# IBM/BadDiffusion

Hardware: AMD Instinct MI355X
Metric: train images/sec (32x32 UNet, DDPM-CIFAR10-32 topology, bs128/GPU, poison_rate 0.1) (higher is better)
Workload: dtype f32 (split-bf16 hi+lo products, fp32 accumulate); 1 GPU; BASELINE configs[1]: CIFAR10 DDPM-CIFAR10-32 train step, batch 128/GPU, poison_rate 0.1, BOX_14 trigger, HAT target, clip 1.0 + Adam, fp32 storage; global_batch=128, parallelism=dp1, params=35746308

## Files before the change

baddiffusion_amd/_lib.py:

```python
import ctypes as C
import os

import torch

_HERE = os.path.dirname(os.path.abspath(__file__))
LIB_PATH = os.path.join(_HERE, "libbd_hip.so")

i32, i64, f32, f64, vp, sz = C.c_int, C.c_int64, C.c_float, C.c_double, C.c_void_p, C.c_size_t


class PoisonQsampleDesc(C.Structure):
    _fields_ = [("B", i32), ("C", i32), ("H", i32), ("W", i32),
                ("images_f32", vp), ("images_u8", vp), ("is_poison", vp), ("trigger", vp), ("target_img", vp),
                ("noise", vp), ("timesteps", vp), ("alphas", vp), ("alphas_cumprod", vp), ("vmin", f32),
                ("x_noisy", vp), ("ld_noisy", i64), ("target", vp), ("ld_target", i64),
                ("R_out", vp), ("x0_out", vp), ("mask_out", vp), ("image_out", vp), ("row_index", vp), ("flip", vp)]


class QsampleDesc(C.Structure):
    _fields_ = [("B", i32), ("C", i32), ("H", i32), ("W", i32), ("x0", vp), ("R", vp), ("noise", vp),
                ("timesteps", vp), ("alphas", vp), ("alphas_cumprod", vp),
                ("x_noisy", vp), ("ld_noisy", i64), ("target", vp), ("ld_target", i64)]


class DdpmStepDesc(C.Structure):
    _fields_ = [("n", i64), ("model_output", vp), ("sample", vp), ("noise", vp), ("prev_sample", vp),
                ("pred_original", vp), ("alphas_cumprod", vp), ("t", i32), ("prev_t", i32), ("variance_type", i32),
                ("clip_sample", i32), ("clip_sample_range", f32), ("clip_defense", i32), ("clip_defense_range", f32)]


class DdimStepDesc(C.Structure):
    _fields_ = [("n", i64), ("model_output", vp), ("sample", vp), ("noise", vp), ("prev_sample", vp),
                ("pred_original", vp), ("alphas_cumprod", vp), ("t", i32), ("prev_t", i32),
                ("final_alpha_cumprod", f32), ("eta", f32), ("clip_sample", i32), ("clip_sample_range", f32)]


class GnFwdDesc(C.Structure):
    _fields_ = [("B", i32), ("HW", i32), ("C", i32), ("G", i32), ("eps", f32), ("silu", i32),
                ("x", vp), ("ldx", i64), ("gamma", vp), ("beta", vp), ("y", vp), ("ldy", i64),
                ("mean", vp), ("rstd", vp), ("workspace", vp), ("workspace_bytes", sz),
                ("y_split", vp), ("ldys", i64), ("stats", vp), ("stats_splits", i32)]


class GnBwdDesc(C.Structure):
    _fields_ = [("B", i32), ("HW", i32), ("C", i32), ("G", i32), ("silu", i32),
                ("x", vp), ("ldx", i64), ("gamma", vp), ("beta", vp), ("mean", vp), ("rstd", vp),
                ("dy", vp), ("lddy", i64), ("dx", vp), ("lddx", i64), ("accumulate_dx", i32),
                ("dgamma", vp), ("dbeta", vp), ("workspace", vp), ("workspace_bytes", sz),
                ("dx_colsum", vp), ("ld_colsum", i64), ("dx_split", vp), ("lddxs", i64),
                ("dx_add", vp), ("ld_add", i64), ("param_partials", vp), ("dx_split_c0", i32), ("dx_split_c1", i32)]


class GnParamItem(C.Structure):
    _fields_ = [("partials", vp), ("C", i32), ("dgamma", vp), ("dbeta", vp)]


class Operand(C.Structure):
    _fields_ = [("kind", i32), ("kc", i32), ("p", vp), ("ld", i64), ("bs_outer", i64), ("bs_inner", i64),
                ("C", i32), ("Hs", i32), ("Ws", i32), ("Ho", i32), ("Wo", i32), ("stride", i32),
                ("pad_t", i32), ("pad_l", i32), ("ups", i32), ("split", vp)]


class IgemmDesc(C.Structure):
    _fields_ = [("A", Operand), ("B", Operand), ("M", i32), ("N", i32), ("K", i32),
                ("batch_outer", i32), ("batch_inner", i32),
                ("C", vp), ("ldc", i64), ("c_bs_outer", i64), ("c_bs_inner", i64),
                ("alpha", f32), ("out_scale", f32), ("bias", vp),
                ("rowbias", vp), ("ld_rowbias", i64), ("rows_per_group", i32),
                ("residual", vp), ("ldr", i64), ("accumulate", i32), ("ksplit", i32),
                ("workspace", vp), ("workspace_bytes", sz), ("tile", i32), ("mode", i32),
                ("a_colsum", vp)]


class ConvFwdDesc(C.Structure):
    _fields_ = [("B", i32), ("Hs", i32), ("Ws", i32), ("Cin", i32), ("Cout", i32), ("stride", i32),
                ("pad_t", i32), ("pad_l", i32), ("ups", i32), ("Ho", i32), ("Wo", i32),
                ("x", vp), ("ldx", i64), ("w", vp), ("bias", vp), ("rowbias", vp), ("ld_rowbias", i64),
                ("residual", vp), ("ldr", i64), ("out_scale", f32), ("y", vp), ("ldy", i64),
                ("workspace", vp), ("workspace_bytes", sz), ("mode", i32), ("w_split", vp)]


class ConvDgradDesc(C.Structure):
    _fields_ = [("B", i32), ("Hs", i32), ("Ws", i32), ("Cin", i32), ("Cout", i32), ("stride", i32),
                ("pad_t", i32), ("pad_l", i32), ("ups", i32), ("Ho", i32), ("Wo", i32),
                ("dy", vp), ("lddy", i64), ("w", vp), ("dx", vp), ("lddx", i64), ("accumulate", i32),
                ("workspace", vp), ("workspace_bytes", sz), ("mode", i32), ("w_split", vp)]


class ConvWgradDesc(C.Structure):
    _fields_ = [("B", i32), ("Hs", i32), ("Ws", i32), ("Cin", i32), ("Cout", i32), ("stride", i32),
                ("pad_t", i32), ("pad_l", i32), ("ups", i32), ("Ho", i32), ("Wo", i32),
                ("x", vp), ("ldx", i64), ("dy", vp), ("lddy", i64), ("dw", vp),
                ("workspace", vp), ("workspace_bytes", sz), ("mode", i32), ("db", vp)]


class ConvPsDesc(C.Structure):
    _fields_ = [("B", i32), ("H", i32), ("W", i32), ("K", i32), ("N", i32), ("direction", i32),
                ("x_split", vp), ("ldx", i64), ("w_split", vp), ("bias", vp), ("rowbias", vp), ("ld_rowbias", i64),
                ("residual", vp), ("ldr", i64), ("out_scale", f32), ("y", vp), ("ldy", i64), ("accumulate", i32),
                ("workspace", vp), ("workspace_bytes", sz), ("gn_part", vp), ("gn_groups", i32), ("mode", i32)]


class ConvPsWgradDesc(C.Structure):
    _fields_ = [("B", i32), ("H", i32), ("W", i32), ("Cin", i32), ("Cout", i32), ("x_split", vp), ("ldx", i64),
                ("dy_split", vp), ("lddy", i64), ("dw", vp), ("db", vp), ("workspace", vp), ("workspace_bytes", sz),
                ("mode", i32)]


class UpsampleConvDesc(C.Structure):
    _fields_ = [("B", i32), ("H", i32), ("W", i32), ("Cin", i32), ("Cout", i32), ("x_split", vp), ("ldx", i64), ("dy_split", vp),
                ("lddy", i64), ("e_split", vp), ("et_split", vp), ("bias", vp), ("y", vp), ("ldy", i64), ("dx", vp), ("lddx", i64),
                ("accumulate", i32), ("dw", vp), ("db", vp), ("workspace", vp), ("workspace_bytes", sz), ("mode", i32)]


class ConvS2DgradDesc(C.Structure):
    _fields_ = [("B", i32), ("Ho", i32), ("Wo", i32), ("Cin", i32), ("Cout", i32), ("pad", i32), ("dy_split", vp), ("lddy", i64),
                ("wT_split", vp), ("dx", vp), ("lddx", i64), ("accumulate", i32), ("mode", i32)]


class GemmSpDesc(C.Structure):
    _fields_ = [("M", i32), ("N", i32), ("K", i32), ("batch", i32), ("a", vp), ("lda", i64), ("a_bs", i64), ("a_kmajor", i32),
                ("b", vp), ("ldb", i64), ("b_bs", i64), ("b_kmajor", i32), ("c", vp), ("ldc", i64), ("c_bs", i64),
                ("c_split", vp), ("ldcs", i64), ("cs_bs", i64), ("bias", vp), ("residual", vp), ("ldr", i64), ("r_bs", i64),
                ("alpha", f32), ("out_scale", f32), ("accumulate", i32), ("a_colsum", vp), ("workspace", vp), ("workspace_bytes", sz),
                ("mode", i32)]


class AttnSpDesc(C.Structure):
    _fields_ = [("B", i32), ("heads", i32), ("N", i32), ("dh", i32), ("qkv_split", vp), ("ld", i64), ("scale", f32), ("o_split", vp),
                ("ldo", i64), ("pt_split", vp), ("do_split", vp), ("lddo", i64), ("dst_split", vp), ("dqkv_split", vp), ("lddqkv", i64),
                ("mode", i32)]


class Conv2dDesc(C.Structure):
    _fields_ = [("x", vp), ("ldx", i64), ("w", vp), ("bias", vp), ("y", vp), ("ldy", i64), ("B", i32), ("H", i32), ("W", i32), ("Cin", i32),
                ("Cout", i32), ("KH", i32), ("KW", i32), ("stride_h", i32), ("stride_w", i32), ("pad_h", i32), ("pad_w", i32), ("relu", i32),
                ("w_kc", i32)]


class UnetConfig(C.Structure):
    _fields_ = [("sample_size", i32), ("in_channels", i32), ("out_channels", i32), ("num_blocks", i32),
                ("block_out_channels", i32 * 8), ("down_attn", i32 * 8), ("up_attn", i32 * 8),
                ("layers_per_block", i32), ("downsample_padding", i32), ("flip_sin_to_cos", i32),
                ("freq_shift", f32), ("norm_eps", f32), ("norm_num_groups", i32), ("attention_head_dim", i32),
                ("mid_block_scale_factor", f32), ("compute_mode", i32)]


SIGNATURES = {
    "bd_last_error": (C.c_char_p, []),
    "bd_version": (i32, []),
    "bd_poison_qsample": (i32, [C.POINTER(PoisonQsampleDesc), vp]),
    "bd_qsample": (i32, [C.POINTER(QsampleDesc), vp]),
    "bd_nchw_to_nhwc": (i32, [vp, vp, i32, i32, i32, i32, i64, vp]),
    "bd_nhwc_to_nchw": (i32, [vp, i64, vp, i32, i32, i32, i32, vp]),
    "bd_ddpm_step": (i32, [C.POINTER(DdpmStepDesc), vp]),
    "bd_ddim_step": (i32, [C.POINTER(DdimStepDesc), vp]),
    "bd_to_image": (i32, [vp, i32, i64, i32, i32, i32, i32, vp, vp, vp]),
    "bd_timestep_embedding": (i32, [vp, i32, i32, i32, i32, f32, vp, vp]),
    "bd_gn_workspace_bytes": (sz, [i32, i32]),
    "bd_gn_fwd_takes_stats": (i32, [i32, i32, i32, i32]),
    "bd_gn_fwd": (i32, [C.POINTER(GnFwdDesc), vp]),
    "bd_gn_bwd": (i32, [C.POINTER(GnBwdDesc), vp]),
    "bd_lincomb": (i32, [i32, C.POINTER(vp), C.POINTER(f32), i64, i32, f32, vp, vp]),
    "bd_anp_apply": (i32, [vp, i64, vp, vp, vp, i32, i64, vp, vp]),
    "bd_anp_grad": (i32, [vp, vp, vp, i32, i64, vp, vp, vp, vp, vp]),
    "bd_ssim_workspace_bytes": (sz, [i32, i32, i32, i32]),
    "bd_ssim": (i32, [vp, vp, i32, i32, i32, i32, i64, i64, i64, i64, f32, vp, vp, sz, vp]),
    "bd_conv2d_nhwc": (i32, [C.POINTER(Conv2dDesc), vp]),
    "bd_pool2d_nhwc": (i32, [vp, i64, vp, i64, i32, i32, i32, i32, i32, i32, i32, i32, i32, vp]),
    "bd_resize_bilinear_nhwc": (i32, [vp, i32, vp, i32, i32, i32, i32, i32, i32, f32, f32, vp]),
    "bd_global_avgpool_nhwc": (i32, [vp, i64, vp, i32, i32, i32, vp]),
    "bd_gn_bwd_defers": (i32, [i32, i32, i32, i32]),
    "bd_gn_bwd_params": (i32, [C.POINTER(GnParamItem), i32, i32, vp]),
    "bd_igemm_workspace_bytes": (sz, [C.POINTER(IgemmDesc)]),
    "bd_igemm": (i32, [C.POINTER(IgemmDesc), vp]),
    "bd_split_bf16": (i32, [vp, i64, vp, vp]),
    "bd_split_rows": (i32, [vp, i64, i64, i32, vp, i64, vp]),
    "bd_split_wt": (i32, [vp, i32, i32, vp, vp]),
    "bd_split_rows_ups2": (i32, [vp, i64, i32, i32, i32, i32, vp, i64, vp]),
    "bd_conv3x3_ps": (i32, [C.POINTER(ConvPsDesc), vp]),
    "bd_conv3x3_ps_workspace_bytes": (sz, [C.POINTER(ConvPsDesc)]),
    "bd_conv3x3_ps_gn_splits": (i32, [i32, i32, i32, i32, i32, i32]),
    "bd_upsample_weights": (i32, [vp, i32, i32, vp, vp, vp]),
    "bd_upsample_conv_fwd": (i32, [C.POINTER(UpsampleConvDesc), vp]),
    "bd_upsample_conv_dgrad": (i32, [C.POINTER(UpsampleConvDesc), vp]),
    "bd_upsample_conv_wgrad": (i32, [C.POINTER(UpsampleConvDesc), vp]),
    "bd_upsample_conv_wgrad_workspace_bytes": (sz, [C.POINTER(UpsampleConvDesc)]),
    "bd_upsample_conv_dgrad_workspace_bytes": (sz, [C.POINTER(UpsampleConvDesc)]),
    "bd_conv3x3_s2_dgrad_ps": (i32, [C.POINTER(ConvS2DgradDesc), vp]),
    "bd_gemm_sp_workspace_bytes": (sz, [C.POINTER(GemmSpDesc)]),
    "bd_gemm_sp": (i32, [C.POINTER(GemmSpDesc), vp]),
    "bd_attn_sp_supported": (i32, [i32, i32]),
    "bd_attn_sp_fwd": (i32, [C.POINTER(AttnSpDesc), vp]),
    "bd_attn_sp_bwd": (i32, [C.POINTER(AttnSpDesc), vp]),
    "bd_conv3x3_ps_wgrad": (i32, [C.POINTER(ConvPsWgradDesc), vp]),
    "bd_conv3x3_ps_wgrad_workspace_bytes": (sz, [C.POINTER(ConvPsWgradDesc)]),
    "bd_conv3x3_fwd": (i32, [C.POINTER(ConvFwdDesc), vp]),
    "bd_conv3x3_dgrad": (i32, [C.POINTER(ConvDgradDesc), vp]),
    "bd_conv3x3_wgrad": (i32, [C.POINTER(ConvWgradDesc), vp]),
    "bd_conv3x3_workspace_bytes": (sz, [i32] * 8),
    "bd_colsum": (i32, [vp, i64, i64, i32, i64, vp, i64, i32, vp]),
    "bd_sum2x2": (i32, [vp, i64, vp, i64, i32, i32, i32, i32, i32, vp]),
    "bd_softmax_fwd": (i32, [vp, vp, i64, i32, vp]),
    "bd_softmax_bwd": (i32, [vp, vp, vp, i64, i32, vp]),
    "bd_silu_fwd": (i32, [vp, vp, i64, vp]),
    "bd_silu_bwd": (i32, [vp, vp, vp, i64, i32, vp]),
    "bd_reduce_workspace_bytes": (sz, []),
    "bd_loss_fwd_bwd": (i32, [vp, i64, vp, i64, i64, i32, i32, f32, vp, vp, i64, vp, vp]),
    "bd_sumsq": (i32, [vp, i64, vp, vp, vp]),
    "bd_adam_clip": (i32, [vp, vp, vp, vp, i64, vp, f64, f64, f64, f64, f64, i32, vp, vp]),
    "bd_prof_enable": (i32, [i32]),
    "bd_prof_enabled": (i32, []),
    "bd_prof_reset": (i32, []),
    "bd_prof_num_classes": (i32, []),
    "bd_prof_get": (i32, [i32, C.POINTER(C.c_char_p), C.POINTER(i64), C.POINTER(f64), C.POINTER(f64), C.POINTER(f64)]),
    "bd_mfma_probe": (i32, [i32, i32, i32, C.POINTER(f64), vp]),
    "bd_axpy": (i32, [vp, vp, i64, f32, i32, vp]),
    "bd_adam_clip_dev": (i32, [vp, vp, vp, vp, i64, vp, f64, vp, f64, f64, f64, vp, vp]),
    "bd_unet_create": (i32, [C.POINTER(UnetConfig), C.POINTER(vp)]),
    "bd_unet_destroy": (None, [vp]),
    "bd_unet_set_compute_mode": (i32, [vp, i32]),
    "bd_unet_set_deferred_join": (i32, [vp, i32]),
    "bd_unet_stream_wait_aux": (i32, [vp, vp]),
    "bd_unet_num_params": (i64, [vp]),
    "bd_unet_num_tensors": (i32, [vp]),
    "bd_unet_param_info": (i32, [vp, i32, C.POINTER(C.c_char_p), C.POINTER(i64), C.POINTER(i32), i64 * 4, C.POINTER(i32)]),
    "bd_unet_workspace_bytes": (sz, [vp, i32, i32]),
    "bd_unet_forward": (i32, [vp, i32, i32, vp, vp, i64, vp, i32, vp, i64, vp, sz, vp]),
    "bd_unet_backward": (i32, [vp, i32, vp, vp, i64, vp, i64, vp, vp, sz, vp]),
    "bd_unet_backward_input": (i32, [vp, i32, vp, vp, i64, vp, i64, vp, vp, i64, vp, sz, vp]),
    "bd_unet_num_segments": (i32, [vp]),
    "bd_unet_set_aux_stream": (i32, [vp, i32]),
    "bd_unet_set_static_weights": (i32, [vp, i32]),
    "bd_unet_reset_static_cache": (i32, [vp]),
    "bd_tune_set": (i32, [C.c_char_p, i32]),
    "bd_unet_segment_range": (i32, [vp, i32, C.POINTER(i64), C.POINTER(i64)]),
    "bd_unet_segment_num_ranges": (i32, [vp, i32]),
    "bd_unet_segment_range_k": (i32, [vp, i32, i32, C.POINTER(i64), C.POINTER(i64)]),
    "bd_unet_backward_segment": (i32, [vp, i32, i32, vp, vp, i64, vp, i64, vp, vp, sz, vp, C.POINTER(i64), C.POINTER(i64)]),
}

_lib = None


def load():
    global _lib
    if _lib is not None:
        return _lib
    if not os.path.exists(LIB_PATH):
        raise RuntimeError(
            f"{LIB_PATH} is missing: build it with `python -m baddiffusion_amd.build` (hipcc, gfx950). "
            "There is no CPU / PyTorch fallback for the hot path.")
    lib = C.CDLL(LIB_PATH)
    for name, (res, args) in SIGNATURES.items():
        fn = getattr(lib, name)
        fn.restype = res
        fn.argtypes = args
    _lib = lib
    return lib


def check(status, what=""):
    if status != 0:
        msg = load().bd_last_error()
        raise RuntimeError(f"libbd_hip {what} failed ({status}): {msg.decode() if msg else ''}")


def ptr(t):
    return None if t is None else t.data_ptr()


def stream():
    return torch.cuda.current_stream().cuda_stream
```

baddiffusion_amd/csrc/conv_ps.hip:

```cpp
#include "common.h"
#include <string.h>

#include <type_traits>
#include <cstdlib>

namespace bd {

typedef float floatx16 __attribute__((ext_vector_type(16)));
typedef __bf16 bf16x8 __attribute__((ext_vector_type(8)));
typedef __bf16 bf16x2 __attribute__((ext_vector_type(2)));
typedef __attribute__((address_space(3))) void* lds_ptr;
typedef const __attribute__((address_space(1))) void* gbl_ptr;

constexpr int BD_WT_MAX = 64;
constexpr int PS_BM = 256, PS_BN = 128, PS_NT = 512, PS_STAGES = 3;
constexpr int PS_A_BYTES = PS_BM * 128, PS_B_BYTES = PS_BN * 128, PS_STAGE_BYTES = PS_A_BYTES + PS_B_BYTES;
constexpr int PS_LDS_BYTES = PS_STAGES * PS_STAGE_BYTES;

struct PsParams {
    const char* a;
    const char* w;
    float* y;
    const float* bias; const float* rowbias; const float* residual;
    long long lda, ldy, ldr, ld_rowbias;
// ... 1031 lines not shown
                                                            float* __restrict__ dw, float* __restrict__ db, int brows) {
    const long long i = (long long)blockIdx.x * 256 + threadIdx.x;
    const long long n4 = mn >> 2;
    if (i < n4) {
        float4 a = *reinterpret_cast<const float4*>(part + 4 * i);
#pragma unroll 4
        for (int s = 1; s < ksplit; ++s) {
            const float4 b = *reinterpret_cast<const float4*>(part + (long long)s * mn + 4 * i);
            a.x += b.x; a.y += b.y; a.z += b.z; a.w += b.w;
        }
        *reinterpret_cast<float4*>(dw + 4 * i) = a;
    } else if (db && i - n4 < M) {
        const long long m = i - n4;
        float v = 0.f;
        for (int s = 0; s < brows; ++s) v += part[(long long)ksplit * mn + (long long)s * M + m];
        db[m] = v;
    }
}

__device__ __forceinline__ unsigned ps_pack_hi(float a, float b) { return bd_pack_hi(a, b); }
__device__ __forceinline__ unsigned ps_pack_lo(float a, float b) { return bd_pack_lo(a, b); }

__global__ __launch_bounds__(256) void split_rows_kernel(const float* __restrict__ src, long long lds, long long rows, int C,
                                                          unsigned short* __restrict__ dst, long long ldd) {
    const int c8 = C >> 3;
    const long long total = rows * c8;
    for (long long i = (long long)blockIdx.x * 256 + threadIdx.x; i < total; i += (long long)gridDim.x * 256) {
        const long long r = i / c8;
        const int j = (int)(i - r * c8);
        const float4 a = *reinterpret_cast<const float4*>(src + r * lds + j * 8);
        const float4 b = *reinterpret_cast<const float4*>(src + r * lds + j * 8 + 4);
        unsigned short* o = dst + 2 * r * ldd + (j >> 2) * 64 + (j & 3) * 8;
        *reinterpret_cast<uint4*>(o) = make_uint4(ps_pack_hi(a.x, a.y), ps_pack_hi(a.z, a.w), ps_pack_hi(b.x, b.y), ps_pack_hi(b.z, b.w));
        *reinterpret_cast<uint4*>(o + 32) = make_uint4(ps_pack_lo(a.x, a.y), ps_pack_lo(a.z, a.w), ps_pack_lo(b.x, b.y), ps_pack_lo(b.z, b.w));
    }
}

__global__ __launch_bounds__(256) void split_rows_ups2_kernel(const float* __restrict__ src, long long lds, int B, int H, int W, int C,
                                                               unsigned short* __restrict__ dst, long long ldd) {
    const int c8 = C >> 3;
    const long long total = (long long)B * 4 * H * W * c8;
    for (long long i = (long long)blockIdx.x * 256 + threadIdx.x; i < total; i += (long long)gridDim.x * 256) {
        const long long r = i / c8;
        const int j = (int)(i - r * c8);
        const int x = (int)(r % (2 * W));
        const long long t = r / (2 * W);
        const int y = (int)(t % (2 * H));
        const long long b = t / (2 * H);
        const long long rs = (b * H + (y >> 1)) * W + (x >> 1);
        const float4 a = *reinterpret_cast<const float4*>(src + rs * lds + j * 8);
        const float4 bb = *reinterpret_cast<const float4*>(src + rs * lds + j * 8 + 4);
        unsigned short* o = dst + 2 * r * ldd + (j >> 2) * 64 + (j & 3) * 8;
        *reinterpret_cast<uint4*>(o) = make_uint4(ps_pack_hi(a.x, a.y), ps_pack_hi(a.z, a.w), ps_pack_hi(bb.x, bb.y), ps_pack_hi(bb.z, bb.w));
        *reinterpret_cast<uint4*>(o + 32) = make_uint4(ps_pack_lo(a.x, a.y), ps_pack_lo(a.z, a.w), ps_pack_lo(bb.x, bb.y), ps_pack_lo(bb.z, bb.w));
    }
}

__global__ __launch_bounds__(256) void split_wT_kernel(const float* __restrict__ w, int Cin, int Cout, unsigned short* __restrict__ out) {
    __shared__ float t[32][33];
    const int cib = blockIdx.x, cob = blockIdx.y, tap = blockIdx.z;
    const int tx = threadIdx.x & 31, ty = threadIdx.x >> 5;
#pragma unroll
    for (int i = 0; i < 4; ++i) {
        const int co = cob * 32 + ty + 8 * i;
        t[ty + 8 * i][tx] = w[((long long)co * 9 + tap) * Cin + cib * 32 + tx];
    }
    __syncthreads();
    const int r = threadIdx.x >> 3, c4 = (threadIdx.x & 7) * 4;
    const float v0 = t[c4][r], v1 = t[c4 + 1][r], v2 = t[c4 + 2][r], v3 = t[c4 + 3][r];
    unsigned short* o = out + 2 * (((long long)(cib * 32 + r) * 9 + tap) * Cout + cob * 32) + c4;
    *reinterpret_cast<uint2*>(o) = make_uint2(ps_pack_hi(v0, v1), ps_pack_hi(v2, v3));
    *reinterpret_cast<uint2*>(o + 32) = make_uint2(ps_pack_lo(v0, v1), ps_pack_lo(v2, v3));
}

struct WtTable {
    int n;
    long long off[BD_WT_MAX];
    int cin[BD_WT_MAX], cout[BD_WT_MAX], blk0[BD_WT_MAX + 1];
};
__global__ __launch_bounds__(256) void split_wT_batched_kernel(const float* __restrict__ params, unsigned short* __restrict__ out, WtTable t) {
    __shared__ float tl[32][33];
    int e = 0;
    while (e + 1 < t.n && (int)blockIdx.x >= t.blk0[e + 1]) ++e;
    const int Cin = t.cin[e], Cout = t.cout[e];
    const float* w = params + t.off[e];
    unsigned short* o_base = out + 2 * t.off[e];
    int b = blockIdx.x - t.blk0[e];
    const int ncib = Cin / 32, ncob = Cout / 32;
    const int cib = b % ncib; b /= ncib;
    const int cob = b % ncob; const int tap = b / ncob;
    const int tx = threadIdx.x & 31, ty = threadIdx.x >> 5;
#pragma unroll
    for (int i = 0; i < 4; ++i) {
        const int co = cob * 32 + ty + 8 * i;
        tl[ty + 8 * i][tx] = w[((long long)co * 9 + tap) * Cin + cib * 32 + tx];
    }
    __syncthreads();
    const int r = threadIdx.x >> 3, c4 = (threadIdx.x & 7) * 4;
    const float v0 = tl[c4][r], v1 = tl[c4 + 1][r], v2 = tl[c4 + 2][r], v3 = tl[c4 + 3][r];
    unsigned short* o = o_base + 2 * (((long long)(cib * 32 + r) * 9 + tap) * Cout + cob * 32) + c4;
    *reinterpret_cast<uint2*>(o) = make_uint2(ps_pack_hi(v0, v1), ps_pack_hi(v2, v3));
    *reinterpret_cast<uint2*>(o + 32) = make_uint2(ps_pack_lo(v0, v1), ps_pack_lo(v2, v3));
}

int split_wt_batched(const float* params, uint16_t* out, const long long* off, const int* cin, const int* cout, int n, hipStream_t st) {
    for (int i0 = 0; i0 < n; i0 += BD_WT_MAX) {
        WtTable t;
        t.n = n - i0 < BD_WT_MAX ? n - i0 : BD_WT_MAX;
        int blk = 0;
        for (int i = 0; i < t.n; ++i) {
            t.off[i] = off[i0 + i]; t.cin[i] = cin[i0 + i]; t.cout[i] = cout[i0 + i]; t.blk0[i] = blk;
            blk += 9 * (t.cin[i] / 32) * (t.cout[i] / 32);
        }
        t.blk0[t.n] = blk;
        hipLaunchKernelGGL(split_wT_batched_kernel, dim3((unsigned)blk), dim3(256), 0, st, params, out, t);
        BD_LAUNCH_CHECK("split_wT_batched");
    }
    return BD_OK;
}

static int ilog2x(int v) {
    if (v <= 0 || (v & (v - 1))) return -1;
    int l = 0;
    while ((1 << l) < v) ++l;
    return l;
}

bool conv3x3_ps_supported(int B, int H, int W, int K_channels, int N_channels) {
    return B > 0 && ilog2x(H) >= 0 && ilog2x(W) >= 0 && K_channels % 32 == 0 && N_channels % PS_BN == 0 && K_channels >= 32;
}
static bool ps_large(long long M, int N) { return cdiv(M, PS_BM) * (N / PS_BN) >= 96; }
static void ps_small_split(long long M, int N, int K, int& ksplit, int& cps) {
    const long long tiles = cdiv(M, 128) * (N / 128);
    const int nchunks = 9 * (K / 32);
    static const int slots = [] {
        int dev = 0, cus = 256;
        if (hipGetDevice(&dev) == hipSuccess) (void)hipDeviceGetAttribute(&cus, hipDeviceAttributeMultiprocessorCount, dev);
        return cus;
    }();
    constexpr int mincps = 4;
    int ks = (int)(slots / tiles);
    if (ks < 1) ks = 1;
    if (ks > nchunks / mincps) ks = nchunks / mincps;
    if (ks < 1) ks = 1;
    cps = (int)cdiv(nchunks, ks);
    ksplit = (int)cdiv(nchunks, cps);
}
size_t conv3x3_ps_workspace_bytes(const bd_conv3x3_ps_desc& d) {
    const long long M = (long long)d.B * d.H * d.W;
    if (d.N % PS_BN || ps_large(M, d.N)) return 0;
    int ks, cps;
    ps_small_split(M, d.N, d.K, ks, cps);
    return ks > 1 ? (size_t)ks * (size_t)M * d.N * sizeof(float) : 0;
}

static bool ps_takes_v3(int B, int H, int W, int N) {
    static const bool v3_off = getenv("BD_PS_V3") && atoi(getenv("BD_PS_V3")) == 0;
    static const int v3_maxw = getenv("BD_PS_V3_MAXW") ? atoi(getenv("BD_PS_V3_MAXW")) : (1 << 30);
    const long long M = (long long)B * H * W;
    const int vw = W < 32 ? W : 32;
    return ps_large(M, N) && !v3_off && W >= 16 && W <= v3_maxw && ((long long)H * vw) % PS_BM == 0 && M % PS_BM == 0;
}
int conv3x3_ps_gn_splits(int B, int H, int W, int K, int N, int groups) {
    if (B <= 0 || ilog2x(H) < 0 || ilog2x(W) < 0 || K <= 0 || K % 32 || N <= 0 || N % PS_BN || groups <= 0 || N % groups) return 0;
    const int lc = ilog2x(N / groups);
    if (lc < 2 || lc > 5 || (H * W) % PS_BM) return 0;
    return ps_takes_v3(B, H, W, N) ? H * W / PS_BM : 0;
}

int conv3x3_ps(const bd_conv3x3_ps_desc& d, hipStream_t st) {
    BD_CHECK(d.x_split && d.w_split && d.y, BD_ERR_INVALID, "conv3x3_ps: null pointer");
    BD_CHECK(d.B > 0 && ilog2x(d.H) >= 0 && ilog2x(d.W) >= 0, BD_ERR_UNSUPPORTED, "conv3x3_ps: H, W must be powers of two");
    BD_CHECK(d.K > 0 && d.K % 32 == 0 && d.N > 0 && d.N % PS_BN == 0, BD_ERR_UNSUPPORTED,
             "conv3x3_ps: K channels %% 32 and N channels %% %d must be 0 (got %d, %d)", PS_BN, d.K, d.N);
    BD_CHECK(d.ldx % 32 == 0 && ((uintptr_t)d.x_split & 127) == 0 && ((uintptr_t)d.w_split & 127) == 0, BD_ERR_UNSUPPORTED,
             "conv3x3_ps: split planes need ld %% 32 == 0 and 128-byte aligned bases");
    BD_CHECK(d.direction == 1 || d.direction == -1, BD_ERR_INVALID, "conv3x3_ps: direction must be +1 or -1");
    BD_CHECK(sp_mode_valid(d.mode), BD_ERR_INVALID, "conv3x3_ps: unknown compute mode %d", d.mode);
    const bool sp = d.mode == BD_MODE_BF16;
    BD_CHECK(d.ldy % 4 == 0 && ((uintptr_t)d.y & 15) == 0, BD_ERR_UNSUPPORTED, "conv3x3_ps: y needs ldy %% 4 == 0 and a 16-byte aligned base");
    BD_CHECK(!d.residual || (d.ldr % 4 == 0 && ((uintptr_t)d.residual & 15) == 0), BD_ERR_UNSUPPORTED,
             "conv3x3_ps: residual needs ldr %% 4 == 0 and a 16-byte aligned base");
    BD_CHECK(!d.rowbias || (d.ld_rowbias % 4 == 0 && ((uintptr_t)d.rowbias & 15) == 0), BD_ERR_UNSUPPORTED,
             "conv3x3_ps: rowbias needs ld_rowbias %% 4 == 0 and a 16-byte aligned base");
    BD_CHECK(!d.bias || ((uintptr_t)d.bias & 15) == 0, BD_ERR_UNSUPPORTED, "conv3x3_ps: bias needs a 16-byte aligned base");
    const long long M = (long long)d.B * d.H * d.W;
    BD_CHECK(M < (1ll << 31), BD_ERR_UNSUPPORTED, "conv3x3_ps: pixel count overflows int32");
    BD_CHECK((long long)(d.W + 1) * d.ldx * 4 < (1ll << 31), BD_ERR_UNSUPPORTED, "conv3x3_ps: row pitch too large");
    PsParams p = {};
    p.a = reinterpret_cast<const char*>(d.x_split); p.w = reinterpret_cast<const char*>(d.w_split);
    p.y = d.y; p.bias = d.bias; p.rowbias = d.rowbias; p.residual = d.residual;
    p.lda = d.ldx; p.ldy = d.ldy; p.ldr = d.ldr; p.ld_rowbias = d.ld_rowbias;
    p.C = d.K; p.H = d.H; p.W = d.W; p.lw = ilog2x(d.W); p.lhw = ilog2x(d.W) + ilog2x(d.H);
    p.sign = d.direction; p.M = (int)M; p.N = d.N;
    p.out_scale = d.out_scale == 0.f ? 1.f : d.out_scale; p.accumulate = d.accumulate;
    const bool large = ps_large(M, d.N);
    int rec = -1;
    if (prof_on()) {
        static const char* kName[2][2][2] = {{{"conv_ps128_dgrad", "conv_ps_dgrad"}, {"conv_ps128_fwd", "conv_ps_fwd"}},
                                             {{"conv_ps128_dgrad_bf16", "conv_ps_dgrad_bf16"}, {"conv_ps128_fwd_bf16", "conv_ps_fwd_bf16"}}};
        rec = prof_begin(kName[sp][d.direction > 0][large],
                         2.0 * (double)M * d.N * 9.0 * d.K, ((double)M * d.K + 9.0 * d.K * d.N + (double)M * d.N) * 4.0, st);
    }
    const int epi = (d.residual ? 1 : 0) | (d.rowbias ? 2 : 0) | (d.accumulate ? 4 : 0);
    if (large) {
        p.tiles_m = (int)cdiv(M, PS_BM); p.tiles_n = d.N / PS_BN;
        const dim3 grid((unsigned)(p.tiles_m * p.tiles_n)), block(PS_NT);
        const int vw = d.W < 32 ? d.W : 32;
        const bool v3 = ps_takes_v3(d.B, d.H, d.W, d.N);
        p.lvw = ilog2x(vw);
        if (d.gn_part) {
            BD_CHECK(d.direction == 1 && (epi == 1 || epi == 2) && conv3x3_ps_gn_splits(d.B, d.H, d.W, d.K, d.N, d.gn_groups) > 0, BD_ERR_UNSUPPORTED,
                     "conv3x3_ps: gn_part needs a forward call with exactly one of rowbias / residual and bd_conv3x3_ps_gn_splits() > 0");
            p.gn_part = d.gn_part; p.gn_G = d.gn_groups; p.gn_lcpg = ilog2x(d.N / d.gn_groups);
        }
#define PS_LAUNCH(E) do { if (v3) { if (sp) hipLaunchKernelGGL((conv_ps3_kernel<E, true>), grid, block, 0, st, p); \
                                    else hipLaunchKernelGGL((conv_ps3_kernel<E, false>), grid, block, 0, st, p); } \
                          else if (sp) hipLaunchKernelGGL((conv_ps_kernel<E, true>), grid, block, 0, st, p); \
                          else hipLaunchKernelGGL((conv_ps_kernel<E, false>), grid, block, 0, st, p); } while (0)
        switch (epi) {
            case 0: PS_LAUNCH(0); break;
            case 1: PS_LAUNCH(1); break;
            case 2: PS_LAUNCH(2); break;
            case 3: PS_LAUNCH(3); break;
            case 4: PS_LAUNCH(4); break;
            case 5: PS_LAUNCH(5); break;
            case 6: PS_LAUNCH(6); break;
            default: PS_LAUNCH(7); break;
        }
#undef PS_LAUNCH
        BD_LAUNCH_CHECK("conv_ps");
    } else {
        BD_CHECK(!d.gn_part, BD_ERR_UNSUPPORTED, "conv3x3_ps: gn_part on a small layer (bd_conv3x3_ps_gn_splits() == 0)");
        PsSmallParams pp = {};
        p.tiles_m = (int)cdiv(M, 128); p.tiles_n = d.N / 128;
        pp.q = p;
        ps_small_split(M, d.N, d.K, pp.ksplit, pp.cps);
        if (pp.ksplit > 1) {
            const size_t need = (size_t)pp.ksplit * (size_t)M * d.N * sizeof(float);
            BD_CHECK(d.workspace && d.workspace_bytes >= need, BD_ERR_WORKSPACE, "conv3x3_ps: split-K needs %zu workspace bytes, got %zu", need,
                     d.workspace_bytes);
            pp.partial = reinterpret_cast<float*>(d.workspace);
        }
        const dim3 grid((unsigned)(p.tiles_m * p.tiles_n * pp.ksplit)), block(512);
        constexpr int deep_maxcps = 9;
#define PS128_LAUNCH(E, ...) do { if (sp) hipLaunchKernelGGL((conv_ps128_kernel<E, true, ##__VA_ARGS__>), grid, block, 0, st, pp); \
                                      else hipLaunchKernelGGL((conv_ps128_kernel<E, false, ##__VA_ARGS__>), grid, block, 0, st, pp); } while (0)
        if (pp.ksplit > 1 && pp.cps <= deep_maxcps) {
            PS128_LAUNCH(0, 4);
        } else
        switch (pp.ksplit > 1 ? 0 : epi) {
            case 0: PS128_LAUNCH(0); break;
            case 1: PS128_LAUNCH(1); break;
            case 2: PS128_LAUNCH(2); break;
            case 3: PS128_LAUNCH(3); break;
            case 4: PS128_LAUNCH(4); break;
            case 5: PS128_LAUNCH(5); break;
            case 6: PS128_LAUNCH(6); break;
            default: PS128_LAUNCH(7); break;
        }
#undef PS128_LAUNCH
        BD_LAUNCH_CHECK("conv_ps128");
        if (pp.ksplit > 1) {
            hipLaunchKernelGGL(conv_ps128_reduce, dim3((unsigned)cdiv(M * (d.N / 4), 256)), dim3(256), 0, st, pp);
            BD_LAUNCH_CHECK("conv_ps128_reduce");
        }
    }
    prof_end(rec, st);
    return BD_OK;
}

bool conv3x3_ps_wgrad_supported(int B, int H, int W, int Cin, int Cout) {
    return B > 0 && ilog2x(H) >= 0 && ilog2x(W) >= 0 && Cin % WG_BN == 0 && Cout % WG_BM == 0;
}
static bool ps_wgrad_v3(const bd_conv3x3_ps_wgrad_desc& d) {
    static const bool off = getenv("BD_PS_WG3") && atoi(getenv("BD_PS_WG3")) == 0;
    static const int maxw = getenv("BD_PS_WG3_MAXW") ? atoi(getenv("BD_PS_WG3_MAXW")) : (1 << 30);
    return !off && d.W >= 16 && d.W <= maxw && ((long long)d.B * d.H * d.W) % 32 == 0;
}
static int g_wg3_slots_override = 0;
static void ps_wgrad_split(const bd_conv3x3_ps_wgrad_desc& d, int& ksplit, int& cps) {
    const bool v3 = ps_wgrad_v3(d);
    const long long tiles = (long long)(d.Cout / WG_BM) * ((v3 ? 3 : 9) * d.Cin / WG_BN);
    const int nchunks = (int)cdiv((long long)d.B * d.H * d.W, 32);
    static const int slots = [] {
        int dev = 0, cus = 256;
        if (hipGetDevice(&dev) == hipSuccess) (void)hipDeviceGetAttribute(&cus, hipDeviceAttributeMultiprocessorCount, dev);
        return 2 * cus;
    }();
    static const int slots3_getenv = getenv("BD_PS_WG3_SLOTS") ? atoi(getenv("BD_PS_WG3_SLOTS")) : 0;
    const int slots3_env = g_wg3_slots_override > 0 ? g_wg3_slots_override : slots3_getenv;
    const int slots3 = slots3_env > 0 ? slots3_env : (d.W > 32 ? slots / 4 : slots * 3 / 8);
    constexpr int mincps = 8;
    int ks = (int)((v3 ? slots3 : slots) / tiles);
    if (ks < 1) ks = 1;
    if (ks > nchunks / mincps) ks = nchunks / mincps > 0 ? nchunks / mincps : 1;
    cps = (int)cdiv(nchunks, ks);
    ksplit = (int)cdiv(nchunks, cps);
}
size_t conv3x3_ps_wgrad_workspace_bytes(const bd_conv3x3_ps_wgrad_desc& d) {
    int ks, cps;
    ps_wgrad_split(d, ks, cps);
    return ks > 1 ? (size_t)ks * ((size_t)d.Cout * 9 * d.Cin + d.Cout) * sizeof(float) : 0;
}
int conv3x3_ps_wgrad(const bd_conv3x3_ps_wgrad_desc& d, hipStream_t st) {
    BD_CHECK(d.x_split && d.dy_split && d.dw, BD_ERR_INVALID, "conv3x3_ps_wgrad: null pointer");
    BD_CHECK(d.B > 0 && conv3x3_ps_wgrad_supported(d.B, d.H, d.W, d.Cin, d.Cout), BD_ERR_UNSUPPORTED,
             "conv3x3_ps_wgrad: needs power-of-two H, W, Cin and Cout multiples of 128");
    BD_CHECK(d.ldx % 32 == 0 && d.lddy % 32 == 0 && ((uintptr_t)d.x_split & 127) == 0 && ((uintptr_t)d.dy_split & 127) == 0,
             BD_ERR_UNSUPPORTED, "conv3x3_ps_wgrad: split planes need ld %% 32 == 0 and 128-byte aligned bases");
    BD_CHECK(sp_mode_valid(d.mode), BD_ERR_INVALID, "conv3x3_ps_wgrad: unknown compute mode %d", d.mode);
    const bool sp = d.mode == BD_MODE_BF16;
    PsWgParams p = {};
    p.dy = reinterpret_cast<const char*>(d.dy_split); p.x = reinterpret_cast<const char*>(d.x_split);
    p.lddy = d.lddy; p.ldx = d.ldx; p.Cin = d.Cin; p.Cout = d.Cout; p.H = d.H; p.W = d.W; p.lw = ilog2x(d.W);
    p.lh = ilog2x(d.H); p.lvw = ilog2x(d.W < 32 ? d.W : 32);
    p.P = d.B * d.H * d.W;
    const bool v3 = ps_wgrad_v3(d);
    p.tiles_m = d.Cout / WG_BM; p.tiles_n = (v3 ? 3 : 9) * d.Cin / WG_BN; p.ntaps = 9;
    ps_wgrad_split(d, p.ksplit, p.cps);
    p.want_db = d.db != nullptr;
    const long long mn = (long long)d.Cout * 9 * d.Cin;
    if (p.ksplit > 1) {
        const size_t need = (size_t)p.ksplit * ((size_t)mn + d.Cout) * sizeof(float);
        BD_CHECK(d.workspace && d.workspace_bytes >= need, BD_ERR_WORKSPACE, "conv3x3_ps_wgrad: workspace %zu < %zu", d.workspace_bytes, need);
        p.out = reinterpret_cast<float*>(d.workspace);
    } else {
        p.out = d.dw; p.db = d.db;
    }
    int rec = -1;
    if (prof_on())
        rec = prof_begin(v3 ? (sp ? "conv_ps_wgrad3_bf16" : "conv_ps_wgrad3") : (sp ? "conv_ps_wgrad_bf16" : "conv_ps_wgrad"), 2.0 * (double)p.P * d.Cout * 9.0 * d.Cin,
                         ((double)p.P * (d.Cin + d.Cout) + 9.0 * d.Cin * d.Cout) * 4.0, st);
    const dim3 grid((unsigned)(p.tiles_m * p.tiles_n * p.ksplit));
    if (v3 && sp) hipLaunchKernelGGL(conv_ps_wgrad3_kernel<true>, grid, dim3(512), 0, st, p);
    else if (v3) hipLaunchKernelGGL(conv_ps_wgrad3_kernel<false>, grid, dim3(512), 0, st, p);
    else if (sp) hipLaunchKernelGGL((conv_ps_wgrad_kernel<2, 8, true>), grid, dim3(512), 0, st, p);
    else hipLaunchKernelGGL((conv_ps_wgrad_kernel<2, 8, false>), grid, dim3(512), 0, st, p);
    BD_LAUNCH_CHECK("conv_ps_wgrad");
    if (p.ksplit > 1) {
        const long long total = mn / 4 + (d.db ? d.Cout : 0);
        if (v3) hipLaunchKernelGGL(conv_ps_wgrad_reduce<true>, dim3((unsigned)cdiv(total, 256)), dim3(256), 0, st, p.out, p.ksplit, mn, d.Cout, d.dw, d.db, p.ksplit);
        else hipLaunchKernelGGL(conv_ps_wgrad_reduce<false>, dim3((unsigned)cdiv(total, 256)), dim3(256), 0, st, p.out, p.ksplit, mn, d.Cout, d.dw, d.db, p.ksplit);
        BD_LAUNCH_CHECK("conv_ps_wgrad_reduce");
    }
    prof_end(rec, st);
    return BD_OK;
}

int ups_dweff_combine(const float* de, int Cin, int Cout, float* dw, hipStream_t st);

static void ups_wgrad_split(const bd_upsample_conv_desc& d, int& ksplit, int& cps) {
    bd_conv3x3_ps_wgrad_desc q = {};
    q.B = d.B; q.H = d.H; q.W = d.W; q.Cin = d.Cin; q.Cout = d.Cout;
    const long long tiles = (long long)(d.Cout / WG_BM) * (16 * d.Cin / WG_BN);
    const int nchunks = (int)cdiv((long long)d.B * d.H * d.W, 32);
    int dev = 0, cus = 256;
    if (hipGetDevice(&dev) == hipSuccess) (void)hipDeviceGetAttribute(&cus, hipDeviceAttributeMultiprocessorCount, dev);
    int ks = (int)(2 * cus / tiles);
    if (ks < 1) ks = 1;
    if (ks > nchunks / 8) ks = nchunks / 8 > 0 ? nchunks / 8 : 1;
    cps = (int)cdiv(nchunks, ks);
    ksplit = (int)cdiv(nchunks, cps);
}
size_t upsample_conv_wgrad_workspace_bytes(const bd_upsample_conv_desc& d) {
    int ks, cps;
    ups_wgrad_split(d, ks, cps);
    const size_t mn = (size_t)d.Cout * 16 * d.Cin;
    return ((size_t)ks * (mn + 4 * (size_t)d.Cout) + mn) * sizeof(float);
}
int upsample_conv_wgrad(const bd_upsample_conv_desc& d, hipStream_t st) {
    BD_CHECK(d.x_split && d.dy_split && d.dw, BD_ERR_INVALID, "bd_upsample_conv_wgrad: null pointer");
    BD_CHECK(d.B > 0 && conv3x3_ps_wgrad_supported(d.B, d.H, d.W, d.Cin, d.Cout), BD_ERR_UNSUPPORTED,
             "bd_upsample_conv_wgrad: needs power-of-two H, W, Cin and Cout multiples of 128");
    BD_CHECK(d.ldx % 32 == 0 && d.lddy % 32 == 0 && ((uintptr_t)d.x_split & 127) == 0 && ((uintptr_t)d.dy_split & 127) == 0,
             BD_ERR_UNSUPPORTED, "bd_upsample_conv_wgrad: split planes need ld %% 32 == 0 and 128-byte aligned bases");
    BD_CHECK((long long)d.B * d.H * d.W * 4 < (1ll << 31), BD_ERR_UNSUPPORTED, "bd_upsample_conv_wgrad: pixel count overflows int32");
    BD_CHECK(sp_mode_valid(d.mode), BD_ERR_INVALID, "bd_upsample_conv_wgrad: unknown compute mode %d", d.mode);
    const size_t need = upsample_conv_wgrad_workspace_bytes(d);
    BD_CHECK(d.workspace && d.workspace_bytes >= need, BD_ERR_WORKSPACE, "bd_upsample_conv_wgrad: workspace %zu < %zu", d.workspace_bytes, need);
    PsWgParams p = {};
    p.dy = reinterpret_cast<const char*>(d.dy_split); p.x = reinterpret_cast<const char*>(d.x_split);
    p.lddy = d.lddy; p.ldx = d.ldx; p.Cin = d.Cin; p.Cout = d.Cout; p.H = d.H; p.W = d.W; p.lw = ilog2x(d.W);
    p.P = d.B * d.H * d.W;
    p.tiles_m = d.Cout / WG_BM; p.tiles_n = 16 * d.Cin / WG_BN; p.ntaps = 16;
    ups_wgrad_split(d, p.ksplit, p.cps);
    p.want_db = d.db != nullptr;
    const long long mn = (long long)d.Cout * 16 * d.Cin;
    p.out = reinterpret_cast<float*>(d.workspace);
    float* de = p.out + (size_t)p.ksplit * ((size_t)mn + 4 * (size_t)d.Cout);
    int rec = -1;
    if (prof_on())
        rec = prof_begin(d.mode == BD_MODE_BF16 ? "conv_ph_ups_wgrad_bf16" : "conv_ph_ups_wgrad", 2.0 * (double)p.P * 4.0 * d.Cout * 9.0 * d.Cin,
                         ((double)p.P * (d.Cin + 4.0 * d.Cout) + 9.0 * d.Cin * d.Cout) * 4.0, st);
    const dim3 grid((unsigned)(p.tiles_m * p.tiles_n * p.ksplit));
    if (d.mode == BD_MODE_BF16) hipLaunchKernelGGL((conv_ps_wgrad_kernel<2, 8, true, true>), grid, dim3(512), 0, st, p);
    else hipLaunchKernelGGL((conv_ps_wgrad_kernel<2, 8, false, true>), grid, dim3(512), 0, st, p);
    BD_LAUNCH_CHECK("conv_ps_wgrad (phase)");
    const long long total = mn / 4 + (d.db ? d.Cout : 0);
    hipLaunchKernelGGL(conv_ps_wgrad_reduce<false>, dim3((unsigned)cdiv(total, 256)), dim3(256), 0, st, p.out, p.ksplit, mn, d.Cout, de, d.db, 4 * p.ksplit);
    BD_LAUNCH_CHECK("conv_ps_wgrad_reduce (phase)");
    BD_TRY(ups_dweff_combine(de, d.Cin, d.Cout, d.dw, st));
    prof_end(rec, st);
    return BD_OK;
}

int g_tune_gen = 0;
int tune_set(const char* key, int value) {
    BD_CHECK(key, BD_ERR_INVALID, "bd_tune_set: null key");
    if (!strcmp(key, "ps_wg3_slots")) { g_wg3_slots_override = value > 0 ? value : 0; ++g_tune_gen; return BD_OK; }
    set_error("bd_tune_set: unknown key '%s' (known: ps_wg3_slots)", key);
    return BD_ERR_INVALID;
}
}

extern "C" int bd_tune_set(const char* key, int value) { return bd::tune_set(key, value); }
extern "C" size_t bd_upsample_conv_wgrad_workspace_bytes(const bd_upsample_conv_desc* d) {
    return d ? bd::upsample_conv_wgrad_workspace_bytes(*d) : 0;
}
extern "C" int bd_upsample_conv_wgrad(const bd_upsample_conv_desc* d, bd_stream_t s) {
    BD_CHECK(d, BD_ERR_INVALID, "bd_upsample_conv_wgrad: null descriptor");
    return bd::upsample_conv_wgrad(*d, bd::S(s));
}
extern "C" size_t bd_conv3x3_ps_workspace_bytes(const bd_conv3x3_ps_desc* d) { return d ? bd::conv3x3_ps_workspace_bytes(*d) : 0; }
extern "C" int bd_conv3x3_ps_gn_splits(int B, int H, int W, int K, int N, int groups) { return bd::conv3x3_ps_gn_splits(B, H, W, K, N, groups); }
extern "C" int bd_conv3x3_ps(const bd_conv3x3_ps_desc* d, bd_stream_t s) {
    BD_CHECK(d, BD_ERR_INVALID, "bd_conv3x3_ps: null descriptor");
    return bd::conv3x3_ps(*d, bd::S(s));
}
extern "C" int bd_conv3x3_ps_wgrad(const bd_conv3x3_ps_wgrad_desc* d, bd_stream_t s) {
    BD_CHECK(d, BD_ERR_INVALID, "bd_conv3x3_ps_wgrad: null descriptor");
    return bd::conv3x3_ps_wgrad(*d, bd::S(s));
}
extern "C" size_t bd_conv3x3_ps_wgrad_workspace_bytes(const bd_conv3x3_ps_wgrad_desc* d) {
    return d ? bd::conv3x3_ps_wgrad_workspace_bytes(*d) : 0;
}
extern "C" int bd_split_rows(const float* src, int64_t ld_src, int64_t rows, int C, uint16_t* dst, int64_t ld_dst, bd_stream_t stream) {
    BD_CHECK(src && dst && rows > 0 && C > 0, BD_ERR_INVALID, "bd_split_rows: bad args");
    BD_CHECK(C % 32 == 0 && ld_dst % 32 == 0 && (ld_src & 3) == 0 && bd::aligned16(src) && ((uintptr_t)dst & 127) == 0, BD_ERR_UNSUPPORTED,
             "bd_split_rows: C, ld_dst %% 32, ld_src %% 4, 16-byte aligned src and 128-byte aligned dst required");
    long long nb = bd::cdiv(rows * (C / 8), 256);
    if (nb > 8192) nb = 8192;
    hipLaunchKernelGGL(bd::split_rows_kernel, dim3((unsigned)nb), dim3(256), 0, bd::S(stream), src, (long long)ld_src, (long long)rows, C, dst,
                       (long long)ld_dst);
    BD_LAUNCH_CHECK("split_rows");
    return BD_OK;
}
extern "C" int bd_split_rows_ups2(const float* src, int64_t ld_src, int B, int H, int W, int C, uint16_t* dst, int64_t ld_dst, bd_stream_t stream) {
    BD_CHECK(src && dst && B > 0 && H > 0 && W > 0 && C > 0, BD_ERR_INVALID, "bd_split_rows_ups2: bad args");
    BD_CHECK(C % 32 == 0 && ld_dst % 32 == 0 && (ld_src & 3) == 0 && bd::aligned16(src) && ((uintptr_t)dst & 127) == 0, BD_ERR_UNSUPPORTED,
             "bd_split_rows_ups2: C, ld_dst %% 32, ld_src %% 4, 16-byte aligned src and 128-byte aligned dst required");
    long long nb = bd::cdiv((long long)B * 4 * H * W * (C / 8), 256);
    if (nb > 8192) nb = 8192;
    hipLaunchKernelGGL(bd::split_rows_ups2_kernel, dim3((unsigned)nb), dim3(256), 0, bd::S(stream), src, (long long)ld_src, B, H, W, C, dst,
                       (long long)ld_dst);
    BD_LAUNCH_CHECK("split_rows_ups2");
    return BD_OK;
}
extern "C" int bd_split_wt(const float* w, int Cin, int Cout, uint16_t* out, bd_stream_t stream) {
    BD_CHECK(w && out && Cin > 0 && Cout > 0, BD_ERR_INVALID, "bd_split_wt: bad args");
    BD_CHECK(Cin % 32 == 0 && Cout % 32 == 0 && ((uintptr_t)out & 127) == 0, BD_ERR_UNSUPPORTED, "bd_split_wt: Cin, Cout %% 32 and 128-byte aligned out required");
    hipLaunchKernelGGL(bd::split_wT_kernel, dim3(Cin / 32, Cout / 32, 9), dim3(256), 0, bd::S(stream), w, Cin, Cout, out);
    BD_LAUNCH_CHECK("split_wT");
    return BD_OK;
}
```

baddiffusion_amd/csrc/groupnorm.hip:

```cpp
#include "common.h"

namespace bd {

constexpr int GN_MAX_SPLITS = 128;

static int gn_max_splits(int B) {
    int s = 512 / (B > 0 ? B : 1);
    return s < 1 ? 1 : (s > GN_MAX_SPLITS ? GN_MAX_SPLITS : s);
}
static int gn_splits(int B, int HW) {
    int s = 512 / (B > 0 ? B : 1);
    if (s < 1) s = 1;
    if (s > GN_MAX_SPLITS) s = GN_MAX_SPLITS;
    while (s > 1 && HW / s < 32) s >>= 1;
    return s;
}
static void gn_block(int C, int& threads, int& r) {
    const int q = C / 4;
    r = 256 / q;
    if (r < 1) r = 1;
    threads = q * r;
}

static int gn_apply_rows(int HW, int r) {
// ... 297 lines not shown
            for (int sp = sub; sp < S; sp += nsub) s += (double)p[(long long)sp * 3 * C];
        }
        red[t] = s;
        __syncthreads();
        if (base + t < items && t < (nsub > 1 ? items : 256)) {
            double v = red[t];
            for (int k = 1; k < nsub; ++k) v += red[k * items + t];
            tot[base + t] = v;
        }
        __syncthreads();
    }
    if (t < 2) {
        double v = 0.0;
        const double* q = tot + (t == 0 ? cpg : 0);
        for (int c = 0; c < cpg; ++c) v += q[c] * (double)gamma[g * cpg + c];
        sg[t] = v;
        ds[((long long)b * G + g) * 2 + t] = (float)v;
    }
    if (ppart)
        for (int i = t; i < 2 * cpg; i += 256) {
            const int plane = i / cpg, c = g * cpg + i - plane * cpg;
            ppart[((long long)b * 2 + plane) * C + c] = (float)tot[i];
        }
    if (dx_colsum) {
        __syncthreads();
        const float s1 = (float)sg[0], s2 = (float)sg[1], rs = rstd[b * G + g];
        for (int cl = t; cl < cpg; cl += 256) {
            const int c = g * cpg + cl;
            const float sa = (float)tot[cpg + cl], sh2 = (float)tot[2 * cpg + cl];
            dx_colsum[(long long)b * ld_colsum + c] = rs * (gamma[c] * sa - ((float)HW * s1 + s2 * sh2) * inv_n);
        }
    }
}

__global__ void gn_bwd_apply_kernel(const float* __restrict__ x, long long ldx, const float* __restrict__ dy, long long lddy,
                                    float* __restrict__ dx, long long lddx, int HW, int C, int G, int r, int per,
                                    const float* __restrict__ ds, const float* __restrict__ gamma,
                                    const float* __restrict__ beta, const float* __restrict__ mean,
                                    const float* __restrict__ rstd, float inv_n, int silu, int acc,
                                    unsigned short* __restrict__ dxs, long long lddxs, const float* __restrict__ addp,
                                    long long ldadd, int dxs_c0, int dxs_c1) {
    const int q = C / 4, cpg = C / G;
    const int t = threadIdx.x;
    const int cq = t % q, prow = t / q;
    const int b = blockIdx.y;
    const int p0 = blockIdx.x * per;
    int p1 = p0 + per;
    if (p1 > HW) p1 = HW;
    float mu[4], rs[4], gg[4], bb[4], g1[4], g2[4];
#pragma unroll
    for (int j = 0; j < 4; ++j) {
        const int c = cq * 4 + j, g = c / cpg;
        mu[j] = mean[b * G + g]; rs[j] = rstd[b * G + g];
        g1[j] = ds[((long long)b * G + g) * 2]; g2[j] = ds[((long long)b * G + g) * 2 + 1];
        gg[j] = gamma[c]; bb[j] = beta[c];
    }
    const float* xb = x + (long long)b * HW * ldx + cq * 4;
    const float* db = dy + (long long)b * HW * lddy + cq * 4;
    float* ob = dx + (long long)b * HW * lddx + cq * 4;
    const bool do_acc = dx && acc;
    const float* ab = addp ? addp + (long long)b * HW * ldadd + cq * 4 : xb;
    for (int p = p0 + prow; p < p1; p += 2 * r) {
        float4 v[2], d[2], e[2], a2[2];
#pragma unroll
        for (int u = 0; u < 2; ++u) {
            const bool ok = p + u * r < p1;
            v[u] = gn_ld4_if(xb + (long long)(p + u * r) * ldx, ok);
            d[u] = gn_ld4_if(db + (long long)(p + u * r) * lddy, ok);
            e[u] = gn_ld4_if(ob + (long long)(p + u * r) * lddx, ok && do_acc);
            a2[u] = gn_ld4_if(ab + (long long)(p + u * r) * ldadd, ok && addp != nullptr);
        }
#pragma unroll
        for (int u = 0; u < 2; ++u) {
            const float in[4] = {v[u].x, v[u].y, v[u].z, v[u].w}, dd[4] = {d[u].x, d[u].y, d[u].z, d[u].w};
            const float ee[4] = {e[u].x, e[u].y, e[u].z, e[u].w}, aa[4] = {a2[u].x, a2[u].y, a2[u].z, a2[u].w};
            float o[4];
#pragma unroll
            for (int j = 0; j < 4; ++j) {
                const float xh = (in[j] - mu[j]) * rs[j];
                float dz = dd[j];
                if (silu) dz *= silu_grad_fast(xh * gg[j] + bb[j]);
                o[j] = (rs[j] * (dz * gg[j] - (g1[j] + xh * g2[j]) * inv_n) + ee[j]) + aa[j];
            }
            v[u] = make_float4(o[0], o[1], o[2], o[3]);
        }
#pragma unroll
        for (int u = 0; u < 2; ++u) {
            const int pu = p + u * r;
            if (pu < p1) {
                if (dx) *reinterpret_cast<float4*>(ob + (long long)pu * lddx) = v[u];
                if (dxs && cq * 4 >= dxs_c0 && cq * 4 < dxs_c1) {
                    const float o[4] = {v[u].x, v[u].y, v[u].z, v[u].w};
                    gn_store_split4(dxs + 2 * ((long long)b * HW + pu) * lddxs, cq * 4 - dxs_c0, o);
                }
            }
        }
    }
}

constexpr int GN_RES_EMAX = 16;

struct GnRes {
    int cb, q, R, E, nblk, nt;
};
static int gcd_i(int a, int b) { return b ? gcd_i(b, a % b) : a; }
static bool gn_resident_plan(int B, int HW, int C, int G, GnRes& o, bool wide_ok = false) {
    const int cpg = C / G;
    const int unit = cpg / gcd_i(cpg, 4) * 4;
    for (int nt = 256; nt <= 512; nt *= 2) {
        int best = 0;
        for (int cb = unit; cb <= C; cb += unit) {
            if (C % cb) continue;
            const int q = cb / 4;
            if (q > nt) break;
            if (cdiv(HW, nt / q) <= GN_RES_EMAX && cb / cpg <= 256) best = cb;
        }
        if (!best || (best < 16 && best < C)) continue;
        constexpr int row_align = 64;
        if ((best * 4) % row_align != 0 && best < C) continue;
        while ((long long)B * (C / best) < 512) {
            const int half = best / 2;
            if (half < 16 || half % unit || C % half) break;
            best = half;
        }
        o.cb = best; o.q = best / 4; o.R = nt / o.q; o.E = (int)cdiv(HW, o.R); o.nblk = C / best; o.nt = nt;
        if (wide_ok && nt == 256 && o.E > 8 && 512 % o.q == 0) { o.nt = 512; o.R = 512 / o.q; o.E = (int)cdiv(HW, o.R); }
        return true;
    }
    return false;
}

struct GnCoord {
    int b, bx;
};
__device__ __forceinline__ GnCoord gn_res_coord(int nblk) {
    const unsigned L = blockIdx.x, T = gridDim.x, qq = T >> 3;
    unsigned j = (L & 7) * qq + (L >> 3);
    if (L >= (qq << 3)) j = L;
    GnCoord c;
    c.b = (int)(j / (unsigned)nblk);
    c.bx = (int)(j - (unsigned)c.b * (unsigned)nblk);
    return c;
}

__device__ __forceinline__ void gn_fwd_group_stats(double a, double c2, double n, float eps, float* st, float* mean, float* rstd) {
    const double mu = a / n;
    double var = c2 / n - mu * mu;
    if (var < 0.0) var = 0.0;
    const float m = (float)mu, r = (float)(1.0 / sqrt(var + (double)eps));
    st[0] = m; st[1] = r;
    *mean = m; *rstd = r;
}

template <int EMAX, int NT>
__global__ __launch_bounds__(NT, NT == 256 ? 4 : 2) void gn_fwd_res_kernel(const float* __restrict__ x, long long ldx, float* __restrict__ y,
                                                       long long ldy, int HW, int C, int G, int cb, int q, int R, int E,
                                                       float eps, const float* __restrict__ gamma,
                                                       const float* __restrict__ beta, float* __restrict__ mean,
                                                       float* __restrict__ rstd, int silu, unsigned short* __restrict__ ys,
                                                       long long ldys) {
    __shared__ double shd[4 * NT];
    float* sh = reinterpret_cast<float*>(shd);
    __shared__ float st[2 * 256];
    const int t = threadIdx.x;
    const int cq = t % q, prow = t / q;
    const bool active = prow < R;
    const GnCoord wgc = gn_res_coord(C / cb);
    const int b = wgc.b, c0 = wgc.bx * cb;
    const int cpg = C / G, ng = cb / cpg;
    const float* xb = x + (long long)b * HW * ldx + c0 + cq * 4;
    float4 v[EMAX];
    float sm[4] = {0.f, 0.f, 0.f, 0.f}, sq[4] = {0.f, 0.f, 0.f, 0.f};
#pragma unroll
    for (int i = 0; i < EMAX; ++i) {
        const int p = prow + R * i;
        const bool ok = active && i < E && p < HW;
        v[i] = gn_ld4_if(xb + (long long)p * ldx, ok);
        sm[0] += v[i].x; sm[1] += v[i].y; sm[2] += v[i].z; sm[3] += v[i].w;
        sq[0] += v[i].x * v[i].x; sq[1] += v[i].y * v[i].y; sq[2] += v[i].z * v[i].z; sq[3] += v[i].w * v[i].w;
    }
    const bool wred = q < 64 && (q & (q - 1)) == 0;
    const int rows = wred ? NT / 64 : R;
    if (wred) {
        double a[4], c2[4];
#pragma unroll
        for (int j = 0; j < 4; ++j) { a[j] = (double)sm[j]; c2[j] = (double)sq[j]; }
        for (int off = q; off < 64; off <<= 1) {
#pragma unroll
            for (int j = 0; j < 4; ++j) { a[j] += __shfl_xor(a[j], off); c2[j] += __shfl_xor(c2[j], off); }
        }
        if ((t & 63) < q) {
#pragma unroll
            for (int j = 0; j < 4; ++j) {
                shd[((t >> 6) * cb + cq * 4 + j) * 2 + 0] = a[j];
                shd[((t >> 6) * cb + cq * 4 + j) * 2 + 1] = c2[j];
            }
        }
    } else if (active) {
#pragma unroll
        for (int j = 0; j < 4; ++j) {
            sh[(prow * cb + cq * 4 + j) * 2 + 0] = sm[j];
            sh[(prow * cb + cq * 4 + j) * 2 + 1] = sq[j];
        }
    }
    __syncthreads();
    if (wred) {
        if (t < ng) {
            double a = 0.0, c2 = 0.0;
            for (int pr = 0; pr < rows; ++pr)
                for (int c = t * cpg; c < (t + 1) * cpg; ++c) {
                    a += shd[(pr * cb + c) * 2 + 0];
                    c2 += shd[(pr * cb + c) * 2 + 1];
                }
            gn_fwd_group_stats(a, c2, (double)HW * cpg, eps, st + 2 * t, mean + b * G + c0 / cpg + t, rstd + b * G + c0 / cpg + t);
        }
    } else {
        for (int g = t >> 6; g < ng; g += NT / 64) {
            double a = 0.0, c2 = 0.0;
            for (int idx = t & 63; idx < R * cpg; idx += 64) {
                const int pr = idx / cpg, c = g * cpg + idx - pr * cpg;
                a += (double)sh[(pr * cb + c) * 2 + 0];
                c2 += (double)sh[(pr * cb + c) * 2 + 1];
            }
            for (int off = 1; off < 64; off <<= 1) { a += __shfl_xor(a, off); c2 += __shfl_xor(c2, off); }
            if ((t & 63) == 0)
                gn_fwd_group_stats(a, c2, (double)HW * cpg, eps, st + 2 * g, mean + b * G + c0 / cpg + g, rstd + b * G + c0 / cpg + g);
        }
    }
    __syncthreads();
    if (!active) return;
    float mu[4], rs[4], gg[4], bb[4];
#pragma unroll
    for (int j = 0; j < 4; ++j) {
        const int lc = cq * 4 + j;
        mu[j] = st[2 * (lc / cpg)]; rs[j] = st[2 * (lc / cpg) + 1];
        gg[j] = gamma[c0 + lc]; bb[j] = beta[c0 + lc];
    }
    float* yb = y + (long long)b * HW * ldy + c0 + cq * 4;
#pragma unroll
    for (int i = 0; i < EMAX; ++i) {
        const float in[4] = {v[i].x, v[i].y, v[i].z, v[i].w};
        float o[4];
#pragma unroll
        for (int j = 0; j < 4; ++j) {
            const float z = (in[j] - mu[j]) * rs[j] * gg[j] + bb[j];
            o[j] = silu ? silu_fast_pinned(z) : z;
        }
        v[i] = make_float4(o[0], o[1], o[2], o[3]);
    }
#pragma unroll
    for (int i = 0; i < EMAX; ++i) {
        const int p = prow + R * i;
        if (i < E && p < HW) {
            if (y) *reinterpret_cast<float4*>(yb + (long long)p * ldy) = v[i];
            if (ys) {
                const float o[4] = {v[i].x, v[i].y, v[i].z, v[i].w};
                gn_store_split4(ys + 2 * ((long long)b * HW + p) * ldys, c0 + cq * 4, o);
            }
        }
    }
}

template <int EMAX, int NT>
__global__ __launch_bounds__(NT) void gn_bwd_res_kernel(const float* __restrict__ x, long long ldx,
                                                       const float* __restrict__ dy, long long lddy, float* __restrict__ dx,
                                                       long long lddx, int HW, int C, int G, int cb, int q, int R, int E,
                                                       const float* __restrict__ gamma, const float* __restrict__ beta,
                                                       const float* __restrict__ mean, const float* __restrict__ rstd,
                                                       int silu, int acc, float* __restrict__ part,
                                                       float* __restrict__ dx_colsum, long long ld_colsum,
                                                       unsigned short* __restrict__ dxs, long long lddxs,
                                                       const float* __restrict__ addp, long long ldadd, int dxs_c0, int dxs_c1) {
    __shared__ float sh[3 * 4 * NT];
    __shared__ float ch[3 * 4 * NT];
    __shared__ float sg[2 * 256];
    const int t = threadIdx.x;
    const int cq = t % q, prow = t / q;
    const bool active = prow < R;
    const GnCoord wgc = gn_res_coord(C / cb);
    const int b = wgc.b, c0 = wgc.bx * cb;
    const int cpg = C / G, ng = cb / cpg;
    const float inv_n = 1.0f / ((float)HW * cpg);
    float mu[4], rs[4], gg[4], bb[4];
#pragma unroll
    for (int j = 0; j < 4; ++j) {
        const int c = c0 + (active ? cq * 4 + j : 0);
        mu[j] = mean[b * G + c / cpg]; rs[j] = rstd[b * G + c / cpg];
        gg[j] = gamma[c]; bb[j] = beta[c];
    }
    const float* xb = x + (long long)b * HW * ldx + c0 + cq * 4;
    const float* db = dy + (long long)b * HW * lddy + c0 + cq * 4;
    float4 xh[EMAX], dz[EMAX];
    float s0[4] = {0.f, 0.f, 0.f, 0.f}, s1[4] = {0.f, 0.f, 0.f, 0.f}, s2[4] = {0.f, 0.f, 0.f, 0.f};
#pragma unroll
    for (int i = 0; i < EMAX; ++i) {
        const int p = prow + R * i;
        const bool ok = active && i < E && p < HW;
        xh[i] = gn_ld4_if(xb + (long long)p * ldx, ok);
        dz[i] = gn_ld4_if(db + (long long)p * lddy, ok);
    }
#pragma unroll
    for (int i = 0; i < EMAX; ++i) {
        const int p = prow + R * i;
        const bool ok = active && i < E && p < HW;
        float in[4] = {xh[i].x, xh[i].y, xh[i].z, xh[i].w}, dd[4] = {dz[i].x, dz[i].y, dz[i].z, dz[i].w};
#pragma unroll
        for (int j = 0; j < 4; ++j) {
            const float h = ok ? (in[j] - mu[j]) * rs[j] : 0.f;
            float d = dd[j];
            if (silu) d *= silu_grad_fast(h * gg[j] + bb[j]);
            in[j] = h; dd[j] = d;
            s0[j] += d; s1[j] += d * h; s2[j] += h;
        }
        xh[i] = make_float4(in[0], in[1], in[2], in[3]);
        dz[i] = make_float4(dd[0], dd[1], dd[2], dd[3]);
    }
    const bool wred = q < 64 && (q & (q - 1)) == 0;
    const int rows = wred ? NT / 64 : R;
    if (wred) {
        for (int off = q; off < 64; off <<= 1) {
#pragma unroll
            for (int j = 0; j < 4; ++j) {
                s0[j] += __shfl_xor(s0[j], off); s1[j] += __shfl_xor(s1[j], off); s2[j] += __shfl_xor(s2[j], off);
            }
        }
    }
    if (wred ? (t & 63) < q : active) {
        const int row = wred ? (t >> 6) : prow;
#pragma unroll
        for (int j = 0; j < 4; ++j) {
            float* o = sh + (row * cb + cq * 4 + j) * 3;
            o[0] = s0[j]; o[1] = s1[j]; o[2] = s2[j];
        }
    }
    __syncthreads();
    if (wred) {
        for (int c = t; c < cb; c += NT) {
            float a = 0.f, e = 0.f, h = 0.f;
            for (int pr = 0; pr < rows; ++pr) {
                const float* o = sh + (pr * cb + c) * 3;
                a += o[0]; e += o[1]; h += o[2];
            }
            ch[3 * c] = a; ch[3 * c + 1] = e; ch[3 * c + 2] = h;
            if (part) {
                float* o = part + (long long)b * 2 * C + c0 + c;
                o[0] = e;
                o[C] = a;
            }
        }
    } else {
        for (int c = t >> 6; c < cb; c += NT / 64) {
            float a = 0.f, e = 0.f, h = 0.f;
            for (int pr = t & 63; pr < R; pr += 64) {
                const float* o = sh + (pr * cb + c) * 3;
                a += o[0]; e += o[1]; h += o[2];
            }
            for (int off = 1; off < 64; off <<= 1) { a += __shfl_xor(a, off); e += __shfl_xor(e, off); h += __shfl_xor(h, off); }
            if ((t & 63) == 0) {
                ch[3 * c] = a; ch[3 * c + 1] = e; ch[3 * c + 2] = h;
                if (part) {
                    float* o = part + (long long)b * 2 * C + c0 + c;
                    o[0] = e;
                    o[C] = a;
                }
            }
        }
    }
    __syncthreads();
    if (t < ng) {
        double a = 0.0, e = 0.0;
        for (int c = t * cpg; c < (t + 1) * cpg; ++c) {
            a += (double)ch[3 * c] * gamma[c0 + c];
            e += (double)ch[3 * c + 1] * gamma[c0 + c];
        }
        sg[2 * t] = (float)a; sg[2 * t + 1] = (float)e;
    }
    __syncthreads();
    if (dx_colsum) {
        for (int c = t; c < cb; c += NT) {
            const int g = c / cpg;
            const float r = rstd[b * G + (c0 + c) / cpg];
            dx_colsum[(long long)b * ld_colsum + c0 + c] =
                r * (gamma[c0 + c] * ch[3 * c] - ((float)HW * sg[2 * g] + sg[2 * g + 1] * ch[3 * c + 2]) * inv_n);
        }
    }
    if (!active) return;
    float g1[4], g2[4];
#pragma unroll
    for (int j = 0; j < 4; ++j) {
        const int g = (cq * 4 + j) / cpg;
        g1[j] = sg[2 * g]; g2[j] = sg[2 * g + 1];
    }
    float* ob = dx + (long long)b * HW * lddx + c0 + cq * 4;
#pragma unroll
    for (int i = 0; i < EMAX; ++i) {
        const float h[4] = {xh[i].x, xh[i].y, xh[i].z, xh[i].w}, d[4] = {dz[i].x, dz[i].y, dz[i].z, dz[i].w};
        float o[4];
#pragma unroll
        for (int j = 0; j < 4; ++j) o[j] = rs[j] * (d[j] * gg[j] - (g1[j] + h[j] * g2[j]) * inv_n);
        dz[i] = make_float4(o[0], o[1], o[2], o[3]);
    }
    if (dx && acc) {
#pragma unroll
        for (int i = 0; i < EMAX; ++i) {
            const int p = prow + R * i;
            xh[i] = gn_ld4_if(ob + (long long)p * lddx, i < E && p < HW);
        }
#pragma unroll
        for (int i = 0; i < EMAX; ++i) { dz[i].x += xh[i].x; dz[i].y += xh[i].y; dz[i].z += xh[i].z; dz[i].w += xh[i].w; }
    }
    if (addp) {
        const float* ab = addp + (long long)b * HW * ldadd + c0 + cq * 4;
#pragma unroll
        for (int i = 0; i < EMAX; ++i) {
            const int p = prow + R * i;
            xh[i] = gn_ld4_if(ab + (long long)p * ldadd, i < E && p < HW);
        }
#pragma unroll
        for (int i = 0; i < EMAX; ++i) { dz[i].x += xh[i].x; dz[i].y += xh[i].y; dz[i].z += xh[i].z; dz[i].w += xh[i].w; }
    }
#pragma unroll
    for (int i = 0; i < EMAX; ++i) {
        const int p = prow + R * i;
        if (i < E && p < HW) {
            if (dx) *reinterpret_cast<float4*>(ob + (long long)p * lddx) = dz[i];
            if (dxs && c0 + cq * 4 >= dxs_c0 && c0 + cq * 4 < dxs_c1) {
                const float o[4] = {dz[i].x, dz[i].y, dz[i].z, dz[i].w};
                gn_store_split4(dxs + 2 * ((long long)b * HW + p) * lddxs, c0 + cq * 4 - dxs_c0, o);
            }
        }
    }
}

static int gn_common_checks(const char* who, int B, int HW, int C, int G, const void* x, long long ldx) {
    BD_CHECK(B > 0 && HW > 0 && C > 0 && G > 0, BD_ERR_INVALID, "%s: bad shape", who);
    BD_CHECK(C % G == 0, BD_ERR_INVALID, "%s: C=%d not divisible by G=%d", who, C, G);
    BD_CHECK((C & 3) == 0 && (ldx & 3) == 0 && aligned16(x), BD_ERR_UNSUPPORTED,
             "%s: needs C and ld multiples of 4 and a 16B-aligned pointer (C=%d ld=%lld)", who, C, ldx);
    BD_CHECK(C / 4 <= 1024, BD_ERR_UNSUPPORTED, "%s: C=%d too large", who, C);
    BD_CHECK(B <= 65535, BD_ERR_UNSUPPORTED, "%s: B=%d too large", who, B);
    return BD_OK;
}

}

using namespace bd;

extern "C" size_t bd_gn_workspace_bytes(int B, int C) {
    const size_t ms = (size_t)gn_max_splits(B);
    size_t fwd = (size_t)B * ms * (size_t)C * 2 * sizeof(double);
    size_t bwd = (size_t)B * ms * (size_t)C * 3 * sizeof(float) + (size_t)B * C * 2 * sizeof(float) + 256;
    return fwd > bwd ? fwd : bwd;
}

extern "C" int bd_gn_fwd(const bd_gn_fwd_desc* d, bd_stream_t stream) {
    BD_CHECK(d, BD_ERR_INVALID, "bd_gn_fwd: null descriptor");
    BD_TRY(gn_common_checks("bd_gn_fwd", d->B, d->HW, d->C, d->G, d->x, d->ldx));
    BD_CHECK(d->gamma && d->beta && (d->y || d->y_split) && d->mean && d->rstd && d->workspace, BD_ERR_INVALID, "bd_gn_fwd: null pointer");
    BD_CHECK((d->ldy & 3) == 0 && aligned16(d->y) && aligned16(d->gamma) && aligned16(d->beta), BD_ERR_UNSUPPORTED,
             "bd_gn_fwd: y/gamma/beta must be 16B aligned, ldy multiple of 4");
    BD_CHECK(!d->y_split || (d->C % 32 == 0 && d->ldys % 32 == 0 && ((uintptr_t)d->y_split & 127) == 0), BD_ERR_UNSUPPORTED,
             "bd_gn_fwd: y_split needs C %% 32 == 0, ldys %% 32 == 0 and a 128-byte aligned base");
    GnRes rp;
    if (gn_resident_plan(d->B, d->HW, d->C, d->G, rp)) {
        const dim3 grid((unsigned)rp.nblk * (unsigned)d->B);
        int rec = -1;
        if (prof_on())
            rec = prof_begin("gn_fwd_res", 0.0, (double)d->B * d->HW * d->C * 4.0 * (1.0 + (d->y ? 1.0 : 0.0) + (d->y_split ? 1.0 : 0.0)), S(stream));
#define BD_GN_FWD_RES(EM, NT)                                                                                              \
    hipLaunchKernelGGL((gn_fwd_res_kernel<EM, NT>), grid, dim3(NT), 0, S(stream), d->x, (long long)d->ldx, d->y,             \
                       (long long)d->ldy, d->HW, d->C, d->G, rp.cb, rp.q, rp.R, rp.E, d->eps, d->gamma, d->beta, d->mean,       \
                       d->rstd, d->silu, d->y_split, (long long)d->ldys)
        if (rp.nt == 512 && rp.E <= 8) BD_GN_FWD_RES(8, 512);
        else if (rp.nt == 512) BD_GN_FWD_RES(GN_RES_EMAX, 512);
        else if (rp.E <= 4) BD_GN_FWD_RES(4, 256);
        else BD_GN_FWD_RES(GN_RES_EMAX, 256);
#undef BD_GN_FWD_RES
        BD_LAUNCH_CHECK("gn_fwd_res");
        prof_end(rec, S(stream));
        return BD_OK;
    }
    const int S_ = gn_splits(d->B, d->HW);
    const size_t need = (size_t)d->B * S_ * d->G * 2 * sizeof(double);
    BD_CHECK(d->workspace_bytes >= need, BD_ERR_WORKSPACE, "bd_gn_fwd: workspace %zu < %zu", d->workspace_bytes, need);
    int threads, r;
    gn_block(d->C, threads, r);
    const double* part = reinterpret_cast<double*>(d->workspace);
    int Sf = S_;
    if (d->stats) {
        BD_CHECK(d->stats_splits > 0, BD_ERR_INVALID, "bd_gn_fwd: stats without stats_splits");
        part = d->stats; Sf = d->stats_splits;
    } else {
        hipLaunchKernelGGL(gn_stats_kernel, dim3(S_, d->B), dim3(threads), (size_t)r * d->C * 2 * sizeof(float), S(stream), d->x,
                           (long long)d->ldx, d->HW, d->C, d->G, r, S_, reinterpret_cast<double*>(d->workspace));
        BD_LAUNCH_CHECK("gn_stats");
    }
    {
        const int per = gn_apply_rows(d->HW, r);
        hipLaunchKernelGGL(gn_fwd_finalize_kernel, dim3(d->B), dim3(256), 0, S(stream), part, d->G, Sf,
                           (double)d->HW * (d->C / d->G), d->eps, d->mean, d->rstd);
        hipLaunchKernelGGL(gn_apply_kernel, dim3((unsigned)cdiv(d->HW, per), d->B), dim3(threads), 0, S(stream), d->x,
                           (long long)d->ldx, d->y, (long long)d->ldy, d->HW, d->C, d->G, r, per, d->gamma, d->beta, d->mean,
                           d->rstd, d->silu, d->y_split, (long long)d->ldys);
    }
    BD_LAUNCH_CHECK("gn_apply");
    return BD_OK;
}

extern "C" int bd_gn_fwd_takes_stats(int B, int HW, int C, int G) {
    GnRes rp;
    return B > 0 && HW > 0 && C > 0 && G > 0 && C % G == 0 && (C & 3) == 0 && !gn_resident_plan(B, HW, C, G, rp) ? 1 : 0;
}

extern "C" int bd_gn_bwd_defers(int B, int HW, int C, int G) {
    return B > 0 && HW > 0 && C > 0 && G > 0 && C % G == 0 && (C & 3) == 0 ? 1 : 0;
}

extern "C" int bd_gn_bwd_params(const bd_gn_param_item* items, int n, int B, bd_stream_t stream) {
    BD_CHECK(items && n > 0 && B > 0, BD_ERR_INVALID, "bd_gn_bwd_params: bad arguments");
    for (int i0 = 0; i0 < n; i0 += GN_PARAM_MAX) {
        GnParamTable t;
        t.n = n - i0 < GN_PARAM_MAX ? n - i0 : GN_PARAM_MAX;
        int blk = 0;
        for (int i = 0; i < t.n; ++i) {
            const bd_gn_param_item& it = items[i0 + i];
            BD_CHECK(it.partials && it.dgamma && it.dbeta && it.C > 0, BD_ERR_INVALID, "bd_gn_bwd_params: item %d", i0 + i);
            t.part[i] = it.partials; t.dg[i] = it.dgamma; t.db[i] = it.dbeta; t.C[i] = it.C; t.blk0[i] = blk;
            blk += (int)cdiv(2 * it.C, 64);
        }
        t.blk0[t.n] = blk;
        hipLaunchKernelGGL(gn_bwd_param_batched_kernel, dim3((unsigned)blk), dim3(1024), 0, S(stream), t, B);
        BD_LAUNCH_CHECK("gn_bwd_param_batched");
    }
    return BD_OK;
}

extern "C" int bd_gn_bwd(const bd_gn_bwd_desc* d, bd_stream_t stream) {
    BD_CHECK(d, BD_ERR_INVALID, "bd_gn_bwd: null descriptor");
    BD_TRY(gn_common_checks("bd_gn_bwd", d->B, d->HW, d->C, d->G, d->x, d->ldx));
    BD_CHECK(d->gamma && d->beta && d->mean && d->rstd && d->dy && (d->dx || d->dx_split) && d->workspace,
             BD_ERR_INVALID, "bd_gn_bwd: null pointer");
    const bool no_params = !d->dgamma && !d->dbeta && !d->param_partials;
    BD_CHECK(no_params || (d->dgamma && d->dbeta), BD_ERR_INVALID, "bd_gn_bwd: dgamma and dbeta go together (both null with null param_partials = no parameter gradients)");
    BD_CHECK(!d->dx_split || (d->C % 32 == 0 && d->lddxs % 32 == 0 && ((uintptr_t)d->dx_split & 127) == 0), BD_ERR_UNSUPPORTED,
             "bd_gn_bwd: dx_split needs C %% 32 == 0, lddxs %% 32 == 0 and a 128-byte aligned base");
    const int xs0 = d->dx_split_c1 > d->dx_split_c0 ? d->dx_split_c0 : 0, xs1 = d->dx_split_c1 > d->dx_split_c0 ? d->dx_split_c1 : d->C;
    BD_CHECK(!d->dx_split || (xs0 >= 0 && xs1 <= d->C && xs0 % 32 == 0 && xs1 % 32 == 0 && d->lddxs >= xs1 - xs0), BD_ERR_INVALID,
             "bd_gn_bwd: dx_split channel range [%d, %d) must be whole 32-channel blocks inside C = %d with lddxs >= its width", xs0, xs1, d->C);
    BD_CHECK(d->dx || !d->accumulate_dx, BD_ERR_INVALID, "bd_gn_bwd: accumulate_dx needs dx");
    BD_CHECK((d->lddy & 3) == 0 && (d->lddx & 3) == 0 && aligned16(d->dy) && aligned16(d->dx) && aligned16(d->gamma) &&
                 aligned16(d->beta), BD_ERR_UNSUPPORTED, "bd_gn_bwd: pointers must be 16B aligned, ld multiples of 4");
    BD_CHECK(!(d->dx_colsum && (d->accumulate_dx || d->dx_add)), BD_ERR_INVALID, "bd_gn_bwd: dx_colsum is the column sum of this launch's dx term alone");
    BD_CHECK(!d->dx_add || (d->dx && (d->ld_add & 3) == 0 && aligned16(d->dx_add)), BD_ERR_INVALID, "bd_gn_bwd: dx_add needs dx, a 16B-aligned pointer and ld_add %% 4 == 0");
    GnRes rp;
    if (gn_resident_plan(d->B, d->HW, d->C, d->G, rp, true)) {
        const size_t need_r = d->param_partials || no_params ? 0 : (size_t)d->B * d->C * 2 * sizeof(float);
        BD_CHECK(d->workspace_bytes >= need_r, BD_ERR_WORKSPACE, "bd_gn_bwd: workspace %zu < %zu", d->workspace_bytes, need_r);
        float* part_r = d->param_partials ? d->param_partials : (no_params ? nullptr : reinterpret_cast<float*>(d->workspace));
        const dim3 grid((unsigned)rp.nblk * (unsigned)d->B);
        int rec = -1;
        if (prof_on())
            rec = prof_begin("gn_bwd_res", 0.0, (double)d->B * d->HW * 4.0 * ((double)d->C * (2.0 + (d->accumulate_dx ? 1.0 : 0.0) + (d->dx_add ? 1.0 : 0.0) +
                             (d->dx ? 1.0 : 0.0)) + (d->dx_split ? (double)(xs1 - xs0) : 0.0)), S(stream));
#define BD_GN_BWD_RES(EM, NT)                                                                                              \
    hipLaunchKernelGGL((gn_bwd_res_kernel<EM, NT>), grid, dim3(NT), 0, S(stream), d->x, (long long)d->ldx, d->dy,            \
                       (long long)d->lddy, d->dx, (long long)d->lddx, d->HW, d->C, d->G, rp.cb, rp.q, rp.R, rp.E, d->gamma,     \
                       d->beta, d->mean, d->rstd, d->silu, d->accumulate_dx, part_r, d->dx_colsum, (long long)d->ld_colsum, \
                       d->dx_split, (long long)d->lddxs, d->dx_add, (long long)d->ld_add, xs0, xs1)
        if (rp.nt == 512 && rp.E <= 8) BD_GN_BWD_RES(8, 512);
        else if (rp.nt == 512) BD_GN_BWD_RES(GN_RES_EMAX, 512);
        else if (rp.E <= 4) BD_GN_BWD_RES(4, 256);
        else BD_GN_BWD_RES(GN_RES_EMAX, 256);
#undef BD_GN_BWD_RES
        BD_LAUNCH_CHECK("gn_bwd_res");
        prof_end(rec, S(stream));
        if (d->param_partials || no_params) return BD_OK;
        hipLaunchKernelGGL(gn_bwd_param_kernel, dim3((unsigned)cdiv(2 * d->C, 64)), dim3(1024), 0, S(stream), part_r, d->B, 2 * d->C,
                           d->C, d->dgamma, d->dbeta);
        BD_LAUNCH_CHECK("gn_bwd_param");
        return BD_OK;
    }
    const int S_ = gn_splits(d->B, d->HW);
    const size_t part_bytes = align_up((size_t)d->B * S_ * d->C * 3 * sizeof(float), 256);
    const size_t need = part_bytes + (size_t)d->B * d->G * 2 * sizeof(float);
    BD_CHECK(d->workspace_bytes >= need, BD_ERR_WORKSPACE, "bd_gn_bwd: workspace %zu < %zu", d->workspace_bytes, need);
    float* part = reinterpret_cast<float*>(d->workspace);
    float* ds = reinterpret_cast<float*>(reinterpret_cast<char*>(d->workspace) + part_bytes);
    int threads, r;
    gn_block(d->C, threads, r);
    hipLaunchKernelGGL(gn_bwd_stats_kernel, dim3(S_, d->B), dim3(threads), (size_t)r * d->C * 3 * sizeof(float), S(stream), d->x,
                       (long long)d->ldx, d->dy, (long long)d->lddy, d->HW, d->C, d->G, r, S_, d->gamma, d->beta, d->mean,
                       d->rstd, d->silu, part);
    BD_LAUNCH_CHECK("gn_bwd_stats");
    if (!d->param_partials && !no_params) {
        hipLaunchKernelGGL(gn_bwd_param_kernel, dim3((unsigned)cdiv(2 * d->C, 64)), dim3(1024), 0, S(stream), part, d->B * S_, 3 * d->C,
                           d->C, d->dgamma, d->dbeta);
        BD_LAUNCH_CHECK("gn_bwd_param");
    }
    {
        const int per = gn_apply_rows(d->HW, r);
        const float inv_n = 1.0f / ((float)d->HW * (d->C / d->G));
        hipLaunchKernelGGL(gn_bwd_finalize_kernel, dim3(d->B, (unsigned)d->G), dim3(256), (size_t)(256 + 3 * (d->C / d->G) + 2) * sizeof(double),
                           S(stream), part, d->HW, d->C, d->G, S_, d->gamma, d->rstd, inv_n, ds, d->dx_colsum, (long long)d->ld_colsum,
                           d->param_partials);
        hipLaunchKernelGGL(gn_bwd_apply_kernel, dim3((unsigned)cdiv(d->HW, per), d->B), dim3(threads), 0, S(stream), d->x,
                           (long long)d->ldx, d->dy, (long long)d->lddy, d->dx, (long long)d->lddx, d->HW, d->C, d->G, r, per, ds,
                           d->gamma, d->beta, d->mean, d->rstd, inv_n, d->silu, d->accumulate_dx, d->dx_split,
                           (long long)d->lddxs, d->dx_add, (long long)d->ld_add, xs0, xs1);
    }
    BD_LAUNCH_CHECK("gn_bwd_apply");
    return BD_OK;
}
```

baddiffusion_amd/csrc/unet_plan.cpp:

```cpp
#include "common.h"

#include <functional>
#include <string>
#include <vector>
#include <cmath>
#include <cstdlib>

namespace bd {

int conv3x3_fwd(const bd_conv3x3_fwd_desc& d, hipStream_t st);
int conv3x3_dgrad(const bd_conv3x3_dgrad_desc& d, hipStream_t st);
int conv3x3_wgrad(const bd_conv3x3_wgrad_desc& d, hipStream_t st);
bool conv3x3_wgrad_is_thin(const bd_conv3x3_wgrad_desc& d);
int conv3x3_ps(const bd_conv3x3_ps_desc& d, hipStream_t st);
bool conv3x3_ps_supported(int B, int H, int W, int K_channels, int N_channels);
int conv3x3_ps_wgrad(const bd_conv3x3_ps_wgrad_desc& d, hipStream_t st);
size_t conv3x3_ps_wgrad_workspace_bytes(const bd_conv3x3_ps_wgrad_desc& d);
bool conv3x3_ps_wgrad_supported(int B, int H, int W, int Cin, int Cout);
int upsample_weights(const float* w, int Cin, int Cout, uint16_t* e_split, uint16_t* et_split, hipStream_t st);
int upsample_conv_fwd(const bd_upsample_conv_desc& d, hipStream_t st);
int upsample_conv_dgrad(const bd_upsample_conv_desc& d, hipStream_t st);
int upsample_conv_wgrad(const bd_upsample_conv_desc& d, hipStream_t st);
size_t upsample_conv_wgrad_workspace_bytes(const bd_upsample_conv_desc& d);
size_t upsample_conv_dgrad_workspace_bytes(const bd_upsample_conv_desc& d);
bool upsample_conv_ps_supported(int B, int H, int W, int Cin, int Cout);
int conv3x3_s2_dgrad_ps(const bd_conv3x3_s2_dgrad_desc& d, hipStream_t st);
int gemm_sp(const bd_gemm_sp_desc& d, hipStream_t st);
size_t gemm_sp_workspace_bytes(const bd_gemm_sp_desc& d);
bool gemm_sp_supported(int M, int N, int K);
int attn_sp_fwd(const bd_attn_sp_desc& d, hipStream_t st);
int attn_sp_bwd(const bd_attn_sp_desc& d, hipStream_t st);
bool attn_sp_supported(int N, int dh);
int split_wt_batched(const float* params, uint16_t* out, const long long* off, const int* cin, const int* cout, int n, hipStream_t st);

struct View {
    int buf = -1;
    int coff = 0;
    int C = 0, ld = 0, H = 0, W = 0;
};

enum Region { R_VALUE = 0, R_GRAD = 1, R_SCRATCH = 2 };
struct Buf {
    int64_t per_sample = 0, fixed = 0;
    int region = R_VALUE, group = 0;
    int64_t off = 0;
    int gbuf = -1;
    std::function<bool(int, int)> live;
};

struct Param {
    std::string name;
    int64_t off;
    int rank;
    int64_t shape[4];
    int layout;
};

struct Ctx {
    bool dry = false;
    bool training = true;
    int B = 0;
    int64_t s0 = 0;
    int LB = 0;
    float* ws = nullptr;
    const float* params = nullptr;
    float* grads = nullptr;
    hipStream_t st = nullptr;
    const float* x = nullptr; int64_t ldx = 0;
    const int64_t* t = nullptr; int t_stride = 0;
    float* out = nullptr; int64_t ldo = 0;
    const float* dout = nullptr; int64_t lddo = 0;
    bool wg = true;
    float* dx = nullptr; int64_t lddx = 0;
    char* opws = nullptr; size_t opws_bytes = 0; size_t opws_need = 0;
    hipStream_t st2 = nullptr; hipEvent_t ev_fork = nullptr, ev_join[2] = {nullptr, nullptr};
    char* opws2 = nullptr; int par = 0; bool launched = false, pend[2] = {false, false};
    const uint16_t* w_split = nullptr;
    const uint16_t* wT_split = nullptr;
    std::vector<char> ginit;
    float* gnpart = nullptr; size_t gnpart_floats = 0, gnpart_used = 0, gnpart_need = 0;
    std::vector<bd_gn_param_item> gn_items;
    float* gn_slot(int B, int HW, int C, int G, float* dgamma, float* dbeta) {
        if (!wg || !bd_gn_bwd_defers(B, HW, C, G)) return nullptr;
        const size_t n = ((size_t)B * 2 * C + 63) / 64 * 64;
        if (dry) { gnpart_need += n; return nullptr; }
        if (!gnpart || gnpart_used + n > gnpart_floats) return nullptr;
        float* p = gnpart + gnpart_used;
        gnpart_used += n;
        bd_gn_param_item it; it.partials = p; it.C = C; it.dgamma = dgamma; it.dbeta = dbeta;
        gn_items.push_back(it);
        return p;
    }
};

struct Conv3 {
    int64_t pw, pb;
    int Cin, Cout, Hs, Ws;
    int stride, pad, ups;
    int Ho, Wo;
};
static Conv3 conv3_same(int64_t pw, int64_t pb, int Cin, int Cout, int H, int W) { return Conv3{pw, pb, Cin, Cout, H, W, 1, 1, 0, H, W}; }
struct Opnd { const float* p; int64_t ld; };
struct Conv3Epi {
    const float* rowbias = nullptr; int64_t ld_rowbias = 0;
    const float* residual = nullptr; int64_t ldr = 0;
    float out_scale = 1.f;
    int gn_splits = 0;
};

typedef std::function<int(Ctx&)> Step;

}

using namespace bd;

struct bd_unet {
    bd_unet_config cfg;
    hipStream_t aux_stream = nullptr;
    hipEvent_t aux_ev_fork = nullptr, aux_ev_join[2] = {nullptr, nullptr};
    hipEvent_t aux_ev_seg = nullptr;
    bool aux_pend[2] = {false, false};
    int aux_enabled = 1, aux_defer = 0;
    std::vector<Buf> bufs;
    std::vector<Param> params;
    int64_t nparams = 0;
    std::vector<Step> fwd;
    struct BStep { Step fn; int seg; int group; };
    std::vector<BStep> bwd;
    struct Seg { int64_t lo, hi; int64_t tw_lo = -1, tw_hi = -1, tb_lo = -1, tb_hi = -1; };
    std::vector<Seg> segs;
    int cur_seg = 0, cur_group = 0;
    int lay_B = -1, lay_train = -1, lay_gen = -1;
    int fwd_gen = -1, fwd_B = -1; const void* fwd_ws = nullptr;
    int64_t value_floats = 0, grad_floats = 0, scratch_floats = 0;
    size_t opws_bytes = 0, gnpart_floats = 0;
    int T = 0, sumC = 0;
    int64_t p_tw = 0, p_tb = 0;
    int b_tproj = -1, b_dtproj = -1, b_embs = -1;
    std::vector<long long> wt_off; std::vector<int> wt_cin, wt_cout;
    struct GSplit { int buf, coff, C, H, W; int b_pl; std::function<bool(int)> want; bool claimed = false, emitted = false; };
    std::vector<GSplit> gsplits;
    int reg_gsplit(const View& y, std::function<bool(int)> want) {
        static const bool off = getenv("BD_GSPLIT") && atoi(getenv("BD_GSPLIT")) == 0;
        if (off || y.buf < 0 || y.C % 32 != 0) return -1;
        GSplit e; e.buf = y.buf; e.coff = y.coff; e.C = y.C; e.H = y.H; e.W = y.W; e.want = std::move(want);
        const int keep = cur_group;
        e.b_pl = new_buf((int64_t)y.H * y.W * y.C, 0, R_GRAD);
        cur_group = keep;
        gsplits.push_back(std::move(e));
        const int idx = (int)gsplits.size() - 1;
        bufs[gsplits[idx].b_pl].live = [this, idx](int B, int training) { return training && gsplits[idx].emitted && gsplits[idx].want(B); };
        return idx;
    }
    int claim_gsplit(const View& x, bool emits) {
        int got = -1;
        for (int i = 0; i < (int)gsplits.size(); ++i) {
            GSplit& e = gsplits[i];
            if (e.claimed || e.buf != x.buf || e.coff < x.coff || e.coff + e.C > x.coff + x.C) continue;
            e.claimed = true;
            if (emits && got < 0) { e.emitted = true; got = i; }
        }
        return got;
    }
    struct UpsW { int64_t pw; int C, H, W; int b_e, b_et; };
    int static_weights = 0; const void* prep_params = nullptr; const void* prep_ws = nullptr; int prep_B = -1;
    std::vector<UpsW> upsw;

    int new_buf(int64_t per_sample, int64_t fixed, int region) {
        Buf b;
        b.per_sample = per_sample; b.fixed = fixed; b.region = region; b.group = cur_group;
        bufs.push_back(b);
        return (int)bufs.size() - 1;
    }
    View new_tensor(int H, int W, int C) {
        View v;
        v.buf = new_buf((int64_t)H * W * C, 0, R_VALUE);
        bufs[v.buf].gbuf = new_buf((int64_t)H * W * C, 0, R_GRAD);
        v.coff = 0; v.C = C; v.ld = C; v.H = H; v.W = W;
        return v;
    }
    View slice(const View& v, int coff, int C) const {
        View s = v;
        s.coff = v.coff + coff; s.C = C;
        return s;
    }
    int scratch(int64_t per_sample, int64_t fixed = 0) { return new_buf(per_sample, fixed, R_SCRATCH); }
    int64_t add_param(const std::string& name, std::initializer_list<int64_t> shape, int layout = 0) {
        Param p;
        p.name = name; p.rank = (int)shape.size(); p.layout = layout;
        int64_t n = 1; int i = 0;
        for (auto s : shape) { p.shape[i++] = s; n *= s; }
        for (; i < 4; ++i) p.shape[i] = 1;
        nparams = (nparams + 31) / 32 * 32;
        p.off = nparams;
        nparams += n;
        params.push_back(p);
        if (!segs.empty()) {
            Seg& s = segs[cur_seg];
            if (s.lo < 0 || p.off < s.lo) s.lo = p.off;
            if (p.off + n > s.hi) s.hi = p.off + n;
        }
        return p.off;
    }
    void alias_param(const std::string& name, int64_t off, std::initializer_list<int64_t> shape) {
        Param p;
        p.name = name; p.rank = (int)shape.size(); p.layout = 0; p.off = off;
        int i = 0;
        for (auto s : shape) p.shape[i++] = s;
        for (; i < 4; ++i) p.shape[i] = 1;
        params.push_back(p);
    }
    void F(Step s) { fwd.push_back(std::move(s)); }
    void Bk(Step s) { bwd.push_back({std::move(s), cur_seg, cur_group}); }

    float* VP(Ctx& c, const View& v) const { return c.ws + bufs[v.buf].off + c.s0 * bufs[v.buf].per_sample + v.coff; }
    float* GP(Ctx& c, const View& v) const {
        const Buf& g = bufs[bufs[v.buf].gbuf];
        return c.ws + g.off + c.s0 * g.per_sample + v.coff;
    }
    float* BP(Ctx& c, int b) const { return c.ws + bufs[b].off + c.s0 * bufs[b].per_sample; }
    float* MEANP(Ctx& c, int b, int G) const { return c.ws + bufs[b].off + c.s0 * G; }
    float* RSTDP(Ctx& c, int b, int G) const { return c.ws + bufs[b].off + ((int64_t)c.LB + c.s0) * G; }
    static int64_t rows(const Ctx& c, const View& v) { return (int64_t)c.B * v.H * v.W; }

    template <class F>
    int on_aux(Ctx& c, F&& launch) const {
        if (!c.st2 || c.dry) return launch(c.st, c.opws);
        BD_HIP_TRY(hipEventRecord(c.ev_fork, c.st));
        BD_HIP_TRY(hipStreamWaitEvent(c.st2, c.ev_fork, 0));
        c.launched = true;
        return launch(c.st2, c.opws2);
    }
    static int aux_wait(Ctx& c, int p) {
        if (!c.pend[p]) return BD_OK;
        BD_HIP_TRY(hipStreamWaitEvent(c.st, c.ev_join[p], 0));
        c.pend[p] = false;
        return BD_OK;
    }
    static int aux_mark(Ctx& c, int p) {
        if (!c.launched) return BD_OK;
        BD_HIP_TRY(hipEventRecord(c.ev_join[p], c.st2));
        c.pend[p] = true; c.launched = false;
        return BD_OK;
    }
    static void need(Ctx& c, size_t bytes) { if (bytes > c.opws_need) c.opws_need = bytes; }
    static void note_conv(Ctx& c) { need(c, bd_conv3x3_workspace_bytes(0, 0, 0, 0, 0, 0, 0, 0)); }
    static int take_ginit(Ctx& c, int buf) {
        const int acc = c.ginit[buf];
        c.ginit[buf] = 1;
        return acc;
    }
    static int lay_batch(const Ctx& c) { return c.LB > 0 ? c.LB : c.B; }
    static bool planes(const Ctx& c) { return c.dry || c.w_split; }
    static uint16_t* U16(float* p) { return reinterpret_cast<uint16_t*>(p); }
    static const uint16_t* U16(const float* p) { return reinterpret_cast<const uint16_t*>(p); }

    int igemm(Ctx& c, bd_igemm_desc& g) const {
        g.workspace = c.opws; g.workspace_bytes = c.opws_bytes; g.mode = cfg.compute_mode;
        if (c.dry) { need(c, igemm_workspace_bytes(g)); return BD_OK; }
        return igemm_launch(g, c.st);
    }
    int gemm_s(Ctx& c, bd_gemm_sp_desc& g, bool aux = false) const {
        if (aux && !c.wg) return BD_OK;
        g.workspace_bytes = c.opws_bytes; g.mode = cfg.compute_mode;
        if (c.dry) { need(c, gemm_sp_workspace_bytes(g)); return BD_OK; }
        if (aux) return on_aux(c, [&](hipStream_t st, char* ws) { g.workspace = ws; return gemm_sp(g, st); });
        g.workspace = c.opws;
        return gemm_sp(g, c.st);
    }
    static bd_operand dense(const float* p, int64_t ld, int kc) {
        bd_operand o = {};
        o.kind = BD_OPK_DENSE; o.kc = kc; o.p = p; o.ld = ld;
        return o;
    }
    int linear_fwd(Ctx& c, const float* A, int64_t lda, const float* W, const float* bias, float* C, int64_t ldc, int M, int N,
                   int K, const float* residual = nullptr, int64_t ldr = 0, float out_scale = 1.f) const {
        bd_igemm_desc g = {};
        g.A = dense(A, lda, 1); g.B = dense(W, K, 1);
        g.M = M; g.N = N; g.K = K; g.batch_outer = g.batch_inner = 1;
        g.C = C; g.ldc = ldc; g.alpha = 1.f; g.out_scale = out_scale; g.bias = bias; g.residual = residual; g.ldr = ldr;
        return igemm(c, g);
    }
    int linear_dgrad(Ctx& c, const float* dY, int64_t lddy, const float* W, float* dX, int64_t lddx, int M, int N, int K,
                     int acc) const {
        bd_igemm_desc g = {};
        g.A = dense(dY, lddy, 1); g.B = dense(W, K, 0);
        g.M = M; g.N = K; g.K = N; g.batch_outer = g.batch_inner = 1;
        g.C = dX; g.ldc = lddx; g.alpha = 1.f; g.out_scale = 1.f; g.accumulate = acc;
        return igemm(c, g);
    }
    int linear_wgrad(Ctx& c, const float* dY, int64_t lddy, const float* X, int64_t ldx, float* dW, int M, int N, int K,
                     float* db = nullptr) const {
        if (!c.wg) return BD_OK;
        bd_igemm_desc g = {};
        g.A = dense(dY, lddy, 0); g.B = dense(X, ldx, 0);
        g.M = N; g.N = K; g.K = M; g.batch_outer = g.batch_inner = 1;
        g.C = dW; g.ldc = K; g.alpha = 1.f; g.out_scale = 1.f; g.a_colsum = db;
        if (c.dry) return igemm(c, g);
        g.workspace_bytes = c.opws_bytes; g.mode = cfg.compute_mode;
        return on_aux(c, [&](hipStream_t st, char* ws) { g.workspace = ws; return igemm_launch(g, st); });
    }
    int colsum(Ctx& c, const float* x, int64_t ldx, int64_t nrows, int N, int64_t rpg, float* out, int64_t ldo) const {
        if (c.dry) return BD_OK;
        return bd_colsum(x, ldx, nrows, N, rpg, out, ldo, 0, c.st);
    }
    int bias_grad(Ctx& c, const float* dY, int64_t ld, int HW, int N, int scratch_buf, float* db, float* db2 = nullptr) const {
        if (!c.wg) return BD_OK;
        float* s = BP(c, scratch_buf);
        BD_TRY(colsum(c, dY, ld, (int64_t)c.B * HW, N, HW, s, N));
        BD_TRY(colsum(c, s, N, c.B, N, c.B, db, N));
        if (db2) BD_TRY(colsum(c, s, N, c.B, N, c.B, db2, N));
        return BD_OK;
    }
    int add(Ctx& c, const float* src, int64_t lds, float* dst, int64_t ldd, int64_t nrows, int C, float scale, int acc) const {
        if (c.dry) return BD_OK;
        return add_launch(src, lds, dst, ldd, nrows, C, scale, acc, c.st);
    }
    int split_rows(Ctx& c, const float* src, int64_t ld, int64_t nrows, int C, float* dst) const {
        if (c.dry) return BD_OK;
        return bd_split_rows(src, ld, nrows, C, U16(dst), C, (bd_stream_t)c.st);
    }

    int gn_fwd(Ctx& c, const View& x, int64_t pg, int64_t pb, float* y, int64_t ldy, int stats_buf, int silu, bool planes = false,
               int stats_splits = 0) const {
        bd_gn_fwd_desc d = {};
        d.B = c.B; d.HW = x.H * x.W; d.C = x.C; d.G = cfg.norm_num_groups; d.eps = cfg.norm_eps; d.silu = silu;
        d.x = VP(c, x); d.ldx = x.ld; d.gamma = c.params + pg; d.beta = c.params + pb;
        if (planes) { d.y = nullptr; d.ldy = x.C; d.y_split = U16(y); d.ldys = x.C; }
        else { d.y = y; d.ldy = ldy; }
        d.mean = MEANP(c, stats_buf, d.G); d.rstd = RSTDP(c, stats_buf, d.G);
        d.workspace = c.opws; d.workspace_bytes = c.opws_bytes;
        if (stats_splits > 0) { d.stats = reinterpret_cast<const double*>(c.opws); d.stats_splits = stats_splits; }
        if (c.dry) { need(c, bd_gn_workspace_bytes(c.B, x.C)); return BD_OK; }
        return bd_gn_fwd(&d, (bd_stream_t)c.st);
    }
    int gn_bwd(Ctx& c, bd_gn_bwd_desc& d, const View& x, int64_t pg, int64_t pb, int stats_buf, const float* dy, int64_t lddy, int silu) const {
        d.B = c.B; d.HW = x.H * x.W; d.C = x.C; d.G = cfg.norm_num_groups; d.silu = silu;
        d.x = VP(c, x); d.ldx = x.ld; d.gamma = c.params + pg; d.beta = c.params + pb;
        d.mean = MEANP(c, stats_buf, d.G); d.rstd = RSTDP(c, stats_buf, d.G);
        d.dy = dy; d.lddy = lddy;
        if (c.wg) { d.dgamma = c.grads + pg; d.dbeta = c.grads + pb; }
        else { d.dx_colsum = nullptr; d.ld_colsum = 0; }
        d.workspace = c.opws; d.workspace_bytes = c.opws_bytes;
        d.param_partials = c.gn_slot(d.B, d.HW, d.C, d.G, d.dgamma, d.dbeta);
        if (c.dry) return BD_OK;
        return bd_gn_bwd(&d, (bd_stream_t)c.st);
    }
    int gn_bwd(Ctx& c, const View& x, int64_t pg, int64_t pb, int stats_buf, const float* dy, int64_t lddy, int silu,
               const float* dx_add = nullptr, int64_t ld_add = 0, int gs = -1) const {
        bd_gn_bwd_desc d = {};
        d.dx_add = dx_add; d.ld_add = ld_add;
        if (gs >= 0 && planes(c) && gsplits[gs].want(lay_batch(c))) {
            const GSplit& e = gsplits[gs];
            d.dx_split = U16(BP(c, e.b_pl)); d.lddxs = e.C; d.dx_split_c0 = e.coff - x.coff; d.dx_split_c1 = d.dx_split_c0 + e.C;
        }
        d.dx = GP(c, x); d.lddx = x.ld; d.accumulate_dx = take_ginit(c, x.buf);
        return gn_bwd(c, d, x, pg, pb, stats_buf, dy, lddy, silu);
    }

    template <class D>
    static void conv3_geometry(D& d, const Ctx& c, const Conv3& k) {
        d.B = c.B; d.Hs = k.Hs; d.Ws = k.Ws; d.Cin = k.Cin; d.Cout = k.Cout; d.stride = k.stride; d.pad_t = k.pad; d.pad_l = k.pad; d.ups = k.ups;
        d.Ho = k.Ho; d.Wo = k.Wo;
    }
    bool ps_shape(int B, int H, int W, int Cin, int Cout) const {
        static const bool off = getenv("BD_CONV_PS") && atoi(getenv("BD_CONV_PS")) == 0;
        return !off && mode_bf16(cfg.compute_mode) && conv3x3_ps_supported(B, H, W, Cin, Cout) && conv3x3_ps_supported(B, H, W, Cout, Cin) &&
               conv3x3_ps_wgrad_supported(B, H, W, Cin, Cout);
    }
    bool ps_ok(const Ctx& c, int H, int W, int Cin, int Cout) const { return planes(c) && ps_shape(lay_batch(c), H, W, Cin, Cout); }
    bool phase_shape(int B, int H, int W, int Cin, int Cout, int classes = 4, int min_wgs = 128) const {
        const long long wgs = (long long)classes * (((long long)B * H * W + 255) / 256) * (Cout / 128);
        return mode_bf16(cfg.compute_mode) && upsample_conv_ps_supported(B, H, W, Cin, Cout) && wgs >= min_wgs;
    }
    bool phase_ok(const Ctx& c, int H, int W, int Cin, int Cout, int classes = 4, int min_wgs = 128) const {
        return planes(c) && phase_shape(lay_batch(c), H, W, Cin, Cout, classes, min_wgs);
    }
    int conv3_planes(Ctx& c, const Conv3& k, int direction, const Opnd& x, float* y, int64_t ldy, int acc, const Conv3Epi& e) const {
        bd_conv3x3_ps_desc d = {};
        d.B = c.B; d.H = k.Ho; d.W = k.Wo; d.direction = direction;
        d.K = direction > 0 ? k.Cin : k.Cout; d.N = direction > 0 ? k.Cout : k.Cin;
        d.x_split = U16(x.p); d.ldx = x.ld; d.w_split = (direction > 0 ? c.w_split : c.wT_split) + 2 * k.pw;
        if (direction > 0) d.bias = c.params + k.pb;
        d.rowbias = e.rowbias; d.ld_rowbias = e.ld_rowbias; d.residual = e.residual; d.ldr = e.ldr; d.out_scale = e.out_scale;
        d.y = y; d.ldy = ldy; d.accumulate = acc;
        d.workspace = c.opws; d.workspace_bytes = c.opws_bytes; d.mode = cfg.compute_mode;
        if (e.gn_splits > 0) {
            d.gn_part = reinterpret_cast<double*>(c.opws); d.gn_groups = cfg.norm_num_groups;
            if (c.dry) need(c, (size_t)c.B * e.gn_splits * d.gn_groups * 2 * sizeof(double));
        }
        if (c.dry) { note_conv(c); return BD_OK; }
        return conv3x3_ps(d, c.st);
    }
    int conv3_fwd(Ctx& c, const Conv3& k, bool ps, const Opnd& x, float* y, int64_t ldy, const Conv3Epi& e = Conv3Epi()) const {
        if (ps) return conv3_planes(c, k, 1, x, y, ldy, 0, e);
        bd_conv3x3_fwd_desc d = {};
        conv3_geometry(d, c, k);
        d.x = x.p; d.ldx = x.ld; d.w = c.params + k.pw; d.bias = c.params + k.pb;
        d.rowbias = e.rowbias; d.ld_rowbias = e.ld_rowbias; d.residual = e.residual; d.ldr = e.ldr; d.out_scale = e.out_scale;
        d.y = y; d.ldy = ldy;
        d.workspace = c.opws; d.workspace_bytes = c.opws_bytes; d.mode = cfg.compute_mode;
        if (c.dry) { note_conv(c); return BD_OK; }
        if (c.w_split) d.w_split = c.w_split + 2 * k.pw;
        return conv3x3_fwd(d, c.st);
    }
    int conv3_dgrad(Ctx& c, const Conv3& k, bool ps, const Opnd& dy, float* dx, int64_t lddx, int acc) const {
        if (ps) return conv3_planes(c, k, -1, dy, dx, lddx, acc, Conv3Epi());
        bd_conv3x3_dgrad_desc d = {};
        conv3_geometry(d, c, k);
        d.dy = dy.p; d.lddy = dy.ld; d.w = c.params + k.pw; d.dx = dx; d.lddx = lddx; d.accumulate = acc;
        d.workspace = c.opws; d.workspace_bytes = c.opws_bytes; d.mode = cfg.compute_mode;
        if (c.dry) { note_conv(c); return BD_OK; }
        if (c.w_split) d.w_split = c.w_split + 2 * k.pw;
        return conv3x3_dgrad(d, c.st);
    }
    int conv3_wgrad(Ctx& c, const Conv3& k, bool ps, const Opnd& x, const Opnd& dy, int bias_scratch = -1) const {
        if (!c.wg) return BD_OK;
        if (ps) {
            bd_conv3x3_ps_wgrad_desc d = {};
            d.B = c.B; d.H = k.Ho; d.W = k.Wo; d.Cin = k.Cin; d.Cout = k.Cout;
            d.x_split = U16(x.p); d.ldx = x.ld; d.dy_split = U16(dy.p); d.lddy = dy.ld;
            d.dw = c.grads + k.pw; d.db = c.grads + k.pb;
            d.workspace_bytes = c.opws_bytes; d.mode = cfg.compute_mode;
            if (c.dry) {
                note_conv(c);
                need(c, conv3x3_ps_wgrad_workspace_bytes(d));
                return BD_OK;
            }
            return on_aux(c, [&](hipStream_t st, char* ws) { d.workspace = ws; return conv3x3_ps_wgrad(d, st); });
        }
        bd_conv3x3_wgrad_desc d = {};
        conv3_geometry(d, c, k);
        d.x = x.p; d.ldx = x.ld; d.dy = dy.p; d.lddy = dy.ld; d.dw = c.grads + k.pw; d.db = c.grads + k.pb;
        if (bias_scratch >= 0 && !conv3x3_wgrad_is_thin(d)) {
            d.db = nullptr;
            BD_TRY(bias_grad(c, dy.p, dy.ld, k.Ho * k.Wo, k.Cout, bias_scratch, c.grads + k.pb));
        }
        d.workspace = c.opws; d.workspace_bytes = c.opws_bytes; d.mode = cfg.compute_mode;
        if (c.dry) { note_conv(c); return BD_OK; }
        return on_aux(c, [&](hipStream_t st, char* ws) { d.workspace = ws; return conv3x3_wgrad(d, st); });
    }
    int grad_planes(Ctx& c, int gs, const float* dy, int64_t lddy, int64_t nrows, int C, int b_scratch, Opnd& out) const {
        const bool ready = gs >= 0 && gsplits[gs].emitted;
        float* pl = BP(c, ready ? gsplits[gs].b_pl : b_scratch);
        if (!ready) BD_TRY(split_rows(c, dy, lddy, nrows, C, pl));
        out = Opnd{pl, C};
        return BD_OK;
    }

    void build();
    void node_time_embed();
    void node_conv_in(const View& y);
    void node_resnet(const std::string& pre, const View& x, const View& y, int toff, float scale);
    void node_attention(const std::string& pre, const View& x, const View& y, float scale);
    void node_downsample(const std::string& pre, const View& x, const View& y);
    void node_upsample(const std::string& pre, const View& x, const View& y);
    void node_conv_out(const View& x);
    void layout(int B, int training);
};

void bd_unet::node_time_embed() {
    const int c0 = cfg.block_out_channels[0];
    const int64_t pw1 = add_param("time_embedding.linear_1.weight", {T, c0});
    const int64_t pb1 = add_param("time_embedding.linear_1.bias", {T});
    const int64_t pw2 = add_param("time_embedding.linear_2.weight", {T, T});
    const int64_t pb2 = add_param("time_embedding.linear_2.bias", {T});
    segs[cur_seg].hi = nparams;
    nparams = (nparams + 31) / 32 * 32;
    p_tw = nparams; nparams += (int64_t)sumC * T;
    p_tb = nparams; nparams += sumC;
    const int b_tsin = new_buf(c0, 0, R_VALUE), b_e1 = new_buf(T, 0, R_VALUE), b_e1s = new_buf(T, 0, R_VALUE);
    const int b_emb = new_buf(T, 0, R_VALUE);
    b_embs = new_buf(T, 0, R_VALUE);
    b_tproj = new_buf(sumC, 0, R_VALUE);
    b_dtproj = new_buf(sumC, 0, R_GRAD);
    const int b_dembs = scratch(T), b_demb = scratch(T), b_de1s = scratch(T), b_de1 = scratch(T);
    F([=](Ctx& c) {
        if (!c.dry)
            BD_TRY(bd_timestep_embedding(c.t, c.t_stride, c.B, c0, cfg.flip_sin_to_cos, cfg.freq_shift, BP(c, b_tsin), (bd_stream_t)c.st));
        BD_TRY(linear_fwd(c, BP(c, b_tsin), c0, c.params + pw1, c.params + pb1, BP(c, b_e1), T, c.B, T, c0));
        if (!c.dry) BD_TRY(bd_silu_fwd(BP(c, b_e1), BP(c, b_e1s), (int64_t)c.B * T, (bd_stream_t)c.st));
        BD_TRY(linear_fwd(c, BP(c, b_e1s), T, c.params + pw2, c.params + pb2, BP(c, b_emb), T, c.B, T, T));
        if (!c.dry) BD_TRY(bd_silu_fwd(BP(c, b_emb), BP(c, b_embs), (int64_t)c.B * T, (bd_stream_t)c.st));
        BD_TRY(linear_fwd(c, BP(c, b_embs), T, c.params + p_tw, c.params + p_tb, BP(c, b_tproj), sumC, c.B, sumC, T));
        return (int)BD_OK;
    });
    Bk([=](Ctx& c) {
        if (!c.wg) return (int)BD_OK;
        float* dtp = BP(c, b_dtproj);
        BD_TRY(linear_dgrad(c, dtp, sumC, c.params + p_tw, BP(c, b_dembs), T, c.B, sumC, T, 0));
        if (!c.dry) BD_TRY(bd_silu_bwd(BP(c, b_emb), BP(c, b_dembs), BP(c, b_demb), (int64_t)c.B * T, 0, (bd_stream_t)c.st));
        BD_TRY(linear_wgrad(c, BP(c, b_demb), T, BP(c, b_e1s), T, c.grads + pw2, c.B, T, T, c.grads + pb2));
        BD_TRY(linear_dgrad(c, BP(c, b_demb), T, c.params + pw2, BP(c, b_de1s), T, c.B, T, T, 0));
        if (!c.dry) BD_TRY(bd_silu_bwd(BP(c, b_e1), BP(c, b_de1s), BP(c, b_de1), (int64_t)c.B * T, 0, (bd_stream_t)c.st));
        BD_TRY(linear_wgrad(c, BP(c, b_de1), T, BP(c, b_tsin), c0, c.grads + pw1, c.B, T, c0, c.grads + pb1));
        return (int)BD_OK;
    });
}

void bd_unet::node_conv_in(const View& y) {
    const int S_ = cfg.sample_size;
    const int64_t pw = add_param("conv_in.weight", {y.C, cfg.in_channels, 3, 3}, 1);
    const int64_t pb = add_param("conv_in.bias", {y.C});
    const Conv3 k = conv3_same(pw, pb, cfg.in_channels, y.C, S_, S_);
    F([=](Ctx& c) { return conv3_fwd(c, k, false, {c.x, c.ldx}, VP(c, y), y.ld); });
    Bk([=](Ctx& c) {
        const Opnd dy = {GP(c, y), y.ld};
        BD_TRY(conv3_wgrad(c, k, false, {c.x, c.ldx}, dy));
        if (!c.dx && !c.dry) return (int)BD_OK;
        return conv3_dgrad(c, k, false, dy, c.dx, c.lddx, 0);
    });
}

void bd_unet::node_resnet(const std::string& pre, const View& x, const View& y, int toff, float scale) {
    const int Cin = x.C, Cout = y.C, H = x.H, W = x.W, HW = H * W;
    const bool shortcut = Cin != Cout;
    const int64_t pn1w = add_param(pre + "norm1.weight", {Cin}), pn1b = add_param(pre + "norm1.bias", {Cin});
    const int64_t pc1w = add_param(pre + "conv1.weight", {Cout, Cin, 3, 3}, 1), pc1b = add_param(pre + "conv1.bias", {Cout});
    alias_param(pre + "time_emb_proj.weight", p_tw + (int64_t)toff * T, {Cout, T});
    alias_param(pre + "time_emb_proj.bias", p_tb + toff, {Cout});
    {
        Seg& sg = segs[cur_seg];
        const int64_t wlo = p_tw + (int64_t)toff * T, whi = wlo + (int64_t)Cout * T, blo = p_tb + toff, bhi = blo + Cout;
        if (sg.tw_lo < 0) { sg.tw_lo = wlo; sg.tw_hi = whi; sg.tb_lo = blo; sg.tb_hi = bhi; }
        else {
            if (wlo < sg.tw_lo) sg.tw_lo = wlo;
            if (whi > sg.tw_hi) sg.tw_hi = whi;
            if (blo < sg.tb_lo) sg.tb_lo = blo;
            if (bhi > sg.tb_hi) sg.tb_hi = bhi;
        }
    }
    const int b_embs_ = b_embs, T_ = T;
    const int64_t pn2w = add_param(pre + "norm2.weight", {Cout}), pn2b = add_param(pre + "norm2.bias", {Cout});
    const int64_t pc2w = add_param(pre + "conv2.weight", {Cout, Cout, 3, 3}, 1), pc2b = add_param(pre + "conv2.bias", {Cout});
    const Conv3 k1 = conv3_same(pc1w, pc1b, Cin, Cout, H, W), k2 = conv3_same(pc2w, pc2b, Cout, Cout, H, W);
    int64_t psw = -1, psb = -1;
    if (shortcut) {
        psw = add_param(pre + "conv_shortcut.weight", {Cout, Cin, 1, 1}, 1);
        psb = add_param(pre + "conv_shortcut.bias", {Cout});
    }
    if (Cin % 32 == 0 && Cout % 32 == 0) {
        wt_off.push_back(pc1w); wt_cin.push_back(Cin); wt_cout.push_back(Cout);
        wt_off.push_back(pc2w); wt_cin.push_back(Cout); wt_cout.push_back(Cout);
    }
    const int b_a1 = new_buf((int64_t)HW * Cin, 0, R_VALUE), b_h1 = new_buf((int64_t)HW * Cout, 0, R_VALUE);
    const int b_a2 = new_buf((int64_t)HW * Cout, 0, R_VALUE);
    const int b_a1s = new_buf((int64_t)HW * Cin, 0, R_VALUE), b_a2s = new_buf((int64_t)HW * Cout, 0, R_VALUE);
    const int G = cfg.norm_num_groups;
    const int b_st1 = new_buf(2 * G, 0, R_VALUE), b_st2 = new_buf(2 * G, 0, R_VALUE);
    View h1v; h1v.buf = b_h1; h1v.coff = 0; h1v.C = Cout; h1v.ld = Cout; h1v.H = H; h1v.W = W;
    bufs[b_h1].gbuf = -1;
    const int b_dys = scale != 1.f ? scratch((int64_t)HW * Cout) : -1;
    const int b_da2 = scratch((int64_t)HW * Cout), b_dh1 = scratch((int64_t)HW * Cout);
    const int b_da1 = scratch((int64_t)HW * Cin);
    const int b_dyS = scratch((int64_t)HW * Cout), b_dh1S = scratch((int64_t)HW * Cout);
    const float inv = 1.f / scale;
    const int sumC_ = sumC;
    const int gs_in = claim_gsplit(x, true);
    const int gs_out = b_dys < 0 ? reg_gsplit(y, [this, H, W, Cout](int B) { return ps_shape(B, H, W, Cout, Cout); }) : -1;

    F([=](Ctx& c) {
        const bool ps1 = ps_ok(c, H, W, Cin, Cout), ps2 = ps_ok(c, H, W, Cout, Cout);
        float* a1 = BP(c, ps1 ? b_a1s : b_a1);
        float* a2 = BP(c, ps2 ? b_a2s : b_a2);
        BD_TRY(gn_fwd(c, x, pn1w, pn1b, a1, Cin, b_st1, 1, ps1));
        Conv3Epi e1;
        e1.rowbias = BP(c, b_tproj) + toff; e1.ld_rowbias = sumC_;
        if (ps1 && ps2 && bd_gn_fwd_takes_stats(c.B, HW, Cout, G)) e1.gn_splits = bd_conv3x3_ps_gn_splits(c.B, H, W, Cin, Cout, G);
        BD_TRY(conv3_fwd(c, k1, ps1, {a1, Cin}, BP(c, b_h1), Cout, e1));
        BD_TRY(gn_fwd(c, h1v, pn2w, pn2b, a2, Cout, b_st2, 1, ps2, e1.gn_splits));
        Conv3Epi e2;
        e2.residual = VP(c, x); e2.ldr = x.ld; e2.out_scale = inv;
        if (shortcut) {
            BD_TRY(linear_fwd(c, VP(c, x), x.ld, c.params + psw, c.params + psb, VP(c, y), y.ld, (int)rows(c, x), Cout, Cin));
            e2.residual = VP(c, y); e2.ldr = y.ld;
        }
        return conv3_fwd(c, k2, ps2, {a2, Cout}, VP(c, y), y.ld, e2);
    });
    Bk([=](Ctx& c) {
        const int M = (int)rows(c, x);
        Opnd dy = {GP(c, y), y.ld};
        if (b_dys >= 0) {
            BD_TRY(add(c, dy.p, dy.ld, BP(c, b_dys), Cout, M, Cout, inv, 0));
            dy = {BP(c, b_dys), Cout};
        }
        const bool ps1 = ps_ok(c, H, W, Cin, Cout), ps2 = ps_ok(c, H, W, Cout, Cout);
        Opnd dy2 = dy;
        if (ps2) BD_TRY(grad_planes(c, gs_out, dy.p, dy.ld, M, Cout, b_dyS, dy2));
        BD_TRY(conv3_wgrad(c, k2, ps2, {BP(c, ps2 ? b_a2s : b_a2), Cout}, dy2));
        BD_TRY(conv3_dgrad(c, k2, ps2, dy2, BP(c, b_da2), Cout, 0));
        float* dh1 = BP(c, ps1 ? b_dh1S : b_dh1);
        {
            bd_gn_bwd_desc d = {};
            d.lddx = Cout;
            if (ps1) { d.dx_split = U16(dh1); d.lddxs = Cout; }
            else d.dx = dh1;
            d.dx_colsum = BP(c, b_dtproj) + toff; d.ld_colsum = sumC_;
            BD_TRY(gn_bwd(c, d, h1v, pn2w, pn2b, b_st2, BP(c, b_da2), Cout, 1));
        }
        if (c.dry) BD_TRY(linear_wgrad(c, BP(c, b_dtproj), sumC_, BP(c, b_embs_), T_, c.grads, c.B, sumC_, T_, c.grads));
        BD_TRY(conv3_wgrad(c, k1, ps1, {BP(c, ps1 ? b_a1s : b_a1), Cin}, {dh1, Cout}));
        BD_TRY(conv3_dgrad(c, k1, ps1, {dh1, Cout}, BP(c, b_da1), Cin, 0));
        if (shortcut) {
            BD_TRY(linear_wgrad(c, dy.p, dy.ld, VP(c, x), x.ld, c.grads + psw, M, Cout, Cin, c.grads + psb));
            const int acc = take_ginit(c, x.buf);
            static const bool sc_sp = !(getenv("BD_SHORTCUT_SP") && atoi(getenv("BD_SHORTCUT_SP")) == 0);
            if (sc_sp && ps2 && gemm_sp_supported(M, Cin, Cout) && x.ld % 4 == 0) {
                bd_gemm_sp_desc g = {};
                g.M = M; g.N = Cin; g.K = Cout; g.batch = 1;
                g.a = U16(dy2.p); g.lda = Cout;
                g.b = c.w_split + 2 * psw; g.ldb = Cin; g.b_kmajor = 1;
                g.c = GP(c, x); g.ldc = x.ld; g.accumulate = acc; g.alpha = 1.f; g.out_scale = 1.f;
                BD_TRY(gemm_s(c, g));
            } else {
                BD_TRY(linear_dgrad(c, dy.p, dy.ld, c.params + psw, GP(c, x), x.ld, M, Cout, Cin, acc));
            }
        }
        return gn_bwd(c, x, pn1w, pn1b, b_st1, BP(c, b_da1), Cin, 1, shortcut ? nullptr : dy.p, dy.ld, gs_in);
    });
}

void bd_unet::node_attention(const std::string& pre, const View& x, const View& y, float scale) {
    const int C = x.C, H = x.H, W = x.W, N = H * W;
    const int heads = cfg.attention_head_dim > 0 ? C / cfg.attention_head_dim : 1;
    const int dh = C / heads;
    const float sm_scale = 1.0f / std::sqrt((float)C / (float)heads);
    const int64_t pgw = add_param(pre + "group_norm.weight", {C}), pgb = add_param(pre + "group_norm.bias", {C});
    const int64_t pqw = add_param(pre + "query.weight", {C, C});
    add_param(pre + "key.weight", {C, C});
    add_param(pre + "value.weight", {C, C});
    const int64_t pqb = add_param(pre + "query.bias", {C});
    add_param(pre + "key.bias", {C});
    add_param(pre + "value.bias", {C});
    const int64_t ppw = add_param(pre + "proj_attn.weight", {C, C}), ppb = add_param(pre + "proj_attn.bias", {C});
    const int G = cfg.norm_num_groups;
    const int b_n = new_buf((int64_t)N * C, 0, R_VALUE), b_qkv = new_buf((int64_t)N * 3 * C, 0, R_VALUE);
    const int b_p = new_buf((int64_t)heads * N * N, 0, R_VALUE), b_o = new_buf((int64_t)N * C, 0, R_VALUE);
    const int b_st = new_buf(2 * G, 0, R_VALUE);
    const int b_dys = scale != 1.f ? scratch((int64_t)N * C) : -1;
    const int b_do = scratch((int64_t)N * C), b_dp = scratch((int64_t)heads * N * N);
    const int b_dqkv = scratch((int64_t)N * 3 * C), b_dn = scratch((int64_t)N * C);
    const int b_dyS = scratch((int64_t)N * C);
    const float inv = 1.f / scale;

    auto batched = [=](bd_igemm_desc& g, int B) {
        g.batch_outer = B; g.batch_inner = heads;
    };
    auto sp_shape = [=](int B) {
        return mode_bf16(cfg.compute_mode) && attn_sp_supported(N, dh) && gemm_sp_supported((int)((int64_t)B * N), C, C) &&
               gemm_sp_supported(3 * C, C, 32);
    };
    auto use_sp = [=](const Ctx& c) { return planes(c) && sp_shape(lay_batch(c)); };
    const int gs_in = claim_gsplit(x, true);
    const int gs_out = b_dys < 0 ? reg_gsplit(y, sp_shape) : -1;
    F([=](Ctx& c) {
        const int M = (int)rows(c, x);
        const bool sp = use_sp(c);
        BD_TRY(gn_fwd(c, x, pgw, pgb, BP(c, b_n), C, b_st, 0, sp));
        if (sp) {
            bd_gemm_sp_desc q = {};
            q.M = M; q.N = 3 * C; q.K = C; q.batch = 1;
            q.a = U16(BP(c, b_n)); q.lda = C; q.b = c.w_split + 2 * pqw; q.ldb = C;
            q.c_split = U16(BP(c, b_qkv)); q.ldcs = 3 * C; q.bias = c.params + pqb; q.alpha = 1.f; q.out_scale = 1.f;
            BD_TRY(gemm_s(c, q));
            if (!c.dry) {
                bd_attn_sp_desc a = {};
                a.B = c.B; a.heads = heads; a.N = N; a.dh = dh; a.qkv_split = U16(BP(c, b_qkv)); a.ld = 3 * C; a.scale = sm_scale;
                a.o_split = U16(BP(c, b_o)); a.ldo = C; a.pt_split = c.training ? U16(BP(c, b_p)) : nullptr; a.mode = cfg.compute_mode;
                BD_TRY(attn_sp_fwd(a, c.st));
            }
            bd_gemm_sp_desc o = {};
            o.M = M; o.N = C; o.K = C; o.batch = 1;
            o.a = U16(BP(c, b_o)); o.lda = C; o.b = c.w_split + 2 * ppw; o.ldb = C;
            o.c = VP(c, y); o.ldc = y.ld; o.bias = c.params + ppb; o.residual = VP(c, x); o.ldr = x.ld; o.alpha = 1.f; o.out_scale = inv;
            return gemm_s(c, o);
        }
        BD_TRY(linear_fwd(c, BP(c, b_n), C, c.params + pqw, c.params + pqb, BP(c, b_qkv), 3 * C, M, 3 * C, C));
        float* qkv = BP(c, b_qkv);
        {
            {
                bd_igemm_desc g = {};
                g.A = dense(qkv, 3 * C, 1); g.A.bs_outer = (int64_t)N * 3 * C; g.A.bs_inner = dh;
                g.B = dense(qkv + C, 3 * C, 1); g.B.bs_outer = (int64_t)N * 3 * C; g.B.bs_inner = dh;
                g.M = N; g.N = N; g.K = dh; batched(g, c.B);
                g.C = BP(c, b_p); g.ldc = N; g.c_bs_outer = (int64_t)heads * N * N; g.c_bs_inner = (int64_t)N * N;
                g.alpha = sm_scale; g.out_scale = 1.f;
                BD_TRY(igemm(c, g));
            }
            if (!c.dry) BD_TRY(bd_softmax_fwd(BP(c, b_p), BP(c, b_p), (int64_t)c.B * heads * N, N, (bd_stream_t)c.st));
            {
                bd_igemm_desc g = {};
                g.A = dense(BP(c, b_p), N, 1); g.A.bs_outer = (int64_t)heads * N * N; g.A.bs_inner = (int64_t)N * N;
                g.B = dense(qkv + 2 * C, 3 * C, 0); g.B.bs_outer = (int64_t)N * 3 * C; g.B.bs_inner = dh;
                g.M = N; g.N = dh; g.K = N; batched(g, c.B);
                g.C = BP(c, b_o); g.ldc = C; g.c_bs_outer = (int64_t)N * C; g.c_bs_inner = dh;
                g.alpha = 1.f; g.out_scale = 1.f;
                BD_TRY(igemm(c, g));
            }
        }
        return linear_fwd(c, BP(c, b_o), C, c.params + ppw, c.params + ppb, VP(c, y), y.ld, M, C, C, VP(c, x), x.ld, inv);
    });
    Bk([=](Ctx& c) {
        const int M = (int)rows(c, x);
        const float* dy = GP(c, y); int64_t lddy = y.ld;
        if (b_dys >= 0) {
            BD_TRY(add(c, dy, lddy, BP(c, b_dys), C, M, C, inv, 0));
            dy = BP(c, b_dys); lddy = C;
        }
        if (use_sp(c)) {
            Opnd dyS;
            BD_TRY(grad_planes(c, gs_out, dy, lddy, M, C, b_dyS, dyS));
            bd_gemm_sp_desc w = {};
            w.M = C; w.N = C; w.K = M; w.batch = 1;
            w.a = U16(dyS.p); w.lda = C; w.a_kmajor = 1; w.b = U16(BP(c, b_o)); w.ldb = C; w.b_kmajor = 1;
            w.c = c.grads + ppw; w.ldc = C; w.a_colsum = c.grads + ppb; w.alpha = 1.f; w.out_scale = 1.f;
            BD_TRY(gemm_s(c, w, true));
            bd_gemm_sp_desc g = {};
            g.M = M; g.N = C; g.K = C; g.batch = 1;
            g.a = U16(dyS.p); g.lda = C; g.b = c.w_split + 2 * ppw; g.ldb = C; g.b_kmajor = 1;
            g.c_split = U16(BP(c, b_do)); g.ldcs = C; g.alpha = 1.f; g.out_scale = 1.f;
            BD_TRY(gemm_s(c, g));
            if (!c.dry) {
                bd_attn_sp_desc a = {};
                a.B = c.B; a.heads = heads; a.N = N; a.dh = dh; a.qkv_split = U16(BP(c, b_qkv)); a.ld = 3 * C; a.scale = sm_scale;
                a.pt_split = U16(BP(c, b_p)); a.do_split = U16(BP(c, b_do)); a.lddo = C; a.dst_split = U16(BP(c, b_dp));
                a.dqkv_split = U16(BP(c, b_dqkv)); a.lddqkv = 3 * C; a.mode = cfg.compute_mode;
                BD_TRY(attn_sp_bwd(a, c.st));
            }
            bd_gemm_sp_desc wq = {};
            wq.M = 3 * C; wq.N = C; wq.K = M; wq.batch = 1;
            wq.a = U16(BP(c, b_dqkv)); wq.lda = 3 * C; wq.a_kmajor = 1; wq.b = U16(BP(c, b_n)); wq.ldb = C; wq.b_kmajor = 1;
            wq.c = c.grads + pqw; wq.ldc = C; wq.a_colsum = c.grads + pqb; wq.alpha = 1.f; wq.out_scale = 1.f;
            BD_TRY(gemm_s(c, wq, true));
            bd_gemm_sp_desc dn = {};
            dn.M = M; dn.N = C; dn.K = 3 * C; dn.batch = 1;
            dn.a = U16(BP(c, b_dqkv)); dn.lda = 3 * C; dn.b = c.w_split + 2 * pqw; dn.ldb = C; dn.b_kmajor = 1;
            dn.c = BP(c, b_dn); dn.ldc = C; dn.alpha = 1.f; dn.out_scale = 1.f;
            BD_TRY(gemm_s(c, dn));
            return gn_bwd(c, x, pgw, pgb, b_st, BP(c, b_dn), C, 0, dy, lddy, gs_in);
        }
        float* qkv = BP(c, b_qkv); float* dqkv = BP(c, b_dqkv); float* P = BP(c, b_p); float* dP = BP(c, b_dp);
        float* dO = BP(c, b_do);
        BD_TRY(linear_wgrad(c, dy, lddy, BP(c, b_o), C, c.grads + ppw, M, C, C, c.grads + ppb));
        BD_TRY(linear_dgrad(c, dy, lddy, c.params + ppw, dO, C, M, C, C, 0));
        {
            bd_igemm_desc g = {};
            g.A = dense(dO, C, 1); g.A.bs_outer = (int64_t)N * C; g.A.bs_inner = dh;
            g.B = dense(qkv + 2 * C, 3 * C, 1); g.B.bs_outer = (int64_t)N * 3 * C; g.B.bs_inner = dh;
            g.M = N; g.N = N; g.K = dh; batched(g, c.B);
            g.C = dP; g.ldc = N; g.c_bs_outer = (int64_t)heads * N * N; g.c_bs_inner = (int64_t)N * N;
            g.alpha = 1.f; g.out_scale = 1.f;
            BD_TRY(igemm(c, g));
        }
        {
            bd_igemm_desc g = {};
            g.A = dense(P, N, 0); g.A.bs_outer = (int64_t)heads * N * N; g.A.bs_inner = (int64_t)N * N;
            g.B = dense(dO, C, 0); g.B.bs_outer = (int64_t)N * C; g.B.bs_inner = dh;
            g.M = N; g.N = dh; g.K = N; batched(g, c.B);
            g.C = dqkv + 2 * C; g.ldc = 3 * C; g.c_bs_outer = (int64_t)N * 3 * C; g.c_bs_inner = dh;
            g.alpha = 1.f; g.out_scale = 1.f;
            BD_TRY(igemm(c, g));
        }
        if (!c.dry) BD_TRY(bd_softmax_bwd(P, dP, dP, (int64_t)c.B * heads * N, N, (bd_stream_t)c.st));
        {
            bd_igemm_desc g = {};
            g.A = dense(dP, N, 1); g.A.bs_outer = (int64_t)heads * N * N; g.A.bs_inner = (int64_t)N * N;
            g.B = dense(qkv + C, 3 * C, 0); g.B.bs_outer = (int64_t)N * 3 * C; g.B.bs_inner = dh;
            g.M = N; g.N = dh; g.K = N; batched(g, c.B);
            g.C = dqkv; g.ldc = 3 * C; g.c_bs_outer = (int64_t)N * 3 * C; g.c_bs_inner = dh;
            g.alpha = sm_scale; g.out_scale = 1.f;
            BD_TRY(igemm(c, g));
// ... 145 lines not shown
            if (i != n - 1) { res /= 2; skips.push_back({boc[i], res}); }
        }
    }
    struct UpRes { int C1, C2, Cout, H; };
    std::vector<std::vector<UpRes>> ups(n);
    {
        int sk = (int)skips.size();
        int res = S0 >> (n - 1);
        for (int i = 0; i < n; ++i) {
            const int out = boc[n - 1 - i];
            const int prev = i == 0 ? boc[n - 1] : boc[n - i];
            for (int j = 0; j <= L; ++j) {
                const Skip& s = skips[--sk];
                ups[i].push_back({j == 0 ? prev : out, s.C, out, res});
            }
            if (i != n - 1) res *= 2;
        }
    }
    sumC = 0;
    for (int i = 0; i < n; ++i) sumC += L * boc[i];
    sumC += 2 * boc[n - 1];
    for (int i = 0; i < n; ++i) for (auto& u : ups[i]) sumC += u.Cout;

    const int nseg = 2 * n + 4;
    segs.assign(nseg, Seg{-1, -1});
    const int seg_out = 0;
    auto seg_up = [&](int i) { return 1 + (n - 1 - i); };
    const int seg_mid = n + 1;
    auto seg_down = [&](int i) { return n + 2 + (n - 1 - i); };
    const int seg_in = 2 * n + 2, seg_time = 2 * n + 3;

    std::vector<std::vector<View>> cat(n);
    for (int i = 0; i < n; ++i)
        for (auto& u : ups[i]) {
            View v = new_tensor(u.H, u.H, u.C1 + u.C2);
            cat[i].push_back(v);
        }
    std::vector<View> skipv(skips.size());
    {
        int sk = (int)skips.size();
        for (int i = 0; i < n; ++i)
            for (size_t j = 0; j < ups[i].size(); ++j) {
                --sk;
                skipv[sk] = slice(cat[i][j], ups[i][j].C1, ups[i][j].C2);
            }
    }

    cur_group = 0;
    cur_seg = seg_time; segs[seg_time].lo = 0;
    node_time_embed();
    int toff = 0, group = 1;
    cur_seg = seg_in; cur_group = group++;
    node_conv_in(skipv[0]);
    int sk = 1;
    View h = skipv[0];
    int res = S0;
    for (int i = 0; i < n; ++i) {
        cur_seg = seg_down(i);
        const std::string bp = "down_blocks." + std::to_string(i) + ".";
        for (int j = 0; j < L; ++j) {
            cur_group = group++;
            View dst = skipv[sk];
            if (cfg.down_attn[i]) {
                View mid = new_tensor(res, res, boc[i]);
                node_resnet(bp + "resnets." + std::to_string(j) + ".", h, mid, toff, 1.f);
                cur_group = group++;
                node_attention(bp + "attentions." + std::to_string(j) + ".", mid, dst, 1.f);
            } else {
                node_resnet(bp + "resnets." + std::to_string(j) + ".", h, dst, toff, 1.f);
            }
            toff += boc[i];
            h = dst; ++sk;
        }
        if (i != n - 1) {
            cur_group = group++;
            View dst = skipv[sk];
            node_downsample(bp + "downsamplers.0.", h, dst);
            h = dst; ++sk; res /= 2;
        }
    }
    {
        cur_seg = seg_mid;
        const int C = boc[n - 1];
        const float s = cfg.mid_block_scale_factor;
        View m1 = new_tensor(res, res, C), m2 = new_tensor(res, res, C);
        View dst = slice(cat[0][0], 0, ups[0][0].C1);
        cur_group = group++;
        node_resnet("mid_block.resnets.0.", h, m1, toff, s); toff += C;
        cur_group = group++;
        node_attention("mid_block.attentions.0.", m1, m2, s);
        cur_group = group++;
        node_resnet("mid_block.resnets.1.", m2, dst, toff, s); toff += C;
    }
    View last;
    for (int i = 0; i < n; ++i) {
        cur_seg = seg_up(i);
        const std::string bp = "up_blocks." + std::to_string(i) + ".";
        const int nl = (int)ups[i].size();
        for (int j = 0; j < nl; ++j) {
            const UpRes& u = ups[i][j];
            View dst;
            const bool last_layer = j == nl - 1;
            if (!last_layer) dst = slice(cat[i][j + 1], 0, ups[i][j + 1].C1);
            else dst = new_tensor(u.H, u.H, u.Cout);
            cur_group = group++;
            if (cfg.up_attn[i]) {
                View mid = new_tensor(u.H, u.H, u.Cout);
                node_resnet(bp + "resnets." + std::to_string(j) + ".", cat[i][j], mid, toff, 1.f);
                cur_group = group++;
                node_attention(bp + "attentions." + std::to_string(j) + ".", mid, dst, 1.f);
            } else {
                node_resnet(bp + "resnets." + std::to_string(j) + ".", cat[i][j], dst, toff, 1.f);
            }
            toff += u.Cout;
            last = dst;
        }
        if (i != n - 1) {
            cur_group = group++;
            View dst = slice(cat[i + 1][0], 0, ups[i + 1][0].C1);
            node_upsample(bp + "upsamplers.0.", last, dst);
        }
    }
    cur_seg = seg_out; cur_group = group++;
    node_conv_out(last);
    nparams = (nparams + 3) / 4 * 4;
}

void bd_unet::layout(int B, int training) {
    if (lay_B == B && lay_train == training && lay_gen == bd::g_tune_gen) return;
    auto al = [](int64_t x) { return (x + 63) / 64 * 64; };
    int64_t v = 0, g = 0;
    for (auto& b : bufs) if (b.region == R_VALUE) { b.off = v; if (!b.live || b.live(B, training)) v += al(b.per_sample * B + b.fixed); }
    value_floats = v;
    for (auto& b : bufs) if (b.region == R_GRAD) { b.off = v + g; if (!b.live || b.live(B, training)) g += al(b.per_sample * B + b.fixed); }
    grad_floats = training ? g : 0;
    const int64_t base = value_floats + grad_floats;
    int64_t smax = 0;
    for (int pass = 0; pass < 2; ++pass) {
        int cur = -1; int64_t s = 0;
        for (auto& b : bufs) if (b.region == R_SCRATCH) {
            if (b.group != cur) { cur = b.group; s = 0; }
            const int64_t n = al(b.per_sample * B + b.fixed);
            if (pass == 0) { if (s + n > smax) smax = s + n; }
            else b.off = base + (b.group & 1) * smax + s;
            s += n;
        }
    }
    scratch_floats = training ? 2 * smax : 0;
    Ctx c;
    c.dry = true; c.B = B; c.ws = nullptr; c.ginit.assign(bufs.size(), 0);
    c.opws_bytes = (size_t)1 << 62;
    for (auto& f : fwd) f(c);
    if (training) for (auto it = bwd.rbegin(); it != bwd.rend(); ++it) it->fn(c);
    opws_bytes = align_up(c.opws_need, 256);
    gnpart_floats = training ? c.gnpart_need : 0;
    lay_B = B; lay_train = training; lay_gen = bd::g_tune_gen;
    prep_params = nullptr; prep_ws = nullptr; prep_B = -1;
}

extern "C" int bd_unet_create(const bd_unet_config* cfg, bd_unet** out) {
    BD_CHECK(cfg && out, BD_ERR_INVALID, "bd_unet_create: null argument");
    const int n = cfg->num_blocks;
    BD_CHECK(n >= 1 && n <= 8, BD_ERR_INVALID, "bd_unet_create: num_blocks %d out of range", n);
    BD_CHECK(cfg->layers_per_block >= 1, BD_ERR_INVALID, "bd_unet_create: layers_per_block");
    BD_CHECK(cfg->sample_size > 0 && (cfg->sample_size % (1 << (n - 1))) == 0, BD_ERR_INVALID,
             "bd_unet_create: sample_size %d not divisible by 2^%d", cfg->sample_size, n - 1);
    BD_CHECK(cfg->in_channels > 0 && cfg->out_channels > 0, BD_ERR_INVALID, "bd_unet_create: channels");
    BD_CHECK(cfg->norm_num_groups > 0, BD_ERR_INVALID, "bd_unet_create: norm_num_groups");
    for (int i = 0; i < n; ++i) {
        const int C = cfg->block_out_channels[i];
        BD_CHECK(C > 0 && C % cfg->norm_num_groups == 0 && C % 4 == 0, BD_ERR_UNSUPPORTED,
                 "bd_unet_create: block_out_channels[%d]=%d must be a multiple of norm_num_groups and of 4", i, C);
        if (cfg->attention_head_dim > 0 && (cfg->down_attn[i] || cfg->up_attn[n - 1 - i]))
            BD_CHECK(C % cfg->attention_head_dim == 0 && cfg->attention_head_dim % 4 == 0, BD_ERR_UNSUPPORTED,
                     "bd_unet_create: attention_head_dim %d must divide %d and be a multiple of 4", cfg->attention_head_dim, C);
    }
    BD_CHECK(cfg->mid_block_scale_factor != 0.f, BD_ERR_INVALID, "bd_unet_create: mid_block_scale_factor == 0");
    BD_CHECK(mode_valid(cfg->compute_mode), BD_ERR_INVALID, "bd_unet_create: compute_mode %d", cfg->compute_mode);
    bd_unet* u = new (std::nothrow) bd_unet();
    BD_CHECK(u, BD_ERR_INVALID, "bd_unet_create: out of host memory");
    u->cfg = *cfg;
    u->build();
    *out = u;
    return BD_OK;
}
extern "C" void bd_unet_destroy(bd_unet* u) {
    if (!u) return;
    if (u->aux_stream) {
        (void)hipStreamSynchronize(u->aux_stream);
        (void)hipEventDestroy(u->aux_ev_fork);
        (void)hipEventDestroy(u->aux_ev_join[0]);
        (void)hipEventDestroy(u->aux_ev_join[1]);
        (void)hipEventDestroy(u->aux_ev_seg);
        (void)hipStreamDestroy(u->aux_stream);
    }
    delete u;
}
extern "C" int bd_unet_set_aux_stream(bd_unet* u, int enabled) {
    BD_CHECK(u, BD_ERR_INVALID, "bd_unet_set_aux_stream: null plan");
    u->aux_enabled = enabled ? 1 : 0;
    return BD_OK;
}
extern "C" int bd_unet_set_deferred_join(bd_unet* u, int enabled) {
    BD_CHECK(u, BD_ERR_INVALID, "bd_unet_set_deferred_join: null plan");
    u->aux_defer = enabled ? 1 : 0;
    return BD_OK;
}
extern "C" int bd_unet_stream_wait_aux(bd_unet* u, bd_stream_t stream) {
    BD_CHECK(u, BD_ERR_INVALID, "bd_unet_stream_wait_aux: null plan");
    if (!u->aux_stream || !u->aux_ev_seg) return BD_OK;
    BD_HIP_TRY(hipStreamWaitEvent(S(stream), u->aux_ev_seg, 0));
    return BD_OK;
}
extern "C" int bd_unet_set_static_weights(bd_unet* u, int enabled) {
    BD_CHECK(u, BD_ERR_INVALID, "bd_unet_set_static_weights: null plan");
    u->static_weights = enabled ? 1 : 0;
    u->prep_params = nullptr; u->prep_ws = nullptr; u->prep_B = -1;
    return BD_OK;
}
extern "C" int bd_unet_set_compute_mode(bd_unet* u, int mode) {
    BD_CHECK(u && mode_valid(mode), BD_ERR_INVALID, "bd_unet_set_compute_mode: bad arguments (mode %d)", mode);
    if (u->cfg.compute_mode != mode) {
        u->lay_B = -1;
        u->prep_params = nullptr; u->prep_ws = nullptr; u->prep_B = -1;
    }
    u->cfg.compute_mode = mode;
    return BD_OK;
}
extern "C" int bd_unet_reset_static_cache(bd_unet* u) {
    BD_CHECK(u, BD_ERR_INVALID, "bd_unet_reset_static_cache: null plan");
    u->prep_params = nullptr; u->prep_ws = nullptr; u->prep_B = -1;
    return BD_OK;
}
extern "C" int64_t bd_unet_num_params(const bd_unet* u) { return u ? u->nparams : 0; }
extern "C" int bd_unet_num_tensors(const bd_unet* u) { return u ? (int)u->params.size() : 0; }
extern "C" int bd_unet_param_info(const bd_unet* u, int i, const char** name, int64_t* offset, int* rank, int64_t shape[4],
                                  int* layout) {
    BD_CHECK(u && i >= 0 && i < (int)u->params.size(), BD_ERR_INVALID, "bd_unet_param_info: index out of range");
    const Param& p = u->params[i];
    if (name) *name = p.name.c_str();
    if (offset) *offset = p.off;
    if (rank) *rank = p.rank;
    if (shape) for (int k = 0; k < 4; ++k) shape[k] = p.shape[k];
    if (layout) *layout = p.layout;
    return BD_OK;
}
static size_t wsplit_elems(const bd_unet* u) { return (size_t)(u->nparams / 32 * 32); }
static size_t wsplit_bytes(const bd_unet* u) { return align_up(wsplit_elems(u) * 2 * sizeof(uint16_t), 256); }

extern "C" size_t bd_unet_workspace_bytes(bd_unet* u, int B, int training) {
    if (!u || B <= 0) return 0;
    u->layout(B, training);
    return (size_t)(u->value_floats + u->grad_floats + u->scratch_floats) * sizeof(float) + u->opws_bytes + 256 +
           2 * wsplit_bytes(u) + align_up(u->opws_bytes, 256) +
           align_up(u->gnpart_floats * sizeof(float), 256);
}

static int unet_ctx(bd_unet* u, Ctx& c, int B, int training, void* workspace, size_t workspace_bytes) {
    BD_CHECK(u, BD_ERR_INVALID, "bd_unet: null plan");
    BD_CHECK(B > 0, BD_ERR_INVALID, "bd_unet: B must be > 0");
    const size_t need = bd_unet_workspace_bytes(u, B, training);
    BD_CHECK(workspace && workspace_bytes >= need, BD_ERR_WORKSPACE, "bd_unet: workspace %zu < %zu bytes", workspace_bytes, need);
    BD_CHECK(aligned16(workspace), BD_ERR_INVALID, "bd_unet: workspace must be 16-byte aligned");
    c.B = B; c.LB = B;
    c.ws = reinterpret_cast<float*>(workspace);
    const size_t fl = (size_t)(u->value_floats + u->grad_floats + u->scratch_floats) * sizeof(float);
    c.opws = reinterpret_cast<char*>(workspace) + align_up(fl, 256);
    c.opws_bytes = u->opws_bytes;
    if (mode_bf16(u->cfg.compute_mode)) {
        c.w_split = reinterpret_cast<const uint16_t*>(c.opws + align_up(u->opws_bytes, 256));
    }
    c.opws2 = c.opws + align_up(u->opws_bytes, 256) + 2 * wsplit_bytes(u);
    c.gnpart = u->gnpart_floats ? reinterpret_cast<float*>(c.opws2 + align_up(u->opws_bytes, 256)) : nullptr;
    c.gnpart_floats = u->gnpart_floats; c.gnpart_used = 0;
    if (c.w_split) c.wT_split = reinterpret_cast<const uint16_t*>(c.opws + align_up(u->opws_bytes, 256) + wsplit_bytes(u));
    c.ginit.assign(u->bufs.size(), 0);
    return BD_OK;
}

static int unet_aux_init(bd_unet* u) {
    if (u->aux_stream) return BD_OK;
    int lo = 0, hi = 0;
    BD_HIP_TRY(hipDeviceGetStreamPriorityRange(&lo, &hi));
    BD_HIP_TRY(hipStreamCreateWithPriority(&u->aux_stream, hipStreamNonBlocking, lo));
    BD_HIP_TRY(hipEventCreateWithFlags(&u->aux_ev_fork, hipEventDisableTiming));
    BD_HIP_TRY(hipEventCreateWithFlags(&u->aux_ev_join[0], hipEventDisableTiming));
    BD_HIP_TRY(hipEventCreateWithFlags(&u->aux_ev_join[1], hipEventDisableTiming));
    BD_HIP_TRY(hipEventCreateWithFlags(&u->aux_ev_seg, hipEventDisableTiming));
    return BD_OK;
}

extern "C" int bd_unet_forward(bd_unet* u, int B, int training, const float* params, const float* x, int64_t ldx,
                               const int64_t* t, int t_stride, float* out, int64_t ldo, void* workspace, size_t workspace_bytes,
                               bd_stream_t stream) {
    Ctx c;
    BD_TRY(unet_ctx(u, c, B, training, workspace, workspace_bytes));
    BD_CHECK(params && x && t && out, BD_ERR_INVALID, "bd_unet_forward: null pointer");
    BD_CHECK(ldx >= u->cfg.in_channels && ldo >= u->cfg.out_channels, BD_ERR_INVALID, "bd_unet_forward: ld < channels");
    BD_CHECK(aligned16(params), BD_ERR_INVALID, "bd_unet_forward: params must be 16-byte aligned");
    c.params = params; c.x = x; c.ldx = ldx; c.t = t; c.t_stride = t_stride; c.out = out; c.ldo = ldo; c.st = S(stream);
    c.training = training != 0;
    if (training) { u->fwd_gen = bd::g_tune_gen; u->fwd_B = B; u->fwd_ws = workspace; }
    const bool prepared = u->static_weights && !training && u->prep_params == (const void*)params && u->prep_ws == workspace && u->prep_B == B;
    if (c.w_split && !prepared) {
        BD_TRY(bd_split_bf16(params, (int64_t)wsplit_elems(u), const_cast<uint16_t*>(c.w_split), stream));
        for (const auto& uw : u->upsw)
            if (u->phase_ok(c, uw.H, uw.W, uw.C, uw.C))
                BD_TRY(upsample_weights(params + uw.pw, uw.C, uw.C, bd_unet::U16(u->BP(c, uw.b_e)),
                                        training ? bd_unet::U16(u->BP(c, uw.b_et)) : nullptr, c.st));
        u->prep_params = u->static_weights && !training ? (const void*)params : nullptr; u->prep_ws = workspace; u->prep_B = B;
    }
    auto transpose_weights = [&](hipStream_t st) -> int {
        if (!training || !c.wT_split || u->wt_off.empty()) return BD_OK;
        return split_wt_batched(params, const_cast<uint16_t*>(c.wT_split), u->wt_off.data(), u->wt_cin.data(), u->wt_cout.data(),
                                (int)u->wt_off.size(), st);
    };
    static const long long pipes_min_px = getenv("BD_FWD_PIPES_MINPX") ? atoll(getenv("BD_FWD_PIPES_MINPX")) : 32768;
    if (!u->aux_enabled || B < 2 || (long long)B * u->cfg.sample_size * u->cfg.sample_size < pipes_min_px) {
        BD_TRY(transpose_weights(c.st));
        for (auto& f : u->fwd) BD_TRY(f(c));
        return BD_OK;
    }
    BD_TRY(unet_aux_init(u));
    Ctx c2 = c;
    const int Bh = B / 2;
    const int64_t hw = (int64_t)u->cfg.sample_size * u->cfg.sample_size;
    c.B = Bh;
    c2.B = B - Bh; c2.s0 = Bh; c2.st = u->aux_stream; c2.opws = c.opws2;
    c2.x = x + (int64_t)Bh * hw * ldx; c2.t = t + (int64_t)Bh * t_stride; c2.out = out + (int64_t)Bh * hw * ldo;
    BD_HIP_TRY(hipEventRecord(u->aux_ev_fork, c.st));
    BD_HIP_TRY(hipStreamWaitEvent(c2.st, u->aux_ev_fork, 0));
    BD_TRY(transpose_weights(c2.st));
    for (auto& f : u->fwd) {
        BD_TRY(f(c));
        BD_TRY(f(c2));
    }
    BD_HIP_TRY(hipEventRecord(u->aux_ev_join[0], c2.st));
    BD_HIP_TRY(hipStreamWaitEvent(c.st, u->aux_ev_join[0], 0));
    return BD_OK;
}

extern "C" int bd_unet_num_segments(const bd_unet* u) { return u ? (int)u->segs.size() : 0; }
extern "C" int bd_unet_segment_num_ranges(const bd_unet* u, int seg) {
    if (!u || seg < 0 || seg >= (int)u->segs.size()) return 0;
    return u->segs[seg].tw_lo >= 0 ? 3 : 1;
}
extern "C" int bd_unet_segment_range_k(const bd_unet* u, int seg, int k, int64_t* lo, int64_t* hi) {
    BD_CHECK(u && seg >= 0 && seg < (int)u->segs.size() && k >= 0 && k < bd_unet_segment_num_ranges(u, seg), BD_ERR_INVALID,
             "bd_unet_segment_range_k: segment / range out of range");
    const bd_unet::Seg& s = u->segs[seg];
    const int64_t l = k == 0 ? s.lo : (k == 1 ? s.tw_lo : s.tb_lo), h = k == 0 ? s.hi : (k == 1 ? s.tw_hi : s.tb_hi);
    if (lo) *lo = l;
    if (hi) *hi = h;
    return BD_OK;
}
extern "C" int bd_unet_segment_range(const bd_unet* u, int seg, int64_t* lo, int64_t* hi) {
    BD_CHECK(u && seg >= 0 && seg < (int)u->segs.size(), BD_ERR_INVALID, "bd_unet_segment_range: segment out of range");
    if (lo) *lo = u->segs[seg].lo;
    if (hi) *hi = u->segs[seg].hi;
    return BD_OK;
}

static int unet_backward_run(bd_unet* u, int seg, int B, const float* params, const float* x, int64_t ldx, const float* dout, int64_t lddo,
                             float* grads, bool need_grads, float* dx, int64_t lddx, void* workspace, size_t workspace_bytes,
                             bd_stream_t stream, int64_t* ready_lo, int64_t* ready_hi) {
    Ctx c;
    BD_CHECK(!u || u->fwd_ws != workspace || u->fwd_B != B || u->fwd_gen == bd::g_tune_gen, BD_ERR_INVALID,
             "bd_unet_backward: bd_tune_set was called between the training forward and its backward (the saved activations would move)");
    BD_TRY(unet_ctx(u, c, B, 1, workspace, workspace_bytes));
    BD_CHECK(params && x && dout && (grads || !need_grads), BD_ERR_INVALID, "bd_unet_backward: null pointer");
    BD_CHECK(aligned16(params) && aligned16(grads), BD_ERR_INVALID, "bd_unet_backward: params/grads must be 16-byte aligned");
    BD_CHECK(seg >= -1 && seg < (int)u->segs.size(), BD_ERR_INVALID, "bd_unet_backward: segment %d out of range", seg);
    c.params = params; c.grads = grads; c.dout = dout; c.lddo = lddo; c.st = S(stream);
    c.x = x; c.ldx = ldx;
    c.wg = grads != nullptr; c.dx = dx; c.lddx = lddx;
    const bool aux_on = u->aux_enabled && c.wg;
    const bool defer = aux_on && u->aux_defer && seg >= 0 && seg + 1 < (int)u->segs.size();
    if (!aux_on && !c.wg && u->aux_stream && (u->aux_pend[0] || u->aux_pend[1])) {
        BD_HIP_TRY(hipStreamWaitEvent(c.st, u->aux_ev_seg, 0));
        u->aux_pend[0] = u->aux_pend[1] = false;
    }
    if (aux_on) {
        BD_TRY(unet_aux_init(u));
        c.st2 = u->aux_stream; c.ev_fork = u->aux_ev_fork; c.ev_join[0] = u->aux_ev_join[0]; c.ev_join[1] = u->aux_ev_join[1];
        if (seg > 0 && u->aux_defer) { c.pend[0] = u->aux_pend[0]; c.pend[1] = u->aux_pend[1]; }
        else if (u->aux_pend[0] || u->aux_pend[1]) {
            BD_HIP_TRY(hipStreamWaitEvent(c.st, u->aux_ev_seg, 0));
            u->aux_pend[0] = u->aux_pend[1] = false;
        }
    }
    for (auto it = u->bwd.rbegin(); it != u->bwd.rend(); ++it) {
        if (seg >= 0 && it->seg > seg) break;
        const bool run = seg < 0 || it->seg == seg;
        const bool keep = c.dry;
        c.dry = !run;
        const int par = it->group & 1;
        if (run) BD_TRY(bd_unet::aux_wait(c, par));
        int s = it->fn(c);
        c.dry = keep;
        if (s != BD_OK) return s;
        if (run) BD_TRY(bd_unet::aux_mark(c, par));
    }
    if (!c.gn_items.empty()) BD_TRY(bd_gn_bwd_params(c.gn_items.data(), (int)c.gn_items.size(), c.B, (bd_stream_t)c.st));
    {
        int64_t lo = -1, hi = -1;
        for (int sg = 0; sg < (int)u->segs.size(); ++sg) {
            if (seg >= 0 && sg != seg) continue;
            const bd_unet::Seg& q = u->segs[sg];
            if (q.tb_lo < 0) continue;
            if (lo < 0 || q.tb_lo - u->p_tb < lo) lo = q.tb_lo - u->p_tb;
            if (q.tb_hi - u->p_tb > hi) hi = q.tb_hi - u->p_tb;
        }
        if (lo >= 0) {
            BD_TRY(u->linear_wgrad(c, u->BP(c, u->b_dtproj) + lo, u->sumC, u->BP(c, u->b_embs), u->T, c.grads + u->p_tw + lo * u->T, c.B,
                                   (int)(hi - lo), u->T, c.grads + u->p_tb + lo));
            BD_TRY(bd_unet::aux_mark(c, 0));
        }
    }
    if (defer) {
        u->aux_pend[0] = c.pend[0]; u->aux_pend[1] = c.pend[1];
        BD_HIP_TRY(hipEventRecord(u->aux_ev_seg, c.st2));
// ... 38 lines not shown
```

include/bd_hip.h:

```cpp
#ifndef BD_HIP_H
#define BD_HIP_H

#include <stddef.h>
#include <stdint.h>

#ifdef __cplusplus
extern "C" {
#endif

typedef void* bd_stream_t;

enum bd_status {
    BD_OK = 0,
    BD_ERR_INVALID = -1,
    BD_ERR_UNSUPPORTED = -2,
    BD_ERR_LAUNCH = -3,
    BD_ERR_WORKSPACE = -4
};

const char* bd_last_error(void);
int bd_version(void);

typedef struct {
    int B, C, H, W;
    const float* images_f32;
    const uint8_t* images_u8;
    const uint8_t* is_poison;
    const float* trigger;
    const float* target_img;
    const float* noise;
    const int64_t* timesteps;
    const float* alphas;
    const float* alphas_cumprod;
    float vmin;
    float* x_noisy; int64_t ld_noisy;
    float* target;  int64_t ld_target;
    float* R_out;
    float* x0_out;
    int64_t* mask_out;
    float* image_out;
    const int64_t* row_index;
    const uint8_t* flip;
} bd_poison_qsample_desc;
int bd_poison_qsample(const bd_poison_qsample_desc* d, bd_stream_t stream);

typedef struct {
    int B, C, H, W;
    const float* x0; const float* R; const float* noise;
    const int64_t* timesteps; const float* alphas; const float* alphas_cumprod;
    float* x_noisy; int64_t ld_noisy;
    float* target;  int64_t ld_target;
} bd_qsample_desc;
int bd_qsample(const bd_qsample_desc* d, bd_stream_t stream);

int bd_nchw_to_nhwc(const float* src, float* dst, int B, int C, int H, int W, int64_t ld, bd_stream_t stream);
int bd_nhwc_to_nchw(const float* src, int64_t ld, float* dst, int B, int C, int H, int W, bd_stream_t stream);

typedef struct {
    int64_t n;
    const float* model_output; const float* sample; const float* noise;
    float* prev_sample; float* pred_original;
    const float* alphas_cumprod;
    int t, prev_t;
    int variance_type;
    int clip_sample; float clip_sample_range;
    int clip_defense; float clip_defense_range;
} bd_ddpm_step_desc;
int bd_ddpm_step(const bd_ddpm_step_desc* d, bd_stream_t stream);

typedef struct {
    int64_t n;
    const float* model_output; const float* sample; const float* noise;
    float* prev_sample; float* pred_original;
    const float* alphas_cumprod;
    int t, prev_t; float final_alpha_cumprod; float eta;
    int clip_sample; float clip_sample_range;
} bd_ddim_step_desc;
int bd_ddim_step(const bd_ddim_step_desc* d, bd_stream_t stream);

#define BD_LINCOMB_MAX 6
int bd_lincomb(int k, const float* const* terms, const float* coeffs, int64_t n, int clip, float clip_range, float* out,
               bd_stream_t stream);

int bd_anp_apply(const float* params, int64_t nparams, const float* pert_w, const float* pert_b, const int64_t* items, int n_items,
                 int64_t total_rows, float* eff, bd_stream_t stream);
int bd_anp_grad(const float* params, const float* grad_eff, const int64_t* items, int n_items, int64_t total_rows, const float* pert_w,
                float* grad_w, float* grad_b, float* row_norm, bd_stream_t stream);

int bd_to_image(const float* x, int src_is_nhwc, int64_t ld, int B, int C, int H, int W,
                float* out_f32, uint8_t* out_u8, bd_stream_t stream);

int bd_timestep_embedding(const int64_t* t, int t_stride, int B, int dim, int flip_sin_to_cos,
                          float freq_shift, float* out, bd_stream_t stream);

typedef struct {
    int B, HW, C, G; float eps; int silu;
    const float* x; int64_t ldx;
    const float* gamma; const float* beta;
    float* y; int64_t ldy;
    float* mean; float* rstd;
    void* workspace; size_t workspace_bytes;
    uint16_t* y_split; int64_t ldys;
    const double* stats; int stats_splits;
} bd_gn_fwd_desc;
size_t bd_gn_workspace_bytes(int B, int C);
int bd_gn_fwd_takes_stats(int B, int HW, int C, int G);
int bd_gn_fwd(const bd_gn_fwd_desc* d, bd_stream_t stream);

typedef struct {
    int B, HW, C, G; int silu;
    const float* x; int64_t ldx;
    const float* gamma; const float* beta;
    const float* mean; const float* rstd;
    const float* dy; int64_t lddy;
    float* dx; int64_t lddx; int accumulate_dx;
    float* dgamma; float* dbeta;
    void* workspace; size_t workspace_bytes;
    float* dx_colsum; int64_t ld_colsum;
    uint16_t* dx_split; int64_t lddxs;
    const float* dx_add; int64_t ld_add;
    float* param_partials;
    int dx_split_c0, dx_split_c1;
} bd_gn_bwd_desc;
int bd_gn_bwd(const bd_gn_bwd_desc* d, bd_stream_t stream);
int bd_gn_bwd_defers(int B, int HW, int C, int G);
typedef struct {
    const float* partials;
    int C;
    float* dgamma; float* dbeta;
} bd_gn_param_item;
int bd_gn_bwd_params(const bd_gn_param_item* items, int n, int B, bd_stream_t stream);

enum bd_compute_mode { BD_MODE_F32 = 0, BD_MODE_BF16X3 = 1, BD_MODE_BF16 = 2 };

enum bd_operand_kind {
    BD_OPK_DENSE = 0,
    BD_OPK_CONV = 1,
    BD_OPK_TCONV = 2,
    BD_OPK_WGT = 3
};
typedef struct {
    int kind;
    int kc;
    const float* p; int64_t ld;
    int64_t bs_outer, bs_inner;
    int C, Hs, Ws, Ho, Wo, stride, pad_t, pad_l, ups;
    const uint16_t* split;
} bd_operand;
typedef struct {
    bd_operand A, B;
    int M, N, K;
    int batch_outer, batch_inner;
    float* C; int64_t ldc; int64_t c_bs_outer, c_bs_inner;
    float alpha; float out_scale;
    const float* bias;
    const float* rowbias; int64_t ld_rowbias; int rows_per_group;
    const float* residual; int64_t ldr;
    int accumulate;
    int ksplit;
    void* workspace; size_t workspace_bytes;
    int tile;
    int mode;
    float* a_colsum;
} bd_igemm_desc;
size_t bd_igemm_workspace_bytes(const bd_igemm_desc* d);
int bd_split_bf16(const float* src, int64_t n, uint16_t* out, bd_stream_t stream);
int bd_igemm(const bd_igemm_desc* d, bd_stream_t stream);

typedef struct {
    int B, Hs, Ws, Cin, Cout, stride, pad_t, pad_l, ups;
    int Ho, Wo;
    const float* x; int64_t ldx;
    const float* w;
    const float* bias;
    const float* rowbias; int64_t ld_rowbias;
    const float* residual; int64_t ldr;
    float out_scale;
    float* y; int64_t ldy;
    void* workspace; size_t workspace_bytes;
    int mode;
    const uint16_t* w_split;
} bd_conv3x3_fwd_desc;
int bd_conv3x3_fwd(const bd_conv3x3_fwd_desc* d, bd_stream_t stream);

typedef struct {
    int B, Hs, Ws, Cin, Cout, stride, pad_t, pad_l, ups, Ho, Wo;
    const float* dy; int64_t lddy;
    const float* w;
    float* dx; int64_t lddx; int accumulate;
    void* workspace; size_t workspace_bytes;
    int mode;
    const uint16_t* w_split;
} bd_conv3x3_dgrad_desc;
int bd_conv3x3_dgrad(const bd_conv3x3_dgrad_desc* d, bd_stream_t stream);

typedef struct {
    int B, Hs, Ws, Cin, Cout, stride, pad_t, pad_l, ups, Ho, Wo;
    const float* x; int64_t ldx;
    const float* dy; int64_t lddy;
    float* dw;
    void* workspace; size_t workspace_bytes;
    int mode;
    float* db;
} bd_conv3x3_wgrad_desc;
int bd_conv3x3_wgrad(const bd_conv3x3_wgrad_desc* d, bd_stream_t stream);
size_t bd_conv3x3_workspace_bytes(int B, int Ho, int Wo, int Hs, int Ws, int Cin, int Cout, int ups);

int bd_split_rows(const float* src, int64_t ld_src, int64_t rows, int C, uint16_t* dst, int64_t ld_dst, bd_stream_t stream);
int bd_split_rows_ups2(const float* src, int64_t ld_src, int B, int H, int W, int C, uint16_t* dst, int64_t ld_dst, bd_stream_t stream);
int bd_split_wt(const float* w, int Cin, int Cout, uint16_t* out, bd_stream_t stream);
typedef struct {
    int B, H, W;
    int K, N;
    int direction;
    const uint16_t* x_split; int64_t ldx;
    const uint16_t* w_split;
    const float* bias;
    const float* rowbias; int64_t ld_rowbias;
    const float* residual; int64_t ldr;
    float out_scale;
    float* y; int64_t ldy; int accumulate;
    void* workspace; size_t workspace_bytes;
    double* gn_part; int gn_groups;
    int mode;
} bd_conv3x3_ps_desc;
size_t bd_conv3x3_ps_workspace_bytes(const bd_conv3x3_ps_desc* d);
int bd_conv3x3_ps_gn_splits(int B, int H, int W, int K, int N, int groups);
int bd_conv3x3_ps(const bd_conv3x3_ps_desc* d, bd_stream_t stream);
typedef struct {
    int B, H, W, Cin, Cout;
    const uint16_t* x_split; int64_t ldx;
    const uint16_t* dy_split; int64_t lddy;
    float* dw; float* db;
    void* workspace; size_t workspace_bytes;
    int mode;
} bd_conv3x3_ps_wgrad_desc;
int bd_tune_set(const char* key, int value);
size_t bd_conv3x3_ps_wgrad_workspace_bytes(const bd_conv3x3_ps_wgrad_desc* d);
int bd_conv3x3_ps_wgrad(const bd_conv3x3_ps_wgrad_desc* d, bd_stream_t stream);

int bd_colsum(const float* x, int64_t ldx, int64_t rows, int N, int64_t rows_per_group, float* out,
              int64_t ld_out, int accumulate, bd_stream_t stream);
int bd_sum2x2(const float* du, int64_t ldu, float* dx, int64_t lddx, int B, int H, int W, int C,
              int accumulate, bd_stream_t stream);

int bd_softmax_fwd(const float* s, float* p, int64_t rows, int n, bd_stream_t stream);
int bd_softmax_bwd(const float* p, const float* dp, float* ds, int64_t rows, int n, bd_stream_t stream);

int bd_silu_fwd(const float* x, float* y, int64_t n, bd_stream_t stream);
int bd_silu_bwd(const float* x, const float* dy, float* dx, int64_t n, int accumulate, bd_stream_t stream);

size_t bd_reduce_workspace_bytes(void);
int bd_loss_fwd_bwd(const float* pred, int64_t ldp, const float* target, int64_t ldt, int64_t rows, int C,
                    int loss_type, float grad_scale, float* loss, float* dpred, int64_t lddp,
                    void* workspace, bd_stream_t stream);

size_t bd_ssim_workspace_bytes(int N, int C, int H, int W);
int bd_ssim(const float* preds, const float* target, int N, int C, int H, int W, int64_t stride_n, int64_t stride_c,
            int64_t stride_h, int64_t stride_w, float data_range, float* out, void* workspace, size_t workspace_bytes,
            bd_stream_t stream);

typedef struct {
    const float* x; int64_t ldx;
    const float* w;
    const float* bias;
    float* y; int64_t ldy;
    int B, H, W, Cin, Cout, KH, KW, stride_h, stride_w, pad_h, pad_w;
    int relu;
    int w_kc;
} bd_conv2d_desc;
int bd_conv2d_nhwc(const bd_conv2d_desc* d, bd_stream_t stream);
int bd_pool2d_nhwc(const float* x, int64_t ldx, float* y, int64_t ldy, int B, int H, int W, int C, int kernel, int stride, int pad,
                   int mode, int count_include_pad, bd_stream_t stream);
int bd_resize_bilinear_nhwc(const void* x, int x_is_u8, float* y, int B, int H, int W, int C, int Ho, int Wo, float scale, float shift,
                            bd_stream_t stream);
int bd_global_avgpool_nhwc(const float* x, int64_t ldx, float* y, int B, int HW, int C, bd_stream_t stream);


int bd_sumsq(const float* g, int64_t n, double* sumsq, void* workspace, bd_stream_t stream);
int bd_adam_clip(float* p, const float* g, float* m, float* v, int64_t n, const double* sumsq,
                 double max_norm, double lr, double b1, double b2, double eps, int step, float* grad_norm_out,
                 bd_stream_t stream);

typedef struct {
    int sample_size, in_channels, out_channels;
    int num_blocks;
    int block_out_channels[8];
    int down_attn[8];
    int up_attn[8];
    int layers_per_block;
    int downsample_padding;
    int flip_sin_to_cos; float freq_shift;
    float norm_eps; int norm_num_groups;
    int attention_head_dim;
    float mid_block_scale_factor;
    int compute_mode;
} bd_unet_config;

typedef struct bd_unet bd_unet;
int bd_unet_create(const bd_unet_config* cfg, bd_unet** out);
void bd_unet_destroy(bd_unet* u);
int bd_unet_set_compute_mode(bd_unet* u, int mode);
int64_t bd_unet_num_params(const bd_unet* u);
int bd_unet_num_tensors(const bd_unet* u);
int bd_unet_param_info(const bd_unet* u, int i, const char** name, int64_t* offset, int* rank,
                       int64_t shape[4], int* layout);
size_t bd_unet_workspace_bytes(bd_unet* u, int B, int training);
int bd_unet_forward(bd_unet* u, int B, int training, const float* params, const float* x, int64_t ldx,
                    const int64_t* t, int t_stride, float* out, int64_t ldo,
                    void* workspace, size_t workspace_bytes, bd_stream_t stream);
int bd_unet_backward(bd_unet* u, int B, const float* params, const float* x, int64_t ldx,
                     const float* dout, int64_t lddo, float* grads, void* workspace, size_t workspace_bytes,
                     bd_stream_t stream);
int bd_unet_backward_input(bd_unet* u, int B, const float* params, const float* x, int64_t ldx,
                           const float* dout, int64_t lddo, float* grads, float* dx, int64_t lddx,
                           void* workspace, size_t workspace_bytes, bd_stream_t stream);
int bd_unet_set_aux_stream(bd_unet* u, int enabled);
int bd_unet_set_static_weights(bd_unet* u, int enabled);
int bd_unet_reset_static_cache(bd_unet* u);
int bd_unet_num_segments(const bd_unet* u);
int bd_unet_segment_range(const bd_unet* u, int seg, int64_t* lo, int64_t* hi);
int bd_unet_segment_num_ranges(const bd_unet* u, int seg);
int bd_unet_segment_range_k(const bd_unet* u, int seg, int k, int64_t* lo, int64_t* hi);
int bd_unet_set_deferred_join(bd_unet* u, int enabled);
int bd_unet_stream_wait_aux(bd_unet* u, bd_stream_t stream);
int bd_unet_backward_segment(bd_unet* u, int seg, int B, const float* params, const float* x, int64_t ldx,
                             const float* dout, int64_t lddo, float* grads, void* workspace, size_t workspace_bytes,
                             bd_stream_t stream, int64_t* ready_lo, int64_t* ready_hi);

int bd_prof_enable(int on);
int bd_prof_enabled(void);
int bd_prof_reset(void);
int bd_prof_num_classes(void);
int bd_prof_get(int cls, const char** name, int64_t* launches, double* total_ms, double* flops, double* bytes);

typedef struct {
    int B, H, W, Cin, Cout;
    const uint16_t* x_split; int64_t ldx;
    const uint16_t* dy_split; int64_t lddy;
    const uint16_t* e_split;
    const uint16_t* et_split;
    const float* bias;
    float* y; int64_t ldy;
    float* dx; int64_t lddx; int accumulate;
    float* dw; float* db;
    void* workspace; size_t workspace_bytes;
    int mode;
} bd_upsample_conv_desc;
int bd_upsample_weights(const float* w , int Cin, int Cout, uint16_t* e_split, uint16_t* et_split ,
                        bd_stream_t stream);
int bd_upsample_conv_fwd(const bd_upsample_conv_desc* d, bd_stream_t stream);
int bd_upsample_conv_dgrad(const bd_upsample_conv_desc* d, bd_stream_t stream);
int bd_upsample_conv_wgrad(const bd_upsample_conv_desc* d, bd_stream_t stream);
size_t bd_upsample_conv_wgrad_workspace_bytes(const bd_upsample_conv_desc* d);
size_t bd_upsample_conv_dgrad_workspace_bytes(const bd_upsample_conv_desc* d);

typedef struct {
    int B, Ho, Wo, Cin, Cout, pad;
    const uint16_t* dy_split; int64_t lddy;
    const uint16_t* wT_split;
    float* dx; int64_t lddx; int accumulate;
    int mode;
} bd_conv3x3_s2_dgrad_desc;
int bd_conv3x3_s2_dgrad_ps(const bd_conv3x3_s2_dgrad_desc* d, bd_stream_t stream);

typedef struct {
    int M, N, K, batch;
    const uint16_t* a; int64_t lda, a_bs; int a_kmajor;
    const uint16_t* b; int64_t ldb, b_bs; int b_kmajor;
    float* c; int64_t ldc, c_bs;
    uint16_t* c_split; int64_t ldcs, cs_bs;
    const float* bias;
    const float* residual; int64_t ldr, r_bs;
    float alpha, out_scale;
    int accumulate;
    float* a_colsum;
    void* workspace; size_t workspace_bytes;
    int mode;
} bd_gemm_sp_desc;
size_t bd_gemm_sp_workspace_bytes(const bd_gemm_sp_desc* d);
// ... 30 lines not shown
```

Before: 7082 images/s.

## Fold split-K conv partial sums into the consuming GroupNorm kernels

When the small-shape planar 3x3 conv uses split-K, it no longer launches its reduce kernel. It leaves the per-split fp32 slabs in a dedicated workspace region. The following GroupNorm forward (plus bias and rowbias, optionally writing the folded activation) or GroupNorm backward (dy) sums those slabs while loading. This saves a kernel launch and a full write and re-read of the conv output, at the cost of extra workspace and more register pressure in the GN kernels, and it only applies to shapes with no residual, no accumulate and out_scale 1.

After: 7095 images/s, median of 6. No clear change (+0.2%).

```diff
diff --git a/baddiffusion_amd/_lib.py b/baddiffusion_amd/_lib.py
--- a/baddiffusion_amd/_lib.py
+++ b/baddiffusion_amd/_lib.py
@@ -39,7 +39,9 @@
     _fields_ = [("B", i32), ("HW", i32), ("C", i32), ("G", i32), ("eps", f32), ("silu", i32),
                 ("x", vp), ("ldx", i64), ("gamma", vp), ("beta", vp), ("y", vp), ("ldy", i64),
                 ("mean", vp), ("rstd", vp), ("workspace", vp), ("workspace_bytes", sz),
-                ("y_split", vp), ("ldys", i64), ("stats", vp), ("stats_splits", i32)]
+                ("y_split", vp), ("ldys", i64), ("stats", vp), ("stats_splits", i32),
+                ("x_partials", vp), ("x_nsplit", i32), ("x_split_stride", i64), ("x_bias", vp),
+                ("x_rowbias", vp), ("ld_x_rowbias", i64), ("x_out", vp), ("ldxo", i64)]
 
 
 class GnBwdDesc(C.Structure):
@@ -48,7 +50,8 @@
                 ("dy", vp), ("lddy", i64), ("dx", vp), ("lddx", i64), ("accumulate_dx", i32),
                 ("dgamma", vp), ("dbeta", vp), ("workspace", vp), ("workspace_bytes", sz),
                 ("dx_colsum", vp), ("ld_colsum", i64), ("dx_split", vp), ("lddxs", i64),
-                ("dx_add", vp), ("ld_add", i64), ("param_partials", vp), ("dx_split_c0", i32), ("dx_split_c1", i32)]
+                ("dx_add", vp), ("ld_add", i64), ("param_partials", vp), ("dx_split_c0", i32), ("dx_split_c1", i32),
+                ("dy_partials", vp), ("dy_nsplit", i32), ("dy_split_stride", i64)]
 
 
 class GnParamItem(C.Structure):
@@ -98,7 +101,8 @@
     _fields_ = [("B", i32), ("H", i32), ("W", i32), ("K", i32), ("N", i32), ("direction", i32),
                 ("x_split", vp), ("ldx", i64), ("w_split", vp), ("bias", vp), ("rowbias", vp), ("ld_rowbias", i64),
                 ("residual", vp), ("ldr", i64), ("out_scale", f32), ("y", vp), ("ldy", i64), ("accumulate", i32),
-                ("workspace", vp), ("workspace_bytes", sz), ("gn_part", vp), ("gn_groups", i32), ("mode", i32)]
+                ("workspace", vp), ("workspace_bytes", sz), ("gn_part", vp), ("gn_groups", i32), ("mode", i32),
+                ("defer_fold", i32)]
 
 
 class ConvPsWgradDesc(C.Structure):
@@ -181,6 +185,7 @@
     "bd_conv3x3_ps": (i32, [C.POINTER(ConvPsDesc), vp]),
     "bd_conv3x3_ps_workspace_bytes": (sz, [C.POINTER(ConvPsDesc)]),
     "bd_conv3x3_ps_gn_splits": (i32, [i32, i32, i32, i32, i32, i32]),
+    "bd_conv3x3_ps_ksplit": (i32, [i32, i32, i32, i32, i32]),
     "bd_upsample_weights": (i32, [vp, i32, i32, vp, vp, vp]),
     "bd_upsample_conv_fwd": (i32, [C.POINTER(UpsampleConvDesc), vp]),
     "bd_upsample_conv_dgrad": (i32, [C.POINTER(UpsampleConvDesc), vp]),
diff --git a/baddiffusion_amd/csrc/conv_ps.hip b/baddiffusion_amd/csrc/conv_ps.hip
--- a/baddiffusion_amd/csrc/conv_ps.hip
+++ b/baddiffusion_amd/csrc/conv_ps.hip
@@ -1207,6 +1207,15 @@
     int ks, cps;
     ps_small_split(M, d.N, d.K, ks, cps);
     return ks > 1 ? (size_t)ks * (size_t)M * d.N * sizeof(float) : 0;
+}
+
+int conv3x3_ps_ksplit(int B, int H, int W, int K, int N) {
+    if (!conv3x3_ps_supported(B, H, W, K, N)) return 0;
+    const long long M = (long long)B * H * W;
+    if (ps_large(M, N)) return 0;
+    int ks, cps;
+    ps_small_split(M, N, K, ks, cps);
+    return ks;
 }
 
 static bool ps_takes_v3(int B, int H, int W, int N) {
@@ -1249,6 +1258,8 @@
     p.C = d.K; p.H = d.H; p.W = d.W; p.lw = ilog2x(d.W); p.lhw = ilog2x(d.W) + ilog2x(d.H);
     p.sign = d.direction; p.M = (int)M; p.N = d.N;
     p.out_scale = d.out_scale == 0.f ? 1.f : d.out_scale; p.accumulate = d.accumulate;
+    BD_CHECK(!d.defer_fold || (!d.residual && !d.accumulate && p.out_scale == 1.f), BD_ERR_UNSUPPORTED,
+             "conv3x3_ps: defer_fold with residual, accumulate or out_scale != 1 (the consuming GroupNorm folds slabs + bias + rowbias only)");
     const bool large = ps_large(M, d.N);
     int rec = -1;
     if (prof_on()) {
@@ -1316,7 +1327,7 @@
         }
 #undef PS128_LAUNCH
         BD_LAUNCH_CHECK("conv_ps128");
-        if (pp.ksplit > 1) {
+        if (pp.ksplit > 1 && !d.defer_fold) {
             hipLaunchKernelGGL(conv_ps128_reduce, dim3((unsigned)cdiv(M * (d.N / 4), 256)), dim3(256), 0, st, pp);
             BD_LAUNCH_CHECK("conv_ps128_reduce");
         }
@@ -1479,6 +1490,7 @@
 }
 extern "C" size_t bd_conv3x3_ps_workspace_bytes(const bd_conv3x3_ps_desc* d) { return d ? bd::conv3x3_ps_workspace_bytes(*d) : 0; }
 extern "C" int bd_conv3x3_ps_gn_splits(int B, int H, int W, int K, int N, int groups) { return bd::conv3x3_ps_gn_splits(B, H, W, K, N, groups); }
+extern "C" int bd_conv3x3_ps_ksplit(int B, int H, int W, int K, int N) { return bd::conv3x3_ps_ksplit(B, H, W, K, N); }
 extern "C" int bd_conv3x3_ps(const bd_conv3x3_ps_desc* d, bd_stream_t s) {
     BD_CHECK(d, BD_ERR_INVALID, "bd_conv3x3_ps: null descriptor");
     return bd::conv3x3_ps(*d, bd::S(s));
diff --git a/baddiffusion_amd/csrc/groupnorm.hip b/baddiffusion_amd/csrc/groupnorm.hip
--- a/baddiffusion_amd/csrc/groupnorm.hip
+++ b/baddiffusion_amd/csrc/groupnorm.hip
@@ -473,13 +473,39 @@
     *mean = m; *rstd = r;
 }
 
-template <int EMAX, int NT>
+struct GnFold {
+    const float* part; int nsplit; long long stride;
+    const float* bias; const float* rowbias; long long ld_rowbias;
+    float* out; long long ldo;
+};
+template <int EMAX>
+__device__ __forceinline__ void gn_fold_load(float4 (&v)[EMAX], const GnFold& f, const float* p0, long long ld, int prow, int R, int E, int HW,
+                                             bool active) {
+    constexpr int kSlabs = EMAX <= 4 ? 4 : 1;
+#pragma unroll
+    for (int i = 0; i < EMAX; ++i) {
+        const int p = prow + R * i;
+        v[i] = gn_ld4_if(p0 + (long long)p * ld, active && i < E && p < HW);
+    }
+#pragma unroll kSlabs
+    for (int s = 1; s < f.nsplit; ++s) {
+        const float* ps = p0 + (long long)s * f.stride;
+#pragma unroll
+        for (int i = 0; i < EMAX; ++i) {
+            const int p = prow + R * i;
+            const float4 t = gn_ld4_if(ps + (long long)p * ld, active && i < E && p < HW);
+            v[i].x += t.x; v[i].y += t.y; v[i].z += t.z; v[i].w += t.w;
+        }
+    }
+}
+
+template <int EMAX, int NT, bool FOLD>
 __global__ __launch_bounds__(NT, NT == 256 ? 4 : 2) void gn_fwd_res_kernel(const float* __restrict__ x, long long ldx, float* __restrict__ y,
                                                        long long ldy, int HW, int C, int G, int cb, int q, int R, int E,
                                                        float eps, const float* __restrict__ gamma,
                                                        const float* __restrict__ beta, float* __restrict__ mean,
                                                        float* __restrict__ rstd, int silu, unsigned short* __restrict__ ys,
-                                                       long long ldys) {
+                                                       long long ldys, GnFold f) {
     __shared__ double shd[4 * NT];
     float* sh = reinterpret_cast<float*>(shd);
     __shared__ float st[2 * 256];
@@ -492,11 +518,39 @@
     const float* xb = x + (long long)b * HW * ldx + c0 + cq * 4;
     float4 v[EMAX];
     float sm[4] = {0.f, 0.f, 0.f, 0.f}, sq[4] = {0.f, 0.f, 0.f, 0.f};
+    if constexpr (FOLD) {
+        const long long eo = (long long)b * HW * ldx + c0 + cq * 4;
+        gn_fold_load<EMAX>(v, f, f.part + eo, ldx, prow, R, E, HW, active);
+        if (f.bias) {
+            const float4 t = *reinterpret_cast<const float4*>(f.bias + c0 + cq * 4);
+#pragma unroll
+            for (int i = 0; i < EMAX; ++i) {
+                const bool ok = active && i < E && prow + R * i < HW;
+                v[i].x = ok ? v[i].x + t.x : 0.f; v[i].y = ok ? v[i].y + t.y : 0.f; v[i].z = ok ? v[i].z + t.z : 0.f; v[i].w = ok ? v[i].w + t.w : 0.f;
+            }
+        }
+        if (f.rowbias) {
+            const float4 t = *reinterpret_cast<const float4*>(f.rowbias + (long long)b * f.ld_rowbias + c0 + cq * 4);
+#pragma unroll
+            for (int i = 0; i < EMAX; ++i) {
+                const bool ok = active && i < E && prow + R * i < HW;
+                v[i].x = ok ? v[i].x + t.x : 0.f; v[i].y = ok ? v[i].y + t.y : 0.f; v[i].z = ok ? v[i].z + t.z : 0.f; v[i].w = ok ? v[i].w + t.w : 0.f;
+            }
+        }
+        if (f.out) {
+            float* xo = f.out + (long long)b * HW * f.ldo + c0 + cq * 4;
+#pragma unroll
+            for (int i = 0; i < EMAX; ++i) {
+                const int p = prow + R * i;
+                if (active && i < E && p < HW) *reinterpret_cast<float4*>(xo + (long long)p * f.ldo) = v[i];
+            }
+        }
+    }
 #pragma unroll
     for (int i = 0; i < EMAX; ++i) {
         const int p = prow + R * i;
         const bool ok = active && i < E && p < HW;
-        v[i] = gn_ld4_if(xb + (long long)p * ldx, ok);
+        if constexpr (!FOLD) v[i] = gn_ld4_if(xb + (long long)p * ldx, ok);
         sm[0] += v[i].x; sm[1] += v[i].y; sm[2] += v[i].z; sm[3] += v[i].w;
         sq[0] += v[i].x * v[i].x; sq[1] += v[i].y * v[i].y; sq[2] += v[i].z * v[i].z; sq[3] += v[i].w * v[i].w;
     }
@@ -582,7 +636,7 @@
     }
 }
 
-template <int EMAX, int NT>
+template <int EMAX, int NT, bool FOLD>
 __global__ __launch_bounds__(NT) void gn_bwd_res_kernel(const float* __restrict__ x, long long ldx,
                                                        const float* __restrict__ dy, long long lddy, float* __restrict__ dx,
                                                        long long lddx, int HW, int C, int G, int cb, int q, int R, int E,
@@ -591,7 +645,7 @@
                                                        int silu, int acc, float* __restrict__ part,
                                                        float* __restrict__ dx_colsum, long long ld_colsum,
                                                        unsigned short* __restrict__ dxs, long long lddxs,
-                                                       const float* __restrict__ addp, long long ldadd, int dxs_c0, int dxs_c1) {
+                                                       const float* __restrict__ addp, long long ldadd, int dxs_c0, int dxs_c1, GnFold f) {
     __shared__ float sh[3 * 4 * NT];
     __shared__ float ch[3 * 4 * NT];
     __shared__ float sg[2 * 256];
@@ -618,8 +672,9 @@
         const int p = prow + R * i;
         const bool ok = active && i < E && p < HW;
         xh[i] = gn_ld4_if(xb + (long long)p * ldx, ok);
-        dz[i] = gn_ld4_if(db + (long long)p * lddy, ok);
-    }
+        if constexpr (!FOLD) dz[i] = gn_ld4_if(db + (long long)p * lddy, ok);
+    }
+    if constexpr (FOLD) gn_fold_load<EMAX>(dz, f, f.part + (long long)b * HW * lddy + c0 + cq * 4, lddy, prow, R, E, HW, active);
 #pragma unroll
     for (int i = 0; i < EMAX; ++i) {
         const int p = prow + R * i;
@@ -783,20 +838,35 @@
     BD_CHECK(!d->y_split || (d->C % 32 == 0 && d->ldys % 32 == 0 && ((uintptr_t)d->y_split & 127) == 0), BD_ERR_UNSUPPORTED,
              "bd_gn_fwd: y_split needs C %% 32 == 0, ldys %% 32 == 0 and a 128-byte aligned base");
     GnRes rp;
-    if (gn_resident_plan(d->B, d->HW, d->C, d->G, rp)) {
+    const bool resident = gn_resident_plan(d->B, d->HW, d->C, d->G, rp);
+    GnFold fold = {};
+    if (d->x_partials) {
+        BD_CHECK(resident, BD_ERR_UNSUPPORTED, "bd_gn_fwd: x_partials on a shape the single-pass kernels do not take (bd_gn_fwd_takes_stats() != 0)");
+        BD_CHECK(d->x_nsplit >= 1 && d->x_split_stride >= 0, BD_ERR_INVALID, "bd_gn_fwd: x_partials needs x_nsplit >= 1 and a stride");
+        BD_CHECK(aligned16(d->x_partials) && (d->x_split_stride & 3) == 0 && aligned16(d->x_bias) && aligned16(d->x_rowbias) &&
+                     (d->ld_x_rowbias & 3) == 0 && aligned16(d->x_out) && (d->ldxo & 3) == 0, BD_ERR_UNSUPPORTED,
+                 "bd_gn_fwd: x_partials / x_bias / x_rowbias / x_out must be 16B aligned, their strides multiples of 4");
+        fold.part = d->x_partials; fold.nsplit = d->x_nsplit; fold.stride = (long long)d->x_split_stride;
+        fold.bias = d->x_bias; fold.rowbias = d->x_rowbias; fold.ld_rowbias = (long long)d->ld_x_rowbias;
+        fold.out = d->x_out; fold.ldo = (long long)d->ldxo;
+    }
+    if (resident) {
         const dim3 grid((unsigned)rp.nblk * (unsigned)d->B);
         int rec = -1;
         if (prof_on())
-            rec = prof_begin("gn_fwd_res", 0.0, (double)d->B * d->HW * d->C * 4.0 * (1.0 + (d->y ? 1.0 : 0.0) + (d->y_split ? 1.0 : 0.0)), S(stream));
-#define BD_GN_FWD_RES(EM, NT)                                                                                              \
-    hipLaunchKernelGGL((gn_fwd_res_kernel<EM, NT>), grid, dim3(NT), 0, S(stream), d->x, (long long)d->ldx, d->y,             \
+            rec = prof_begin("gn_fwd_res", 0.0, (double)d->B * d->HW * d->C * 4.0 * ((fold.part ? (double)fold.nsplit + (fold.out ? 1.0 : 0.0) : 1.0) +
+                             (d->y ? 1.0 : 0.0) + (d->y_split ? 1.0 : 0.0)), S(stream));
+#define BD_GN_FWD_RES_(EM, NT, FOLD)                                                                                       \
+    hipLaunchKernelGGL((gn_fwd_res_kernel<EM, NT, FOLD>), grid, dim3(NT), 0, S(stream), d->x, (long long)d->ldx, d->y,       \
                        (long long)d->ldy, d->HW, d->C, d->G, rp.cb, rp.q, rp.R, rp.E, d->eps, d->gamma, d->beta, d->mean,       \
-                       d->rstd, d->silu, d->y_split, (long long)d->ldys)
+                       d->rstd, d->silu, d->y_split, (long long)d->ldys, fold)
+#define BD_GN_FWD_RES(EM, NT) do { if (fold.part) BD_GN_FWD_RES_(EM, NT, true); else BD_GN_FWD_RES_(EM, NT, false); } while (0)
         if (rp.nt == 512 && rp.E <= 8) BD_GN_FWD_RES(8, 512);
         else if (rp.nt == 512) BD_GN_FWD_RES(GN_RES_EMAX, 512);
         else if (rp.E <= 4) BD_GN_FWD_RES(4, 256);
         else BD_GN_FWD_RES(GN_RES_EMAX, 256);
 #undef BD_GN_FWD_RES
+#undef BD_GN_FWD_RES_
         BD_LAUNCH_CHECK("gn_fwd_res");
         prof_end(rec, S(stream));
         return BD_OK;
@@ -859,7 +929,7 @@
 extern "C" int bd_gn_bwd(const bd_gn_bwd_desc* d, bd_stream_t stream) {
     BD_CHECK(d, BD_ERR_INVALID, "bd_gn_bwd: null descriptor");
     BD_TRY(gn_common_checks("bd_gn_bwd", d->B, d->HW, d->C, d->G, d->x, d->ldx));
-    BD_CHECK(d->gamma && d->beta && d->mean && d->rstd && d->dy && (d->dx || d->dx_split) && d->workspace,
+    BD_CHECK(d->gamma && d->beta && d->mean && d->rstd && (d->dy || d->dy_partials) && (d->dx || d->dx_split) && d->workspace,
              BD_ERR_INVALID, "bd_gn_bwd: null pointer");
     const bool no_params = !d->dgamma && !d->dbeta && !d->param_partials;
     BD_CHECK(no_params || (d->dgamma && d->dbeta), BD_ERR_INVALID, "bd_gn_bwd: dgamma and dbeta go together (both null with null param_partials = no parameter gradients)");
@@ -874,25 +944,36 @@
     BD_CHECK(!(d->dx_colsum && (d->accumulate_dx || d->dx_add)), BD_ERR_INVALID, "bd_gn_bwd: dx_colsum is the column sum of this launch's dx term alone");
     BD_CHECK(!d->dx_add || (d->dx && (d->ld_add & 3) == 0 && aligned16(d->dx_add)), BD_ERR_INVALID, "bd_gn_bwd: dx_add needs dx, a 16B-aligned pointer and ld_add %% 4 == 0");
     GnRes rp;
-    if (gn_resident_plan(d->B, d->HW, d->C, d->G, rp, true)) {
+    const bool resident = gn_resident_plan(d->B, d->HW, d->C, d->G, rp, true);
+    GnFold fold = {};
+    if (d->dy_partials) {
+        BD_CHECK(resident, BD_ERR_UNSUPPORTED, "bd_gn_bwd: dy_partials on a shape the single-pass kernels do not take");
+        BD_CHECK(d->dy_nsplit >= 1 && d->dy_split_stride >= 0, BD_ERR_INVALID, "bd_gn_bwd: dy_partials needs dy_nsplit >= 1 and a stride");
+        BD_CHECK(aligned16(d->dy_partials) && (d->dy_split_stride & 3) == 0, BD_ERR_UNSUPPORTED,
+                 "bd_gn_bwd: dy_partials must be 16B aligned, dy_split_stride a multiple of 4");
+        fold.part = d->dy_partials; fold.nsplit = d->dy_nsplit; fold.stride = (long long)d->dy_split_stride;
+    }
+    if (resident) {
         const size_t need_r = d->param_partials || no_params ? 0 : (size_t)d->B * d->C * 2 * sizeof(float);
         BD_CHECK(d->workspace_bytes >= need_r, BD_ERR_WORKSPACE, "bd_gn_bwd: workspace %zu < %zu", d->workspace_bytes, need_r);
         float* part_r = d->param_partials ? d->param_partials : (no_params ? nullptr : reinterpret_cast<float*>(d->workspace));
         const dim3 grid((unsigned)rp.nblk * (unsigned)d->B);
         int rec = -1;
         if (prof_on())
-            rec = prof_begin("gn_bwd_res", 0.0, (double)d->B * d->HW * 4.0 * ((double)d->C * (2.0 + (d->accumulate_dx ? 1.0 : 0.0) + (d->dx_add ? 1.0 : 0.0) +
+            rec = prof_begin("gn_bwd_res", 0.0, (double)d->B * d->HW * 4.0 * ((double)d->C * (1.0 + (fold.part ? (double)fold.nsplit : 1.0) + (d->accumulate_dx ? 1.0 : 0.0) + (d->dx_add ? 1.0 : 0.0) +
                              (d->dx ? 1.0 : 0.0)) + (d->dx_split ? (double)(xs1 - xs0) : 0.0)), S(stream));
-#define BD_GN_BWD_RES(EM, NT)                                                                                              \
-    hipLaunchKernelGGL((gn_bwd_res_kernel<EM, NT>), grid, dim3(NT), 0, S(stream), d->x, (long long)d->ldx, d->dy,            \
+#define BD_GN_BWD_RES_(EM, NT, FOLD)                                                                                       \
+    hipLaunchKernelGGL((gn_bwd_res_kernel<EM, NT, FOLD>), grid, dim3(NT), 0, S(stream), d->x, (long long)d->ldx, d->dy,            \
                        (long long)d->lddy, d->dx, (long long)d->lddx, d->HW, d->C, d->G, rp.cb, rp.q, rp.R, rp.E, d->gamma,     \
                        d->beta, d->mean, d->rstd, d->silu, d->accumulate_dx, part_r, d->dx_colsum, (long long)d->ld_colsum, \
-                       d->dx_split, (long long)d->lddxs, d->dx_add, (long long)d->ld_add, xs0, xs1)
+                       d->dx_split, (long long)d->lddxs, d->dx_add, (long long)d->ld_add, xs0, xs1, fold)
+#define BD_GN_BWD_RES(EM, NT) do { if (fold.part) BD_GN_BWD_RES_(EM, NT, true); else BD_GN_BWD_RES_(EM, NT, false); } while (0)
         if (rp.nt == 512 && rp.E <= 8) BD_GN_BWD_RES(8, 512);
         else if (rp.nt == 512) BD_GN_BWD_RES(GN_RES_EMAX, 512);
         else if (rp.E <= 4) BD_GN_BWD_RES(4, 256);
         else BD_GN_BWD_RES(GN_RES_EMAX, 256);
 #undef BD_GN_BWD_RES
+#undef BD_GN_BWD_RES_
         BD_LAUNCH_CHECK("gn_bwd_res");
         prof_end(rec, S(stream));
         if (d->param_partials || no_params) return BD_OK;
diff --git a/baddiffusion_amd/csrc/unet_plan.cpp b/baddiffusion_amd/csrc/unet_plan.cpp
--- a/baddiffusion_amd/csrc/unet_plan.cpp
+++ b/baddiffusion_amd/csrc/unet_plan.cpp
@@ -73,6 +73,7 @@
     bool wg = true;
     float* dx = nullptr; int64_t lddx = 0;
     char* opws = nullptr; size_t opws_bytes = 0; size_t opws_need = 0;
+    size_t fold_off = 0, fold_bytes = 0, fold_need = 0;
     hipStream_t st2 = nullptr; hipEvent_t ev_fork = nullptr, ev_join[2] = {nullptr, nullptr};
     char* opws2 = nullptr; int par = 0; bool launched = false, pend[2] = {false, false};
     const uint16_t* w_split = nullptr;
@@ -106,7 +107,9 @@
     const float* residual = nullptr; int64_t ldr = 0;
     float out_scale = 1.f;
     int gn_splits = 0;
+    int fold = 0;
 };
+struct GnFoldIn { int nsplit = 0; const float* bias = nullptr; const float* rowbias = nullptr; int64_t ld_rowbias = 0; };
 
 typedef std::function<int(Ctx&)> Step;
 
@@ -134,6 +137,7 @@
     int fwd_gen = -1, fwd_B = -1; const void* fwd_ws = nullptr;
     int64_t value_floats = 0, grad_floats = 0, scratch_floats = 0;
     size_t opws_bytes = 0, gnpart_floats = 0;
+    size_t opws_gen = 0;
     int T = 0, sumC = 0;
     int64_t p_tw = 0, p_tb = 0;
     int b_tproj = -1, b_dtproj = -1, b_embs = -1;
@@ -322,7 +326,7 @@
     }
 
     int gn_fwd(Ctx& c, const View& x, int64_t pg, int64_t pb, float* y, int64_t ldy, int stats_buf, int silu, bool planes = false,
-               int stats_splits = 0) const {
+               int stats_splits = 0, const GnFoldIn& fi = GnFoldIn()) const {
         bd_gn_fwd_desc d = {};
         d.B = c.B; d.HW = x.H * x.W; d.C = x.C; d.G = cfg.norm_num_groups; d.eps = cfg.norm_eps; d.silu = silu;
         d.x = VP(c, x); d.ldx = x.ld; d.gamma = c.params + pg; d.beta = c.params + pb;
@@ -331,14 +335,24 @@
         d.mean = MEANP(c, stats_buf, d.G); d.rstd = RSTDP(c, stats_buf, d.G);
         d.workspace = c.opws; d.workspace_bytes = c.opws_bytes;
         if (stats_splits > 0) { d.stats = reinterpret_cast<const double*>(c.opws); d.stats_splits = stats_splits; }
+        if (fi.nsplit > 1 && !c.dry) {
+            d.x_partials = reinterpret_cast<const float*>(c.opws + c.fold_off); d.x_nsplit = fi.nsplit; d.x_split_stride = rows(c, x) * x.C;
+            d.x_bias = fi.bias; d.x_rowbias = fi.rowbias; d.ld_x_rowbias = fi.ld_rowbias;
+            d.x_out = VP(c, x); d.ldxo = x.ld; d.ldx = x.C;
+        }
         if (c.dry) { need(c, bd_gn_workspace_bytes(c.B, x.C)); return BD_OK; }
         return bd_gn_fwd(&d, (bd_stream_t)c.st);
     }
-    int gn_bwd(Ctx& c, bd_gn_bwd_desc& d, const View& x, int64_t pg, int64_t pb, int stats_buf, const float* dy, int64_t lddy, int silu) const {
+    int gn_bwd(Ctx& c, bd_gn_bwd_desc& d, const View& x, int64_t pg, int64_t pb, int stats_buf, const float* dy, int64_t lddy, int silu,
+               int fold = 0) const {
         d.B = c.B; d.HW = x.H * x.W; d.C = x.C; d.G = cfg.norm_num_groups; d.silu = silu;
         d.x = VP(c, x); d.ldx = x.ld; d.gamma = c.params + pg; d.beta = c.params + pb;
         d.mean = MEANP(c, stats_buf, d.G); d.rstd = RSTDP(c, stats_buf, d.G);
         d.dy = dy; d.lddy = lddy;
+        if (fold > 1 && !c.dry) {
+            d.dy_partials = reinterpret_cast<const float*>(c.opws + c.fold_off); d.dy_nsplit = fold; d.dy_split_stride = rows(c, x) * x.C;
+            d.lddy = x.C;
+        }
         if (c.wg) { d.dgamma = c.grads + pg; d.dbeta = c.grads + pb; }
         else { d.dx_colsum = nullptr; d.ld_colsum = 0; }
         d.workspace = c.opws; d.workspace_bytes = c.opws_bytes;
@@ -347,7 +361,7 @@
         return bd_gn_bwd(&d, (bd_stream_t)c.st);
     }
     int gn_bwd(Ctx& c, const View& x, int64_t pg, int64_t pb, int stats_buf, const float* dy, int64_t lddy, int silu,
-               const float* dx_add = nullptr, int64_t ld_add = 0, int gs = -1) const {
+               const float* dx_add = nullptr, int64_t ld_add = 0, int gs = -1, int fold = 0) const {
         bd_gn_bwd_desc d = {};
         d.dx_add = dx_add; d.ld_add = ld_add;
         if (gs >= 0 && planes(c) && gsplits[gs].want(lay_batch(c))) {
@@ -355,7 +369,7 @@
             d.dx_split = U16(BP(c, e.b_pl)); d.lddxs = e.C; d.dx_split_c0 = e.coff - x.coff; d.dx_split_c1 = d.dx_split_c0 + e.C;
         }
         d.dx = GP(c, x); d.lddx = x.ld; d.accumulate_dx = take_ginit(c, x.buf);
-        return gn_bwd(c, d, x, pg, pb, stats_buf, dy, lddy, silu);
+        return gn_bwd(c, d, x, pg, pb, stats_buf, dy, lddy, silu, fold);
     }
 
     template <class D>
@@ -375,6 +389,21 @@
     }
     bool phase_ok(const Ctx& c, int H, int W, int Cin, int Cout, int classes = 4, int min_wgs = 128) const {
         return planes(c) && phase_shape(lay_batch(c), H, W, Cin, Cout, classes, min_wgs);
+    }
+    int fold_splits(Ctx& c, bool ps, int H, int W, int K, int N) const {
+        if (!ps) return 0;
+        const int G = cfg.norm_num_groups;
+        auto splits = [&](int B) {
+            if (B <= 0 || bd_gn_fwd_takes_stats(B, H * W, N, G)) return 0;
+            const int ks = bd_conv3x3_ps_ksplit(B, H, W, K, N);
+            return ks > 1 ? ks : 0;
+        };
+        if (c.dry)
+            for (int B : {c.B, c.B / 2, c.B - c.B / 2}) {
+                const size_t bytes = (size_t)splits(B) * (size_t)B * H * W * N * sizeof(float);
+                if (bytes > c.fold_need) c.fold_need = bytes;
+            }
+        return splits(c.B);
     }
     int conv3_planes(Ctx& c, const Conv3& k, int direction, const Opnd& x, float* y, int64_t ldy, int acc, const Conv3Epi& e) const {
         bd_conv3x3_ps_desc d = {};
@@ -390,6 +419,7 @@
             if (c.dry) need(c, (size_t)c.B * e.gn_splits * d.gn_groups * 2 * sizeof(double));
         }
         if (c.dry) { note_conv(c); return BD_OK; }
+        if (e.fold > 1) { d.defer_fold = 1; d.workspace = c.opws + c.fold_off; d.workspace_bytes = c.fold_bytes; }
         return conv3x3_ps(d, c.st);
     }
     int conv3_fwd(Ctx& c, const Conv3& k, bool ps, const Opnd& x, float* y, int64_t ldy, const Conv3Epi& e = Conv3Epi()) const {
@@ -404,8 +434,12 @@
         if (c.w_split) d.w_split = c.w_split + 2 * k.pw;
         return conv3x3_fwd(d, c.st);
     }
-    int conv3_dgrad(Ctx& c, const Conv3& k, bool ps, const Opnd& dy, float* dx, int64_t lddx, int acc) const {
-        if (ps) return conv3_planes(c, k, -1, dy, dx, lddx, acc, Conv3Epi());
+    int conv3_dgrad(Ctx& c, const Conv3& k, bool ps, const Opnd& dy, float* dx, int64_t lddx, int acc, int fold = 0) const {
+        if (ps) {
+            Conv3Epi e;
+            e.fold = fold;
+            return conv3_planes(c, k, -1, dy, dx, lddx, acc, e);
+        }
         bd_conv3x3_dgrad_desc d = {};
         conv3_geometry(d, c, k);
         d.dy = dy.p; d.lddy = dy.ld; d.w = c.params + k.pw; d.dx = dx; d.lddx = lddx; d.accumulate = acc;
@@ -567,8 +601,11 @@
         Conv3Epi e1;
         e1.rowbias = BP(c, b_tproj) + toff; e1.ld_rowbias = sumC_;
         if (ps1 && ps2 && bd_gn_fwd_takes_stats(c.B, HW, Cout, G)) e1.gn_splits = bd_conv3x3_ps_gn_splits(c.B, H, W, Cin, Cout, G);
+        e1.fold = fold_splits(c, ps1, H, W, Cin, Cout);
         BD_TRY(conv3_fwd(c, k1, ps1, {a1, Cin}, BP(c, b_h1), Cout, e1));
-        BD_TRY(gn_fwd(c, h1v, pn2w, pn2b, a2, Cout, b_st2, 1, ps2, e1.gn_splits));
+        GnFoldIn f1;
+        if (e1.fold > 1) { f1.nsplit = e1.fold; f1.bias = c.params + pc1b; f1.rowbias = e1.rowbias; f1.ld_rowbias = e1.ld_rowbias; }
+        BD_TRY(gn_fwd(c, h1v, pn2w, pn2b, a2, Cout, b_st2, 1, ps2, e1.gn_splits, f1));
         Conv3Epi e2;
         e2.residual = VP(c, x); e2.ldr = x.ld; e2.out_scale = inv;
         if (shortcut) {
@@ -588,7 +625,8 @@
         Opnd dy2 = dy;
         if (ps2) BD_TRY(grad_planes(c, gs_out, dy.p, dy.ld, M, Cout, b_dyS, dy2));
         BD_TRY(conv3_wgrad(c, k2, ps2, {BP(c, ps2 ? b_a2s : b_a2), Cout}, dy2));
-        BD_TRY(conv3_dgrad(c, k2, ps2, dy2, BP(c, b_da2), Cout, 0));
+        const int fold2 = fold_splits(c, ps2, H, W, Cout, Cout), fold1 = fold_splits(c, ps1, H, W, Cout, Cin);
+        BD_TRY(conv3_dgrad(c, k2, ps2, dy2, BP(c, b_da2), Cout, 0, fold2));
         float* dh1 = BP(c, ps1 ? b_dh1S : b_dh1);
         {
             bd_gn_bwd_desc d = {};
@@ -596,11 +634,11 @@
             if (ps1) { d.dx_split = U16(dh1); d.lddxs = Cout; }
             else d.dx = dh1;
             d.dx_colsum = BP(c, b_dtproj) + toff; d.ld_colsum = sumC_;
-            BD_TRY(gn_bwd(c, d, h1v, pn2w, pn2b, b_st2, BP(c, b_da2), Cout, 1));
+            BD_TRY(gn_bwd(c, d, h1v, pn2w, pn2b, b_st2, BP(c, b_da2), Cout, 1, fold2));
         }
         if (c.dry) BD_TRY(linear_wgrad(c, BP(c, b_dtproj), sumC_, BP(c, b_embs_), T_, c.grads, c.B, sumC_, T_, c.grads));
         BD_TRY(conv3_wgrad(c, k1, ps1, {BP(c, ps1 ? b_a1s : b_a1), Cin}, {dh1, Cout}));
-        BD_TRY(conv3_dgrad(c, k1, ps1, {dh1, Cout}, BP(c, b_da1), Cin, 0));
+        BD_TRY(conv3_dgrad(c, k1, ps1, {dh1, Cout}, BP(c, b_da1), Cin, 0, fold1));
         if (shortcut) {
             BD_TRY(linear_wgrad(c, dy.p, dy.ld, VP(c, x), x.ld, c.grads + psw, M, Cout, Cin, c.grads + psb));
             const int acc = take_ginit(c, x.buf);
@@ -616,7 +654,7 @@
                 BD_TRY(linear_dgrad(c, dy.p, dy.ld, c.params + psw, GP(c, x), x.ld, M, Cout, Cin, acc));
             }
         }
-        return gn_bwd(c, x, pn1w, pn1b, b_st1, BP(c, b_da1), Cin, 1, shortcut ? nullptr : dy.p, dy.ld, gs_in);
+        return gn_bwd(c, x, pn1w, pn1b, b_st1, BP(c, b_da1), Cin, 1, shortcut ? nullptr : dy.p, dy.ld, gs_in, fold1);
     });
 }
 
@@ -1068,7 +1106,8 @@
     c.opws_bytes = (size_t)1 << 62;
     for (auto& f : fwd) f(c);
     if (training) for (auto it = bwd.rbegin(); it != bwd.rend(); ++it) it->fn(c);
-    opws_bytes = align_up(c.opws_need, 256);
+    opws_gen = align_up(c.opws_need, 256);
+    opws_bytes = opws_gen + align_up(c.fold_need, 256);
     gnpart_floats = training ? c.gnpart_need : 0;
     lay_B = B; lay_train = training; lay_gen = bd::g_tune_gen;
     prep_params = nullptr; prep_ws = nullptr; prep_B = -1;
@@ -1182,7 +1221,7 @@
     c.ws = reinterpret_cast<float*>(workspace);
     const size_t fl = (size_t)(u->value_floats + u->grad_floats + u->scratch_floats) * sizeof(float);
     c.opws = reinterpret_cast<char*>(workspace) + align_up(fl, 256);
-    c.opws_bytes = u->opws_bytes;
+    c.opws_bytes = u->opws_gen; c.fold_off = u->opws_gen; c.fold_bytes = u->opws_bytes - u->opws_gen;
     if (mode_bf16(u->cfg.compute_mode)) {
         c.w_split = reinterpret_cast<const uint16_t*>(c.opws + align_up(u->opws_bytes, 256));
     }
diff --git a/include/bd_hip.h b/include/bd_hip.h
--- a/include/bd_hip.h
+++ b/include/bd_hip.h
@@ -102,6 +102,10 @@
     void* workspace; size_t workspace_bytes;
     uint16_t* y_split; int64_t ldys;
     const double* stats; int stats_splits;
+    const float* x_partials; int x_nsplit; int64_t x_split_stride;
+    const float* x_bias;
+    const float* x_rowbias; int64_t ld_x_rowbias;
+    float* x_out; int64_t ldxo;
 } bd_gn_fwd_desc;
 size_t bd_gn_workspace_bytes(int B, int C);
 int bd_gn_fwd_takes_stats(int B, int HW, int C, int G);
@@ -121,6 +125,7 @@
     const float* dx_add; int64_t ld_add;
     float* param_partials;
     int dx_split_c0, dx_split_c1;
+    const float* dy_partials; int dy_nsplit; int64_t dy_split_stride;
 } bd_gn_bwd_desc;
 int bd_gn_bwd(const bd_gn_bwd_desc* d, bd_stream_t stream);
 int bd_gn_bwd_defers(int B, int HW, int C, int G);
@@ -223,9 +228,11 @@
     void* workspace; size_t workspace_bytes;
     double* gn_part; int gn_groups;
     int mode;
+    int defer_fold;
 } bd_conv3x3_ps_desc;
 size_t bd_conv3x3_ps_workspace_bytes(const bd_conv3x3_ps_desc* d);
 int bd_conv3x3_ps_gn_splits(int B, int H, int W, int K, int N, int groups);
+int bd_conv3x3_ps_ksplit(int B, int H, int W, int K, int N);
 int bd_conv3x3_ps(const bd_conv3x3_ps_desc* d, bd_stream_t stream);
 typedef struct {
     int B, H, W, Cin, Cout;
```
